# burchim/EfficientConformer

Hardware: AMD Instinct MI355X
Metric: audio-frames/sec through encoder, EffConformerCTC-Small, 1/2/4/8 GPU (higher is better)
Workload: dtype bf16; 1 GPU; EfficientConformerCTCSmall: bf16 operands / fp32 accumulate, B=256 utterances/GPU (the largest single-GPU batch measured; SURVEY.md 8d lists B in {4, 32, 128}: --batch 128 is 0.79 x this rate, profiles/r5_31_bench_b128.json), lognormal 1.5-16 s (LibriSpeech-shaped), sorted desc; ragged: every utterance at its own length in one concatenated row space per row range (no pad frames; outputs = the refe; global_batch=256, streams_per_gpu=3, parallelism=dp1 (utterance shards), row_ranges=3 ragged row range(s) per GPU, cut for equal valid frames

## Files before the change

efficientconformer_amd/csrc/attention2.hip:

```cpp
#include "kernels.h"

#include <cstdlib>
#include <type_traits>

namespace {

#ifdef EFFCONF_ABLATE
#define ABLATE(p) ((p).ablate)
#else
#define ABLATE(p) 0
#endif
constexpr int BJ = 64;
constexpr int SKEW_LD = 68;
constexpr float RESCALE_T = 4.0f;
constexpr float NEG_BIG = -1.0e30f;

__device__ __forceinline__ uint4 ld16(const bf16_t* p) {
    typedef uint32_t u32x4_a4 __attribute__((ext_vector_type(4), aligned(2)));
    const u32x4_a4 v = *reinterpret_cast<const u32x4_a4*>(p);
    return make_uint4(v[0], v[1], v[2], v[3]);
}

__device__ __forceinline__ uint4 ld16b(const char* p) { return ld16(reinterpret_cast<const bf16_t*>(p)); }

__device__ __forceinline__ void wave_sync() {
    __builtin_amdgcn_fence(__ATOMIC_RELEASE, "wavefront");
    __builtin_amdgcn_wave_barrier();
    __builtin_amdgcn_fence(__ATOMIC_ACQUIRE, "wavefront");
}

typedef short s16x4 __attribute__((ext_vector_type(4)));
__device__ __forceinline__ uint2 lds_tr16(const char* p) {
    const s16x4 v = __builtin_amdgcn_ds_read_tr16_b64_v4i16((__attribute__((address_space(3))) s16x4*)(p));
    union { s16x4 s; uint2 u; } c;
    c.s = v;
    return c.u;
}

template <int DP, int NWV, int QT>
struct Attn2Smem {
    static constexpr int BI = NWV * 16 * QT;
    static constexpr int ERING = 2 * BI;
    static constexpr bool SWZ = (DP == 64);
    static constexpr int KROW = SWZ ? DP * 2 : DP * 2 + 16;
    static __device__ __forceinline__ int koff(int row, int chunk) { return row * KROW + ((SWZ ? (chunk ^ (2 * ((row >> 1) & 3))) : chunk) << 4); }
    static constexpr int VP = DP * 2 + 32;
    static constexpr int K_BYTES = BJ * KROW, V_BYTES = BJ * VP, E_BYTES = ERING * KROW;
    static constexpr int S_BYTES = NWV * QT * 16 * SKEW_LD * 4;
    static constexpr int TOTAL = K_BYTES + V_BYTES + E_BYTES + S_BYTES;
};

template <int DP, int NWV, int QT, int SETS = 0>
__global__ __launch_bounds__(NWV * 64, (QT == 1 && NWV == 4 && DP <= 96) ? ((DP <= 64 && SETS == 1) ? 3 : 2) : 1) void relpos_attention2_kernel(const AttnParams p) {
    using SM = Attn2Smem<DP, NWV, QT>;
    constexpr int KS = DP / 32, DT = DP / 16, BI = SM::BI, NTHR = NWV * 64, CPR = DP / 8, ERING = SM::ERING;
    extern __shared__ __attribute__((aligned(16))) char smem[];
    char* sK = smem;
    char* sV = sK + SM::K_BYTES;
    char* sE = sV + SM::V_BYTES;
    float* sS = reinterpret_cast<float*>(sE + SM::E_BYTES);

    const int tid = threadIdx.x, lane = tid & 63, wave = tid >> 6;
    const int c = lane & 15, g = lane >> 4;
    int qtiles = (p.Tg + BI - 1) / BI;
    int id = xcd_remap(blockIdx.x, gridDim.x);
    int Tg = p.Tg, T = p.T, qt_wg, h, b;
    {
        const int per_b = p.H * qtiles, q8 = p.B >> 3, r8 = p.B & 7;
        const int u = p.rag_off ? ((ABLATE(p) & 8) ? (id * p.B) / (int)gridDim.x : ragged_find_wave(p.rag_wg, p.B, id)) : id / per_b;
        int x, j;
        if (u < r8 * (q8 + 1)) { x = u / (q8 + 1); j = u - x * (q8 + 1); }
        else { const int u2 = u - r8 * (q8 + 1); x = u2 / q8; j = u2 - x * q8; x += r8; }
        b = x + 8 * j;
        int local = id - (p.rag_off ? ((ABLATE(p) & 8) ? id : p.rag_wg[u]) : u * per_b);
        if (p.rag_off) { T = p.lens[b]; Tg = (T + p.G - 1) / p.G; qtiles = (Tg + BI - 1) / BI; }
        qt_wg = local % qtiles; h = local / qtiles;
    }
    if (ABLATE(p) & 128) return;
    const int i0 = qt_wg * BI, iw0 = i0 + wave * 16 * QT;
    const size_t orow0 = p.rag_off ? (size_t)p.rag_off[b] : (size_t)b * p.T;
    const size_t qoff = (p.rag_off ? orow0 * p.D : (size_t)b * p.q_bstride) + (size_t)h * p.q_hstride;
    const bf16_t* Qu = p.qu + qoff;
    const bf16_t* Kh = p.kh + qoff;
    const bf16_t* Vh = p.vt + qoff;
    const int RS = p.q_rowstride, ERS = p.e_rowstride;
    const bf16_t* Eh = p.eh + (size_t)h * p.e_hstride + (p.rag_off ? (size_t)(p.rag_tgmax - Tg) * ERS : 0);
    const int erows = p.causal ? Tg : 2 * Tg - 1;
    const int dceil = (p.d + 7) & ~7;
    const bool ragged_d = dceil != p.d;

    int nkv = (p.lens[b] + p.G - 1) / p.G;
    nkv = nkv < Tg ? nkv : Tg;
    const int band_l = p.band_l < Tg ? p.band_l : Tg, band_r = p.band_r < Tg ? p.band_r : Tg;
    const bool banded = band_l < Tg || band_r < Tg;
    const bool tile_dead = nkv < 1 || i0 + BI - 1 - band_l >= nkv;
    int kbeg = 0, nkeys = nkv;
    if (tile_dead) nkeys = Tg;
    else if (banded) {
        kbeg = i0 - band_l; kbeg = kbeg < 0 ? 0 : kbeg & ~(BJ - 1);
        const int ke = i0 + BI + band_r;
        nkeys = ke < nkv ? ke : nkv;
    }

    const int R0 = Tg - 1 - i0 - (BI - 1) + kbeg;
    constexpr int NB = ((BI + 63) * CPR + NTHR - 1) / NTHR;
    uint4 fb[NB];
    constexpr int NK = (BJ * CPR + NTHR - 1) / NTHR;
    struct Stage { uint4 lk[NK], lv[NK], le[NK]; };
    Stage sa, sb;
#pragma unroll
    for (int n = 0; n < NK; ++n) { sa.lk[n] = make_uint4(0, 0, 0, 0); sa.lv[n] = sa.lk[n]; sa.le[n] = sa.lk[n]; sb.lk[n] = sa.lk[n]; sb.lv[n] = sa.lk[n]; sb.le[n] = sa.lk[n]; }

    uint32_t koffs[NK];
    auto chunk_row = [&](int n) { int q = tid + NTHR * n; q = q < BJ * CPR ? q : BJ * CPR - 1; return q / CPR; };
    auto tail_mask = [&](uint4 a, int n) {
        int q = tid + NTHR * n; q = q < BJ * CPR ? q : BJ * CPR - 1;
        return mask_chunk(a, p.d - (q - (q / CPR) * CPR) * 8);
    };
#pragma unroll
    for (int n = 0; n < NK; ++n) {
        int q = tid + NTHR * n;
        q = q < BJ * CPR ? q : BJ * CPR - 1;
        const int r = q / CPR, x = (q - r * CPR) * 8, xc = x < dceil ? x : 0;
        koffs[n] = (uint32_t)(r * RS + xc) * 2u;
    }
    auto issue_loads = [&](Stage& st_, int jn) __attribute__((always_inline)) {
        if (((ABLATE(p) & 2) && jn > kbeg) || (ABLATE(p) & 64)) return;
        if (jn + BJ <= Tg - (ragged_d ? 1 : 0)) {
            const char* kb = reinterpret_cast<const char*>(Kh + (size_t)jn * RS);
            const char* vb = reinterpret_cast<const char*>(Vh + (size_t)jn * RS);
#pragma unroll
            for (int n = 0; n < NK; ++n) { st_.lk[n] = ld16b(kb + koffs[n]); st_.lv[n] = ld16b(vb + koffs[n]); }
        } else {
#pragma unroll
            for (int n = 0; n < NK; ++n) {
                const int kr = chunk_row(n), j = jn + kr;
                const size_t o = (size_t)(j < Tg ? j : Tg - 1) * RS * 2 + (koffs[n] - (uint32_t)(kr * RS) * 2u);
                st_.lk[n] = tail_mask(ld16b(reinterpret_cast<const char*>(Kh) + o), n); st_.lv[n] = tail_mask(ld16b(reinterpret_cast<const char*>(Vh) + o), n);
            }
        }
        if (jn > kbeg) {
            const int rnew = R0 + (jn - kbeg) + BI - 1;
            if (rnew >= 0 && rnew + 63 < erows - (ragged_d ? 1 : 0)) {
                const char* eb = reinterpret_cast<const char*>(Eh + (size_t)rnew * ERS);
#pragma unroll
                for (int n = 0; n < NK; ++n) st_.le[n] = ld16b(eb + koffs[n]);
            } else {
#pragma unroll
                for (int n = 0; n < NK; ++n) {
                    const int er = chunk_row(n);
                    int r = rnew + er;
                    r = r < 0 ? 0 : (r >= erows ? erows - 1 : r);
                    st_.le[n] = tail_mask(ld16b(reinterpret_cast<const char*>(Eh) + (size_t)r * ERS * 2 + (koffs[n] - (uint32_t)(er * RS) * 2u)), n);
                }
            }
        }
    };
    issue_loads(sa, kbeg);
#pragma unroll
    for (int n = 0; n < NB; ++n) {
        const int q = tid + NTHR * n;
        const int rr = q / CPR, x = (q - rr * CPR) * 8;
        const int r = R0 + (rr < BI + 63 ? rr : BI + 62);
        const int rc = r < 0 ? 0 : (r >= erows ? erows - 1 : r);
        fb[n] = (ABLATE(p) & 16) ? make_uint4(0, 0, 0, 0) : ld16(Eh + (size_t)rc * ERS + (x < dceil ? x : 0));
    }
    bf16x8 qu[QT][KS], qv[QT][KS];
    {
        const float* dv = p.dvu + (size_t)h * p.dvu_ld;
#pragma unroll
        for (int t = 0; t < QT; ++t) {
            const int i = iw0 + 16 * t + c, ic = i < Tg ? i : Tg - 1;
            uint4 ra[KS];
#pragma unroll
            for (int ks = 0; ks < KS; ++ks) {
                const int x = ks * 32 + g * 8;
                ra[ks] = (ABLATE(p) & 32) ? make_uint4(0, 0, 0, 0) : ld16(Qu + (size_t)ic * RS + (x < dceil ? x : 0));
            }
#pragma unroll
            for (int ks = 0; ks < KS; ++ks) {
                const int x = ks * 32 + g * 8;
                const float4 da = *reinterpret_cast<const float4*>(dv + x), db = *reinterpret_cast<const float4*>(dv + x + 4);
                const int valid = i < Tg ? p.d - x : 0;
                const uint4 m = mask_chunk(ra[ks], valid);
                qu[t][ks] = as_bf16x8(m);
                const uint4 w = make_uint4(pack_bf2(__uint_as_float(m.x << 16) + da.x, __uint_as_float(m.x & 0xFFFF0000u) + da.y),
                                           pack_bf2(__uint_as_float(m.y << 16) + da.z, __uint_as_float(m.y & 0xFFFF0000u) + da.w),
                                           pack_bf2(__uint_as_float(m.z << 16) + db.x, __uint_as_float(m.z & 0xFFFF0000u) + db.y),
                                           pack_bf2(__uint_as_float(m.w << 16) + db.z, __uint_as_float(m.w & 0xFFFF0000u) + db.w));
                qv[t][ks] = as_bf16x8(mask_chunk(w, valid));
            }
        }
    }
#pragma unroll
    for (int n = 0; n < NB; ++n) {
        const int q = tid + NTHR * n;
        const int rr = q / CPR, x = (q - rr * CPR) * 8;
        if (q < (BI + 63) * CPR)
            *reinterpret_cast<uint4*>(sE + SM::koff(rr, x >> 3)) = mask_chunk(fb[n], p.d - x);
    }

    f32x4 acc[QT][DT];
    float m_run[QT], l_run[QT];
#pragma unroll
    for (int t = 0; t < QT; ++t) {
        m_run[t] = NEG_BIG; l_run[t] = 0.f;
#pragma unroll
        for (int dt = 0; dt < DT; ++dt) acc[t][dt] = f32x4{0.f, 0.f, 0.f, 0.f};
    }
    const float scale2 = p.scale * 1.44269504088896340736f;
    float* skew0 = sS + (wave * QT) * 16 * SKEW_LD + c * SKEW_LD;
    const int wcol = c - 15 + 4 * g;
    const int woff1 = BI - 16 * QT - 16 * QT * wave;
    const char* vbase = sV + (4 * g + (c >> 2)) * SM::VP + (c & 3) * 8;

    static_assert(BI == 64, "ring phases: two (BI == BJ)");
    uint32_t ldk[NK], ldv[NK], lde[2][NK];
#pragma unroll
    for (int n = 0; n < NK; ++n) {
        int q = tid + NTHR * n;
        q = q < BJ * CPR ? q : BJ * CPR - 1;
        const int r = q / CPR, ch = q - r * CPR;
        ldk[n] = (uint32_t)SM::koff(r, ch);
        ldv[n] = (uint32_t)(r * SM::VP + ch * 16);
        lde[0][n] = (uint32_t)SM::koff((BI - 1 + r) & (ERING - 1), ch);
        lde[1][n] = (uint32_t)SM::koff((BI - 1 + r + 64) & (ERING - 1), ch);
    }
    constexpr bool FULL = (BJ * CPR) % NTHR == 0;
    auto publish = [&](const Stage& st_, int j0, int par) __attribute__((always_inline)) {
        __syncthreads();
#pragma unroll
        for (int n = 0; n < NK; ++n) {
            if (FULL || tid + NTHR * n < BJ * CPR) {
                *reinterpret_cast<uint4*>(sK + ldk[n]) = st_.lk[n];
                *reinterpret_cast<uint4*>(sV + ldv[n]) = st_.lv[n];
                if (j0 > kbeg) *reinterpret_cast<uint4*>(sE + lde[par][n]) = st_.le[n];
            }
        }
        __syncthreads();
    };

    auto compute_block = [&](int j0, int par, auto jtv) __attribute__((always_inline)) {
        constexpr int JTV = decltype(jtv)::value;
        f32x4 st[QT][JTV];
#pragma unroll
        for (int jt = 0; jt < JTV; ++jt) {
#pragma unroll
            for (int t = 0; t < QT; ++t) st[t][jt] = f32x4{0.f, 0.f, 0.f, 0.f};
#pragma unroll
            for (int ks = 0; ks < KS; ++ks) {
                const bf16x8 a = *reinterpret_cast<const bf16x8*>(sK + SM::koff(jt * 16 + c, ks * 4 + g));
#pragma unroll
                for (int t = 0; t < QT; ++t) st[t][jt] = __builtin_amdgcn_mfma_f32_16x16x32_bf16(a, qu[t][ks], st[t][jt], 0, 0, 0);
            }
        }
        const int rw1 = woff1 + 64 * par;
        constexpr int PU = JTV + 1;
        f32x4 pe[QT][PU];
#pragma unroll
        for (int t = 0; t < QT; ++t)
#pragma unroll
            for (int u = 0; u < PU; ++u) pe[t][u] = f32x4{0.f, 0.f, 0.f, 0.f};
#pragma unroll
        for (int u = 0; u < JTV + QT; ++u) {
            const int er = ((rw1 + u * 16) & (ERING - 1)) + c;
#pragma unroll
            for (int ks = 0; ks < KS; ++ks) {
                const bf16x8 a = *reinterpret_cast<const bf16x8*>(sE + SM::koff(er, ks * 4 + g));
#pragma unroll
                for (int t = 0; t < QT; ++t) {
                    const int ut = u - (QT - 1 - t);
                    if (ut >= 0 && ut < PU) pe[t][ut] = __builtin_amdgcn_mfma_f32_16x16x32_bf16(a, qv[t][ks], pe[t][ut], 0, 0, 0);
                }
            }
        }
#pragma unroll
        for (int t = 0; t < QT; ++t) {
            float* row = skew0 + t * 16 * SKEW_LD + wcol;
#pragma unroll
            for (int r = 0; r < 4; ++r) {
                const bool lo = wcol + r >= 0;
                row[r + (lo ? 0 : 16 * JTV)] = lo ? pe[t][0][r] : pe[t][JTV][r];
            }
#pragma unroll
            for (int u = 1; u < JTV; ++u)
#pragma unroll
                for (int r = 0; r < 4; ++r) row[u * 16 + r] = pe[t][u][r];
        }
        wave_sync();

#pragma unroll
        for (int t = 0; t < QT; ++t) {
            const float* skew = skew0 + t * 16 * SKEW_LD;
            float mloc = -INFINITY;
#pragma unroll
            for (int jt = 0; jt < JTV; ++jt) {
                const f32x4 s4 = *reinterpret_cast<const f32x4*>(skew + jt * 16 + g * 4);
#pragma unroll
                for (int r = 0; r < 4; ++r) st[t][jt][r] += s4[r];
            }
            const int iq0 = iw0 + 16 * t;
            if (j0 + BJ > nkv || (banded && (j0 - (iq0 + 15) < -band_l || j0 + BJ - 1 - iq0 > band_r))) {
                const int iq = iq0 + c;
#pragma unroll
                for (int jt = 0; jt < JTV; ++jt)
#pragma unroll
                    for (int r = 0; r < 4; ++r) {
                        const int j = j0 + jt * 16 + g * 4 + r, dj = j - iq;
                        st[t][jt][r] = (j < nkv && dj <= band_r && dj >= -band_l) ? st[t][jt][r] : NEG_BIG;
                    }
            }
            if (tile_dead) {
                const bool dead = nkv < 1 || iq0 + c - band_l >= nkv;
#pragma unroll
                for (int jt = 0; jt < JTV; ++jt)
#pragma unroll
                    for (int r = 0; r < 4; ++r) st[t][jt][r] = dead ? (j0 + jt * 16 + g * 4 + r < Tg ? 0.f : NEG_BIG) : st[t][jt][r];
            }
#pragma unroll
            for (int jt = 0; jt < JTV; ++jt)
#pragma unroll
                for (int r = 0; r < 4; ++r) mloc = fmaxf(mloc, st[t][jt][r]);
            mloc = fmaxf(mloc, __shfl_xor(mloc, 16));
            mloc = fmaxf(mloc, __shfl_xor(mloc, 32));
            if (!__all((mloc - m_run[t]) * scale2 <= RESCALE_T)) {
                const float m_new = fmaxf(m_run[t], mloc);
                const float alpha = __builtin_amdgcn_exp2f((m_run[t] - m_new) * scale2);
                l_run[t] *= alpha;
#pragma unroll
                for (int dt = 0; dt < DT; ++dt) { acc[t][dt][0] *= alpha; acc[t][dt][1] *= alpha; acc[t][dt][2] *= alpha; acc[t][dt][3] *= alpha; }
                m_run[t] = m_new;
            }
            const float nm = -m_run[t] * scale2;
            float lsum = 0.f;
#pragma unroll
            for (int jt = 0; jt < JTV; ++jt)
#pragma unroll
                for (int r = 0; r < 4; ++r) {
                    const float e = __builtin_amdgcn_exp2f(fmaf(st[t][jt][r], scale2, nm));
                    st[t][jt][r] = e;
                    lsum += e;
                }
            l_run[t] += lsum;
        }
#pragma unroll
        for (int c2 = 0; c2 < JTV / 2; ++c2) {
            bf16x8 pf[QT];
#pragma unroll
            for (int t = 0; t < QT; ++t) {
                uint4 pb;
                pb.x = pack_bf2(st[t][2 * c2][0], st[t][2 * c2][1]);
                pb.y = pack_bf2(st[t][2 * c2][2], st[t][2 * c2][3]);
                pb.z = pack_bf2(st[t][2 * c2 + 1][0], st[t][2 * c2 + 1][1]);
                pb.w = pack_bf2(st[t][2 * c2 + 1][2], st[t][2 * c2 + 1][3]);
                pf[t] = as_bf16x8(pb);
            }
#pragma unroll
            for (int dt = 0; dt < DT; ++dt) {
                const uint2 lo = lds_tr16(vbase + (2 * c2) * 16 * SM::VP + dt * 32);
                const uint2 hi = lds_tr16(vbase + (2 * c2 + 1) * 16 * SM::VP + dt * 32);
                const bf16x8 a = as_bf16x8(make_uint4(lo.x, lo.y, hi.x, hi.y));
#pragma unroll
                for (int t = 0; t < QT; ++t) acc[t][dt] = __builtin_amdgcn_mfma_f32_16x16x32_bf16(a, pf[t], acc[t][dt], 0, 0, 0);
            }
        }
    };

    const bool wave_idle = iw0 >= Tg;
    const bool short_ok = !tile_dead;
    auto run_block = [&](int j0, int par) __attribute__((always_inline)) {
        if (wave_idle || (ABLATE(p) & 1)) return;
        if (short_ok && nkeys - j0 <= 32) compute_block(j0, par, std::integral_constant<int, 2>{});
        else compute_block(j0, par, std::integral_constant<int, 4>{});
    };
    constexpr bool TWO_SETS = SETS == 2 || (SETS == 0 && !(NWV == 2 && DP >= 96));
    if constexpr (TWO_SETS) {
        if (kbeg + BJ < nkeys) issue_loads(sb, kbeg + BJ);
        for (int jb = kbeg; jb < nkeys; jb += 2 * BJ)
#pragma unroll
        for (int half2 = 0; half2 < 2; ++half2) {
            const int j0 = jb + half2 * BJ;
            if (j0 >= nkeys) break;
            if (half2 == 0) publish(sa, j0, 0); else publish(sb, j0, 1);
            if (j0 + 2 * BJ < nkeys) { if (half2 == 0) issue_loads(sa, j0 + 2 * BJ); else issue_loads(sb, j0 + 2 * BJ); }
            run_block(j0, half2);
        }
    } else {
        for (int jb = kbeg; jb < nkeys; jb += 2 * BJ)
#pragma unroll
        for (int half2 = 0; half2 < 2; ++half2) {
            const int j0 = jb + half2 * BJ;
            if (j0 >= nkeys) break;
            publish(sa, j0, half2);
            if (j0 + BJ < nkeys) issue_loads(sa, j0 + BJ);
            run_block(j0, half2);
        }
    }

#pragma unroll
    for (int t = 0; t < QT; ++t) {
        float l_tot = l_run[t] + __shfl_xor(l_run[t], 16);
        l_tot += __shfl_xor(l_tot, 32);
        const float inv = 1.0f / l_tot;
        const int i = iw0 + 16 * t + c;
        if (i >= Tg || (ABLATE(p) & 4)) continue;
#pragma unroll
        for (int dt = 0; dt < DT; ++dt) {
            const int x0 = dt * 16 + g * 4;
            if (x0 >= p.d) continue;
            int n0 = h * p.d + x0, toff = 0;
            while (n0 >= p.D) { n0 -= p.D; ++toff; }
            const int t0 = i * p.G + toff;
            if (x0 + 3 < p.d && n0 + 3 < p.D && (n0 & 1) == 0) {
                if (t0 < T || p.rag_off) {
                    typedef uint32_t u32x2_a4 __attribute__((ext_vector_type(2), aligned(4)));
                    u32x2_a4 w;
                    w[0] = t0 < T ? pack_bf2(acc[t][dt][0] * inv, acc[t][dt][1] * inv) : 0u;
                    w[1] = t0 < T ? pack_bf2(acc[t][dt][2] * inv, acc[t][dt][3] * inv) : 0u;
                    *reinterpret_cast<u32x2_a4*>(p.out + (orow0 + t0) * p.ldo + n0) = w;
                }
            } else {
#pragma unroll
                for (int r = 0; r < 4; ++r) {
                    const int x = x0 + r;
                    if (x >= p.d) continue;
                    int n = h * p.d + x, tf = 0;
                    while (n >= p.D) { n -= p.D; ++tf; }
                    const int tt = i * p.G + tf;
                    if (tt < T || p.rag_off) p.out[(orow0 + tt) * p.ldo + n] = tt < T ? f2bf(acc[t][dt][r] * inv) : (bf16_t)0;
                }
            }
        }
    }
}

template <int DP, int NWV, int QT, int SETS = 0>
int launch2(const AttnParams& p, hipStream_t s) {
    using SM = Attn2Smem<DP, NWV, QT>;
    static_assert(SM::TOTAL <= 160 * 1024, "LDS");
    static LdsAttr attr;
    ensure_dynamic_lds(reinterpret_cast<const void*>(&relpos_attention2_kernel<DP, NWV, QT, SETS>), SM::TOTAL, attr);
    const int qtiles = (p.Tg + SM::BI - 1) / SM::BI;
    const int nwg = p.rag_off ? p.rag_nwg : p.B * p.H * qtiles;
    if (nwg <= 0) return 0;
    hipLaunchKernelGGL((relpos_attention2_kernel<DP, NWV, QT, SETS>), dim3(nwg), dim3(NWV * 64), SM::TOTAL, s, p);
    return hipGetLastError() == hipSuccess ? 0 : -1;
}

}

bool relpos_attention2_supported(int dpad) { return dpad == 32 || dpad == 64 || dpad == 96 || dpad == 128 || dpad == 160; }

int launch_relpos_attention2(const AttnParams& p0, int waves, hipStream_t s) {
    if (p0.B <= 0 || p0.Tg <= 0) return 0;
    AttnParams p = p0;
#ifdef EFFCONF_ABLATE
    static const int abl = getenv("EFFCONF_ATTN_ABLATE") ? atoi(getenv("EFFCONF_ATTN_ABLATE")) : 0;
    p.ablate = abl;
#endif
    if (p.dpad < p.d || p.q_rowstride != p.e_rowstride) return -2;
    if (p.rag_off && (waves != 1 || !p.rag_wg || p.q_rowstride != p.G * p.D)) return -2;
#define ATT2_CASE(DPV, SETS1) case DPV: return waves == 1 ? launch2<DPV, 4, 1, SETS1>(p, s) : launch2<DPV, 2, 2>(p, s);
    switch (p.dpad) {
        ATT2_CASE(32, 0) ATT2_CASE(64, 1) ATT2_CASE(96, 1) ATT2_CASE(128, 0)
        case 160: return launch2<160, 4, 1>(p, s);
    }
#undef ATT2_CASE
    return -3;
}
```

efficientconformer_amd/csrc/encoder.hip:

```cpp
#include "kernels.h"
#include "../../include/effconf.h"
#ifdef EFFCONF_DEBUG_ABI
#include "../../include/effconf_debug.h"
#endif

#include <cmath>
#include <cstdio>
#include <cstdlib>
#include <cstring>
#include <map>
#include <string>
#include <vector>

namespace {

thread_local std::string g_err;
int fail(const std::string& m) { g_err = m; return -1; }
#define EC_TRY(expr) do { int _rc = (expr); if (_rc != 0) return fail(std::string(#expr) + " failed rc=" + std::to_string(_rc)); } while (0)

inline int ld8(int d) { return ec_round_up(d, 8); }

#ifdef EFFCONF_ABLATE
static int ablate_mask() { static const int m = getenv("EFFCONF_SKIP") ? atoi(getenv("EFFCONF_SKIP")) : 0; return m; }
#define EC_ABL(bit, stmt) do { if (!(ablate_mask() & (bit))) { stmt; } } while (0)
#else
#define EC_ABL(bit, stmt) do { stmt; } while (0)
#endif

uint16_t h_f2bf(float f) {
    uint32_t u; memcpy(&u, &f, 4);
    u += 0x7FFFu + ((u >> 16) & 1u);
    return (uint16_t)(u >> 16);
}

struct HostTensor { std::vector<float> data; std::vector<int64_t> shape; };

struct PackedLinear { const bf16_t* w = nullptr; const float* bias = nullptr; int N = 0, K = 0, ldw = 0; std::vector<float> hbias;  };
struct LNp { const float* g = nullptr; const float* b = nullptr; };

struct BlockW {
    LNp ln_ffn1, ln_att, ln_conv, ln_ffn2, ln_out;
    PackedLinear ffn1_a, ffn1_b, qkv, qkv_nat, pos, outp, pw1, pw2, res, ffn2_a, ffn2_b;
    const bf16_t *ffn1_bp = nullptr, *ffn2_bp = nullptr;
    const float *u = nullptr, *v = nullptr, *dw_w = nullptr, *dw_b = nullptr;
    const uint16_t* dw_a3 = nullptr;
    const uint16_t* dw_a = nullptr;
    const float* dvu = nullptr; int dvu_ld = 0;
    const bf16_t* pos_table = nullptr;
    bool chain_in = false, chain_out = false;
    PackedLinear c_outp, c_pw1, c_pw2, c_qkv, c_f1a, c_f2a;
    const bf16_t *c_f1b_cm = nullptr, *c_f2b_cm = nullptr;
    const bf16_t *c_f1b = nullptr, *c_f2b = nullptr; const float *c_f1b2 = nullptr, *c_f2b2 = nullptr;
    int c_qkv_chunks = 0, c_pw1_chunks = 0;
    std::vector<float> h_ln_out_g, h_ln_out_b, h_u, h_v, h_f1b2, h_f2b2;
    const uint16_t *xf_img[2] = {nullptr, nullptr}; const float* xf_b2[2] = {nullptr, nullptr}; int xf_nch[2] = {0, 0};
    const uint16_t *xc_wo = nullptr, *xc_p1 = nullptr, *xc_p2 = nullptr, *xc_qkv = nullptr, *xc_f[2] = {nullptr, nullptr};
    const float *xc_bo = nullptr, *xc_bp2 = nullptr; int xc_nch_p1 = 0;
    bool xc_in = false, xc_out = false;
    const float *cc_b = nullptr, *cc_head = nullptr, *cc_tail = nullptr, *cc_full = nullptr;
};

struct TraceEntry { char name[64]; int64_t offset, rows, cols, ld; int32_t dtype; };
struct ProfRec { int cls; double flops, bytes; };

}

int ec_fail(const char* msg) { return fail(msg ? msg : "error"); }


struct EcEncoder {
    EcConfig cfg;
    std::vector<EcBlock> blocks;
    std::map<std::string, HostTensor> host;
    bool finalized = false;
    std::vector<void*> allocs;
    int wide_gemm = 0;
    size_t guard_bytes = 0;
    const float *sub_w9 = nullptr, *sub_b = nullptr;
    PackedLinear lin;
    const bf16_t* lin_fused = nullptr; int lin_fused_ld = 0;
    const uint16_t *sub3_cimg = nullptr, *sub3_wimg = nullptr; const float* sub3_bias = nullptr; int sub3_ncb = 0, sub3_fo = 0;
    const bf16_t* lin_rs = nullptr; const float* conv_tab = nullptr;
    int fuse_subsample = 2;
    bool fuse_chain = true;
    int ctc_mfma = 2;
    int attention_v2 = 1;
    int chain_full_max = 192;
    int dwconv_mfma = 1;
    int chain_pair = 5;
    int chain_small_m = 4096;
    int chain_max_dim = 256;
    int tiled_auto = 1;
    bool tiled_auto_on = false;
    int tiled_min_k = 256;
    std::vector<float*> att_out;
    int split_chain = 1;
    int sub3_auto = 1;
    int split_sublin = 1;
    int split_ffn = 1;
    int exact_attention = 0;
    bool head_major_odd = false;
    const bf16_t* sub2_w = nullptr; const float* sub2_b = nullptr; int sub2_cp = 0;
    std::vector<BlockW> bw;
    const float *fc_wt = nullptr, *fc_b = nullptr;
    const bf16_t *fc_hi = nullptr, *fc_lo = nullptr;
    const int* block_stride = nullptr;
    const int *block_group = nullptr, *block_heads = nullptr;
    MelTables mel{};
    char* trace_arena = nullptr; size_t trace_bytes = 0, trace_used = 0;
    std::vector<TraceEntry> trace;
    bool e_cache_on = false;
    struct ECacheTag { const void* ws; int batch, tm; size_t layout; };
    std::vector<ECacheTag> e_cache;
    static constexpr size_t E_CACHE_MAX = 16;
    bool e_cache_hit(const void* ws, int batch, int tm, size_t layout) const {
        for (const ECacheTag& t : e_cache) if (t.ws == ws) return t.batch == batch && t.tm == tm && t.layout == layout;
        return false;
    }
    void e_cache_put(const void* ws, int batch, int tm, size_t layout) {
        e_cache_drop(ws);
        if (e_cache.size() >= E_CACHE_MAX) e_cache.erase(e_cache.begin());
        e_cache.push_back({ws, batch, tm, layout});
    }
    void e_cache_drop(const void* ws) {
        for (size_t i = 0; i < e_cache.size(); ++i) if (e_cache[i].ws == ws) { e_cache.erase(e_cache.begin() + i); break; }
    }
    bool exact_pack = false, exact_on = false;
    bool exact_split = false;
    struct SplitW { const uint16_t *hi, *lo; int ldh; };
    std::map<std::string, SplitW> xsplit;
    std::map<std::string, const float*> xw;
    std::map<std::pair<int, int>, const float*> xtab;
    const float *xsub_scale[2] = {nullptr, nullptr}, *xsub_shift[2] = {nullptr, nullptr};
    const uint16_t *xsub_cimg = nullptr, *xsub_wimg = nullptr; const float* xsub_bias = nullptr; int xsub_ncb = 0, xsub_fo = 0;
    bool prof_on = false;
    std::vector<hipEvent_t> prof_ev;
    std::vector<ProfRec> prof_rec;
    size_t prof_next = 0;
};

namespace {

template <class T>
const T* upload(EcEncoder* e, const std::vector<T>& v) {
    const size_t guard = e->guard_bytes, used = v.size() * sizeof(T);
    void* d = nullptr;
    size_t bytes = std::max<size_t>((used + 15) / 16 * 16, 16);
    if (hipMalloc(&d, bytes + 2 * guard) != hipSuccess) return nullptr;
    e->allocs.push_back(d);
    char* base = static_cast<char*>(d) + guard;
    if (guard && (hipMemset(d, 0xFF, guard) != hipSuccess || hipMemset(base + used, 0xFF, bytes - used + guard) != hipSuccess)) return nullptr;
    if (!v.empty() && hipMemcpy(base, v.data(), used, hipMemcpyHostToDevice) != hipSuccess) return nullptr;
    return reinterpret_cast<const T*>(base);
}

const HostTensor* find(EcEncoder* e, const std::string& k) {
    auto it = e->host.find(k);
    return it == e->host.end() ? nullptr : &it->second;
}

bool pack_linear(EcEncoder* e, const std::vector<const float*>& row_ptr, const std::vector<float>& bias, int K, PackedLinear* out,
                 bool kperm = false, const float* ln_g = nullptr, const float* ln_b = nullptr, int min_ldw = 0) {
    const int N = (int)row_ptr.size();
    const int Np = ec_round_up(N, 128), Kp = ec_round_up(K > min_ldw ? K : min_ldw, 64);
    std::vector<uint16_t> w((size_t)Np * Kp, 0);
    std::vector<float> b(Np, 0.f);
    for (int n = 0; n < N && n < (int)bias.size(); ++n) b[n] = bias[n];
    for (int n = 0; n < N; ++n) {
        if (!row_ptr[n]) continue;
        for (int k = 0; k < Kp; ++k) {
            int src = k;
            if (kperm) { const int g = k / 16, pp = k % 16, hh = pp >> 3, ee = pp & 7; src = g * 16 + 4 * hh + 8 * (ee >> 2) + (ee & 3); }
            if (src < K) w[(size_t)n * Kp + k] = h_f2bf(row_ptr[n][src] * (ln_g ? ln_g[src] : 1.0f));
        }
        if (ln_b) {
            double acc = 0.0;
            for (int k = 0; k < K; ++k) acc += (double)row_ptr[n][k] * ln_b[k];
            b[n] += (float)acc;
        }
    }
    out->w = upload(e, w);
    out->bias = upload(e, b);
    out->hbias = b;
    out->N = N; out->K = K; out->ldw = Kp;
    return out->w && out->bias;
}

bool pack_named_linear(EcEncoder* e, const std::string& prefix, int N, int K, PackedLinear* out, std::string* err, bool kperm = false,
                       const std::string& fold_ln = "", int min_ldw = 0) {
    const HostTensor* w = find(e, prefix + ".weight");
    const HostTensor* b = find(e, prefix + ".bias");
    if (!w || !b) { *err = "missing tensor " + prefix + ".weight/.bias"; return false; }
    if ((int64_t)w->data.size() != (int64_t)N * K || (int)b->data.size() != N) { *err = "shape mismatch for " + prefix; return false; }
    std::vector<const float*> rows(N);
    for (int n = 0; n < N; ++n) rows[n] = w->data.data() + (size_t)n * K;
    const HostTensor *lg = fold_ln.empty() ? nullptr : find(e, fold_ln + ".weight"), *lb = fold_ln.empty() ? nullptr : find(e, fold_ln + ".bias");
    if (!fold_ln.empty() && (!lg || !lb || (int)lg->data.size() != K || (int)lb->data.size() != K)) { *err = "missing LayerNorm " + fold_ln; return false; }
    return pack_linear(e, rows, b->data, K, out, kperm, lg ? lg->data.data() : nullptr, lb ? lb->data.data() : nullptr, min_ldw);
}

const bf16_t* pack_ffn2_permuted(EcEncoder* e, const std::string& prefix, int D, int F, float scale = 1.0f) {
    const HostTensor* w = find(e, prefix + ".weight");
    if (!w || (int64_t)w->data.size() != (int64_t)D * F) return nullptr;
    const int Np = ec_round_up(D, 128), Kp = ec_round_up(F, 64);
    std::vector<uint16_t> out((size_t)Np * Kp, 0);
    for (int n = 0; n < D; ++n)
        for (int k = 0; k < Kp; ++k) {
            const int g = k / 16, pp = k % 16, hh = pp >> 3, ee = pp & 7;
            const int src = g * 16 + 4 * hh + 8 * (ee >> 2) + (ee & 3);
            if (src < F) out[(size_t)n * Kp + k] = h_f2bf(scale * w->data[(size_t)n * F + src]);
        }
    return upload(e, out);
}

const bf16_t* pack_ffn2_chunkmajor(EcEncoder* e, const std::string& prefix, int D, int F, float scale, int DP) {
    const HostTensor* w = find(e, prefix + ".weight");
    if (!w || (int64_t)w->data.size() != (int64_t)D * F) return nullptr;
    const int nch = ec_round_up(F, 32) / 32;
    std::vector<uint16_t> out((size_t)nch * DP * 32, 0);
    for (int c = 0; c < nch; ++c)
        for (int n = 0; n < DP; ++n)
            for (int pc = 0; pc < 4; ++pc) {
                const int slot = 4 * n + ((pc + (n >> 2)) & 3);
                for (int i = 0; i < 8; ++i) {
                    const int k = 32 * c + 8 * pc + i;
                    const int g = k / 16, pp = k % 16, hh = pp >> 3, ee = pp & 7;
                    const int src = g * 16 + 4 * hh + 8 * (ee >> 2) + (ee & 3);
                    if (n < D && src < F) out[((size_t)c * DP * 4 + slot) * 8 + i] = h_f2bf(scale * w->data[(size_t)n * F + src]);
                }
            }
    return upload(e, out);
}

bool get_ln(EcEncoder* e, const std::string& prefix, int D, LNp* out, std::string* err) {
    const HostTensor* g = find(e, prefix + ".weight");
    const HostTensor* b = find(e, prefix + ".bias");
    if (!g || !b || (int)g->data.size() != D || (int)b->data.size() != D) { *err = "missing/mis-shaped LayerNorm " + prefix; return false; }
    out->g = upload(e, g->data);
    out->b = upload(e, b->data);
    return out->g && out->b;
}

constexpr float kSplitImgMax = 65000.f;
constexpr float kDwMfmaTwoPlaneNorm = 6.0f;

bool bn_fold(EcEncoder* e, const std::string& prefix, int C, std::vector<float>* scale, std::vector<float>* shift, std::string* err) {
    const HostTensor *g = find(e, prefix + ".weight"), *b = find(e, prefix + ".bias");
    const HostTensor *m = find(e, prefix + ".running_mean"), *v = find(e, prefix + ".running_var");
    if (!g || !b || !m || !v || (int)g->data.size() != C) { *err = "missing/mis-shaped BatchNorm " + prefix; return false; }
    scale->resize(C); shift->resize(C);
    for (int c = 0; c < C; ++c) {
        const float s = g->data[c] / std::sqrt(v->data[c] + 1e-5f);
        (*scale)[c] = s;
        (*shift)[c] = b->data[c] - m->data[c] * s;
    }
    return true;
}

const bf16_t* build_pos_table(EcEncoder* e, int max_pos, int D) {
    const int rows = 2 * max_pos - 1, ld = ld8(D);
    std::vector<uint16_t> t((size_t)rows * ld, 0);
    std::vector<float> denom(D / 2);
    for (int i = 0; i < D / 2; ++i) denom[i] = std::pow(10000.0f, (2.0f * (float)i) / (float)D);
    for (int r = 0; r < rows; ++r) {
        const float pos = (float)(max_pos - 1 - r);
        for (int i = 0; i < D / 2; ++i) {
            const float a = pos / denom[i];
            t[(size_t)r * ld + 2 * i] = h_f2bf(std::sin(a));
            t[(size_t)r * ld + 2 * i + 1] = h_f2bf(std::cos(a));
        }
    }
    return upload(e, t);
}

std::string mel_config_error(const EcConfig& c) {
    if (c.n_fft != 512) return "n_fft = " + std::to_string(c.n_fft) + ": only n_fft = 512 is native";
    if (c.win_length <= 0 || c.win_length > c.n_fft) return "win_length = " + std::to_string(c.win_length) + ": must be in 1..n_fft (" + std::to_string(c.n_fft) + ")";
    if (c.hop_length <= 0) return "hop_length = " + std::to_string(c.hop_length) + ": must be >= 1";
    if (c.n_mels < 1 || c.n_mels > 128) return "n_mels = " + std::to_string(c.n_mels) + ": must be in 1..128";
    if (c.sample_rate < 2) return "sample_rate = " + std::to_string(c.sample_rate) + ": must be >= 2";
    return "";
}

bool build_mel_tables(EcEncoder* e, std::string* err) {
    const EcConfig& c = e->cfg;
    *err = mel_config_error(c);
    if (!err->empty()) return false;
    std::vector<float> win(c.n_fft, 0.f);
    const int off = (c.n_fft - c.win_length) / 2;
    for (int n = 0; n < c.win_length; ++n) win[off + n] = (float)(0.5 - 0.5 * std::cos(2.0 * M_PI * n / c.win_length));
    std::vector<float2> tw(c.n_fft / 2);
    for (int k = 0; k < c.n_fft / 2; ++k) {
        const double a = -2.0 * M_PI * k / c.n_fft;
        tw[k] = make_float2((float)std::cos(a), (float)std::sin(a));
    }
    const int nf = c.n_fft / 2 + 1, nm = c.n_mels;
    const double fmin = 0.0, fmax = 8000.0;
    auto hz2mel = [](double f) { return 2595.0 * std::log10(1.0 + f / 700.0); };
    auto mel2hz = [](double m) { return 700.0 * (std::pow(10.0, m / 2595.0) - 1.0); };
    std::vector<double> fpts(nm + 2);
    for (int i = 0; i < nm + 2; ++i) fpts[i] = mel2hz(hz2mel(fmin) + (hz2mel(fmax) - hz2mel(fmin)) * i / (nm + 1));
    std::vector<int> start(nm), count(nm), offs(nm);
    std::vector<float> wts;
    for (int m = 0; m < nm; ++m) {
        int s0 = -1, cnt = 0;
        std::vector<float> row;
        for (int k = 0; k < nf; ++k) {
            const double f = (double)(c.sample_rate / 2) * k / (nf - 1);
            const double down = (f - fpts[m]) / (fpts[m + 1] - fpts[m]);
            const double up = (fpts[m + 2] - f) / (fpts[m + 2] - fpts[m + 1]);
            const double w = std::max(0.0, std::min(down, up));
            if (w > 0.0) {
                if (s0 < 0) s0 = k;
                row.resize(k - s0 + 1, 0.f);
                row[k - s0] = (float)w;
                cnt = k - s0 + 1;
            }
        }
        start[m] = s0 < 0 ? 0 : s0; count[m] = cnt; offs[m] = (int)wts.size();
        wts.insert(wts.end(), row.begin(), row.begin() + cnt);
    }
    e->mel.window = upload(e, win);
    e->mel.twiddle = upload(e, tw);
    e->mel.fb_start = upload(e, start);
    e->mel.fb_count = upload(e, count);
    e->mel.fb_offset = upload(e, offs);
    e->mel.fb_nnz = (int)wts.size();
    e->mel.fb_weight = upload(e, wts);
    return e->mel.window && e->mel.twiddle && e->mel.fb_weight;
}

struct Shapes {
    int B, Tm, T1;
    std::vector<int> Tin, Tout;
    std::vector<long long> Min, Mout, Mq;
    bool ragged = false;
    std::vector<int> wgs, tiles;
    std::vector<double> tg2;
    long long Mfinal = 0;
};

Shapes make_shapes(const EcEncoder* e, int B, int Tm) {
    Shapes s; s.B = B; s.Tm = Tm;
    int t = Tm;
    for (int i = 0; i < e->cfg.sub_layers; ++i) t = (t - 1) / 2 + 1;
    s.T1 = t;
    for (const EcBlock& b : e->blocks) {
        s.Tin.push_back(t);
        s.Min.push_back((long long)B * t);
        s.Mq.push_back((long long)B * ec_round_up(t, b.group_size));
        if (b.conv_stride > 1) t = (t - 1) / b.conv_stride + 1;
        s.Tout.push_back(t);
        s.Mout.push_back((long long)B * t);
    }
    return s;
}

Shapes make_shapes_ragged(const EcEncoder* e, const std::vector<int>& tm) {
    const int B = (int)tm.size(), nb = (int)e->blocks.size();
    int tmax = 0;
    for (int v : tm) tmax = std::max(tmax, v);
    Shapes s = make_shapes(e, B, tmax);
    s.ragged = true;
    s.Min.assign(nb, 0); s.Mout.assign(nb, 0); s.Mq.assign(nb, 0); s.wgs.assign(nb, 0); s.tiles.assign(nb, 0); s.tg2.assign(nb, 0.0);
    for (int b = 0; b < B; ++b) {
        int t = tm[b];
        for (int i = 0; i < e->cfg.sub_layers; ++i) t = (t - 1) / 2 + 1;
        for (int k = 0; k < nb; ++k) {
            const EcBlock& bk = e->blocks[k];
            const int G = bk.group_size, Gn = k + 1 < nb ? e->blocks[k + 1].group_size : 1;
            const int tp = ec_round_up(t, G);
            s.Min[k] += tp; s.Mq[k] += tp;
            s.wgs[k] += bk.num_heads * ec_cdiv(tp / G, 64);
            s.tg2[k] += (double)(tp / G) * (tp / G);
            if (bk.conv_stride > 1) t = (t - 1) / bk.conv_stride + 1;
            const int top = ec_round_up(t, Gn);
            s.Mout[k] += top;
            s.tiles[k] += ec_cdiv(top, 128);
        }
        s.Mfinal += t;
    }
    return s;
}

struct Workspace {
    size_t total = 0;
    size_t mel, sub, sub1, x0, x1, a, hbuf, qu, kh, vt, eh, o, gbuf, cbuf, xs, lens, preds;
    size_t mel_len = 0, row_off = 0, wg_off = 0, tile_off = 0;
    size_t xrect = 0;
// ... 61 lines not shown
    ProfScope(EcEncoder* e_, hipStream_t st_, int cls, double flops, double bytes) : e(e_), st(st_), on(e_->prof_on) {
        if (!on) return;
        if (e->prof_next + 2 > e->prof_ev.size()) {
            for (int i = 0; i < 2; ++i) { hipEvent_t ev; (void)hipEventCreate(&ev); e->prof_ev.push_back(ev); }
        }
        e->prof_rec.push_back(ProfRec{cls, flops, bytes});
        (void)hipEventRecord(e->prof_ev[e->prof_next], st);
    }
    ~ProfScope() {
        if (!on) return;
        (void)hipEventRecord(e->prof_ev[e->prof_next + 1], st);
        e->prof_next += 2;
    }
};
#define PROF(cls, flops, bytes) ProfScope _prof_scope(e, st, (cls), (double)(flops), (double)(bytes))

void trace_add(EcEncoder* e, hipStream_t st, const char* name, const void* ptr, int64_t rows, int64_t cols, int64_t ld, int dtype) {
    if (!e->trace_arena) return;
    const size_t esz = dtype == 1 ? 2 : 4;
    const size_t bytes = (size_t)rows * ld * esz;
    const size_t off = al(e->trace_used);
    if (off + bytes > e->trace_bytes) return;
    (void)hipMemcpyAsync(e->trace_arena + off, ptr, bytes, hipMemcpyDeviceToDevice, st);
    TraceEntry t{};
    snprintf(t.name, sizeof(t.name), "%s", name);
    t.offset = (int64_t)off; t.rows = rows; t.cols = cols; t.ld = ld; t.dtype = dtype;
    e->trace.push_back(t);
    e->trace_used = off + bytes;
}

enum ProfClass { PC_MEL = 0, PC_SUBCONV = 1, PC_GEMM_FFN = 2, PC_GEMM_OTHER = 3, PC_LAYERNORM = 4, PC_ATTENTION = 5,
                 PC_DWCONV = 6, PC_MISC = 7, PC_COUNT = 8 };

int run_gemm(EcEncoder* e, int cls, hipStream_t st, const bf16_t* A, int lda, int M, const PackedLinear& L, int epi, void* C, int ldc,
             const float* R = nullptr, int ldr = 0, float alpha = 1.f) {
    const double out_b = (epi == EPI_F32) ? 4.0 : (epi == EPI_RESID_F32 ? 8.0 : 2.0);
    PROF(cls, 2.0 * M * (double)L.N * L.K, (double)M * L.K * 2 + (double)L.N * L.K * 2 + (double)M * L.N * out_b);
    GemmParams p{};
    p.A = A; p.lda = lda; p.W = L.w; p.ldw = L.ldw; p.bias = L.bias;
    p.M = M; p.N = L.N; p.K = L.K; p.C = C; p.ldc = ldc; p.R = R; p.ldr = ldr; p.alpha = alpha;
    p.wide = e->wide_gemm;
    return launch_gemm(p, epi, st);
}

inline int F1c(const EcBlock& b) { return ec_round_up(b.dim_model * b.ff_ratio, 32); }

void fill_chain_head(ChainParams& cp, const BlockW& W, int D, int Fp, int T, int Tp, const GemmParams& q) {
    cp.D = D;
    cp.ln[2] = ChainLn{W.ln_ffn1.g, W.ln_ffn1.b};
    cp.ln[3] = ChainLn{W.ln_att.g, W.ln_att.b};
    cp.f[1] = ChainFfn{W.c_f1a.w, W.c_f1a.ldw, W.c_f1a.bias, W.c_f1b, W.ffn1_b.ldw, W.c_f1b2, Fp, W.c_f1b_cm};
    cp.g1 = ChainGemm{W.c_qkv.w, W.c_qkv.ldw, W.c_qkv.bias, W.c_qkv_chunks};
    cp.qu = q.qu; cp.kh = q.kh; cp.vt = q.vt; cp.u = W.u; cp.v = W.v; cp.T = T; cp.Tp = Tp;
}

bool prefer_tiled(const EcEncoder* e, int M, int N, int K);

int run_ffn(EcEncoder* e, hipStream_t st, const bf16_t* a, int M, int D, const PackedLinear& L1, const PackedLinear& L2,
            const bf16_t* w2p, float* x, bf16_t* hbuf, const LNp* ln = nullptr) {
    const int F = L1.N;
    if (ffn_fused_supported(D) && !(prefer_tiled(e, M, F, D) && !ln)) {
        PROF(PC_GEMM_FFN, 4.0 * M * (double)D * F, (double)M * D * 10 + 4.0 * D * F);
        FfnParams p{};
        p.A = a; p.lda = ld8(D); p.X = x; p.ldx = D; p.Y = x; p.ldy = D;
        p.W1 = L1.w; p.ldw1 = L1.ldw; p.b1 = L1.bias; p.W2 = w2p; p.ldw2 = L2.ldw; p.b2 = L2.bias;
        p.M = M; p.D = D; p.Fp = ec_round_up(F, 32); p.alpha = 0.5f;
        if (ln) { p.ln_g = ln->g; p.ln_b = ln->b; }
        return launch_ffn_fused(p, st);
    }
    int rc = run_gemm(e, PC_GEMM_FFN, st, a, ld8(D), M, L1, EPI_SWISH_BF16, hbuf, F);
    if (rc) return rc;
    return run_gemm(e, PC_GEMM_FFN, st, hbuf, F, M, L2, EPI_RESID_F32, x, D, x, D, 0.5f);
}

bool prefer_tiled(const EcEncoder* e, int M, int N, int K) {
    (void)M; (void)N;
    return (e->wide_gemm == 2 || e->wide_gemm == 3 || (e->wide_gemm == 0 && (e->tiled_auto == 2 || (e->tiled_auto && e->tiled_auto_on)))) && K > e->tiled_min_k && K % 8 == 0;
}

int run_rs_or_tiled(EcEncoder* e, int cls, hipStream_t st, const bf16_t* A, int lda, int M, const PackedLinear& L, int rs_epi,
                    int tiled_epi, void* C, int ldc, const float* R = nullptr, int ldr = 0, float alpha = 1.f,
                    const float* lnX = nullptr, const LNp* ln = nullptr) {
    const bool ok = (rs_epi == 0 || rs_epi == 1) ? rs_gemm_resident_supported(L.K, L.N) : rs_gemm_supported(L.K);
    if (!ok) return run_gemm(e, cls, st, A, lda, M, L, tiled_epi, C, ldc, R, ldr, alpha);
    if (prefer_tiled(e, M, L.N, L.K)) {
        if (lnX && ln) { PROF(PC_LAYERNORM, 0, (double)M * L.K * 6); EC_TRY(launch_layernorm(lnX, M, L.K, ln->g, ln->b, nullptr, const_cast<bf16_t*>(A), lda, nullptr, nullptr, st)); }
        return run_gemm(e, cls, st, A, lda, M, L, tiled_epi, C, ldc, R, ldr, alpha);
    }
    const double out_b = (tiled_epi == EPI_F32) ? 4.0 : (tiled_epi == EPI_RESID_F32 ? 8.0 : 2.0);
    PROF(cls, 2.0 * M * (double)L.N * L.K, (double)M * L.K * 2 + (double)L.N * L.K * 2 + (double)M * L.N * out_b);
    GemmParams p{};
    p.A = A; p.lda = lda; p.W = L.w; p.ldw = L.ldw; p.bias = L.bias;
    p.M = M; p.N = L.N; p.K = L.K; p.C = C; p.ldc = ldc; p.R = R; p.ldr = ldr; p.alpha = alpha;
    if (lnX && ln) { p.X = lnX; p.ldx = L.K; p.ln_g = ln->g; p.ln_b = ln->b; }
    return launch_rs_gemm(p, rs_epi, st);
}

bool use_sublinear3(const EcEncoder* e) {
    if (!e->sub3_wimg || e->cfg.sub_layers != 1) return false;
    if (e->fuse_subsample == 3) return true;
    return e->fuse_subsample == 2 && e->sub3_auto && (e->cfg.sub_filters[0] > 128 || e->blocks[0].dim_model > 128);
}

int run_subsample_linear(EcEncoder* e, hipStream_t st, const float* mel, int B, int Tm, int T1, bf16_t* sub, bf16_t* act1, float* x) {
    const EcConfig& c = e->cfg;
    const int C0 = c.sub_filters[0], F2 = c.n_mels / 2, Ksub = C0 * F2;
    if (c.sub_layers == 2) {
        const int Tl1 = (Tm - 1) / 2 + 1, F1 = c.n_mels / 2, F2q = c.n_mels / 4, C1 = c.sub_filters[1];
        { PROF(PC_SUBCONV, 2.0 * 9 * B * Tl1 * (double)C0 * F1, (double)B * c.n_mels * Tm * 4 + (double)B * Tl1 * F1 * e->sub2_cp * 2);
          EC_TRY(launch_subsample_conv_cl(mel, B, c.n_mels, Tm, Tl1, e->sub_w9, e->sub_b, C0, e->sub2_cp, act1, st)); }
        trace_add(e, st, "subsample1", act1, (int64_t)B * F1 * Tl1, C0, e->sub2_cp, 1);
        { PROF(PC_GEMM_OTHER, 2.0 * 9 * (double)B * F2q * T1 * C0 * C1, (double)B * Tl1 * F1 * e->sub2_cp * 2 + (double)B * T1 * F2q * C1 * 2);
          EC_TRY(launch_conv2_igemm(act1, B, F1, Tl1, e->sub2_cp, e->sub2_w, 9 * e->sub2_cp, e->sub2_b, C1, F2q, T1, sub, st)); }
        trace_add(e, st, "subsample", sub, (int64_t)B * T1, F2q * C1, F2q * C1, 1);
        EC_TRY(run_gemm(e, PC_GEMM_OTHER, st, sub, F2q * C1, B * T1, e->lin, EPI_F32, x, e->lin.N));
    } else if (use_sublinear3(e)) {
        PROF(PC_SUBCONV, 2.0 * 9 * B * T1 * (double)Ksub + 2.0 * B * T1 * (double)Ksub * e->lin.N,
             (double)B * c.n_mels * Tm * 4 + (double)B * T1 * e->lin.N * 4);
        SubLin3Params sp{};
        sp.mel = mel; sp.B = B; sp.F = c.n_mels; sp.Tm = Tm; sp.To = T1; sp.rows_max = T1;
        sp.cimg = e->sub3_cimg; sp.wimg = e->sub3_wimg; sp.bias = e->sub3_bias; sp.y = x; sp.ldy = e->lin.N; sp.N = e->lin.N; sp.ncb = e->sub3_ncb; sp.Fo = e->sub3_fo;
        EC_TRY(launch_sublinear3(sp, st));
    } else if (e->fuse_subsample >= 2 && e->lin_rs) {
        PROF(PC_SUBCONV, 2.0 * 9 * B * T1 * (double)Ksub + 2.0 * B * T1 * (double)Ksub * e->lin.N,
             (double)B * c.n_mels * Tm * 4 + (double)B * T1 * e->lin.N * 4);
        EC_TRY(launch_sublinear2(mel, B, c.n_mels, Tm, T1, e->conv_tab, e->lin_rs, e->lin.bias, C0, e->lin.N, x, e->lin.N, st));
    } else if (e->fuse_subsample && e->lin_fused) {
        PROF(PC_SUBCONV, 2.0 * 9 * B * T1 * (double)Ksub + 2.0 * B * T1 * (double)Ksub * e->lin.N,
             (double)B * c.n_mels * Tm * 4 + (double)B * T1 * e->lin.N * 4);
        EC_TRY(launch_sublinear_fused(mel, B, c.n_mels, Tm, T1, e->sub_w9, e->sub_b, C0, e->lin_fused, e->lin_fused_ld,
                                      e->lin.bias, e->lin.N, x, e->lin.N, st));
    } else {
        { PROF(PC_SUBCONV, 2.0 * 9 * B * T1 * (double)Ksub, (double)B * c.n_mels * Tm * 4 + (double)B * T1 * Ksub * 2); EC_TRY(launch_subsample_conv(mel, B, c.n_mels, Tm, T1, e->sub_w9, e->sub_b, C0, sub, Ksub, st)); }
        trace_add(e, st, "subsample", sub, (int64_t)B * T1, Ksub, Ksub, 1);
        EC_TRY(run_gemm(e, PC_GEMM_OTHER, st, sub, Ksub, B * T1, e->lin, EPI_F32, x, e->lin.N));
    }
    return 0;
}

static const void* dw_mfma_table(const EcEncoder* e, const uint16_t* t, int ks) { return (e->dwconv_mfma == 2 || (e->dwconv_mfma == 1 && ks == 15)) ? t : nullptr; }
static bool pair_on(const EcEncoder* e, int D) { return e->chain_pair && chain3_supported(D); }

int forward_core(EcEncoder* e, const float* mel, const int64_t* in_len, int from_audio, const Shapes& s, const Workspace& w,
                 char* ws, float* out, int64_t* out_len, hipStream_t st, int out_frames = 0) {
    const EcConfig& c = e->cfg;
    const int B = s.B, nb = (int)e->blocks.size();
    const bool rg = s.ragged;
    e->trace.clear(); e->trace_used = 0;
    int* lens = reinterpret_cast<int*>(ws + w.lens);
    const int *mel_len = nullptr, *row_off = nullptr, *wg_off = nullptr, *tile_off = nullptr;
    if (rg) {
        int* ml = reinterpret_cast<int*>(ws + w.mel_len); int* ro = reinterpret_cast<int*>(ws + w.row_off);
        int* wo = reinterpret_cast<int*>(ws + w.wg_off); int* to = reinterpret_cast<int*>(ws + w.tile_off);
        PROF(PC_MISC, 0, 0);
        EC_TRY(launch_lengths_ragged(in_len, B, from_audio, c.hop_length, c.sub_layers, e->block_stride, e->block_group, e->block_heads, nb, lens, ml,
                                     ro, wo, to, out_len, st));
        mel_len = ml; row_off = ro; wg_off = wo; tile_off = to;
    } else {
        PROF(PC_MISC, 0, 0); EC_TRY(launch_lengths(in_len, B, from_audio, c.hop_length, c.sub_layers, e->block_stride, nb, lens, out_len, st));
    }
    if (from_audio) trace_add(e, st, "mel", mel, (int64_t)B * c.n_mels, s.Tm, s.Tm, 0);
    auto rows_at = [&](int k) { RaggedRows r{}; r.off = row_off + (size_t)k * (B + 1); r.len = lens + (size_t)k * B; r.n = B;
                                r.rows = (int)(k < nb ? s.Min[k] : s.Mfinal); r.tmax = k < nb ? s.Tin[k] : s.Tout[nb - 1]; return r; };

    float* x = reinterpret_cast<float*>(ws + w.x0);
    float* xalt = reinterpret_cast<float*>(ws + w.x1);
    if (rg) {
        const int C0 = c.sub_filters[0], Ksub = C0 * (c.n_mels / 2);
        const RaggedRows r0 = rows_at(0);
        if (c.sub_layers == 2) {
            bf16_t* sub = reinterpret_cast<bf16_t*>(ws + w.sub);
            bf16_t* act1 = reinterpret_cast<bf16_t*>(ws + w.sub1);
            float* xrect = reinterpret_cast<float*>(ws + w.xrect);
            const int Tl1 = (s.Tm - 1) / 2 + 1, T1r = (Tl1 - 1) / 2 + 1, F1 = c.n_mels / 2, F2q = c.n_mels / 4, C1 = c.sub_filters[1];
            { PROF(PC_SUBCONV, 2.0 * 9 * B * Tl1 * (double)C0 * F1, (double)B * c.n_mels * s.Tm * 4 + (double)B * Tl1 * F1 * e->sub2_cp * 2);
              EC_TRY(launch_subsample_conv_cl(mel, B, c.n_mels, s.Tm, Tl1, e->sub_w9, e->sub_b, C0, e->sub2_cp, act1, st, mel_len)); }
            trace_add(e, st, "subsample1", act1, (int64_t)B * F1 * Tl1, C0, e->sub2_cp, 1);
            { PROF(PC_GEMM_OTHER, 2.0 * 9 * (double)B * F2q * T1r * C0 * C1, (double)B * Tl1 * F1 * e->sub2_cp * 2 + (double)B * T1r * F2q * C1 * 2);
              EC_TRY(launch_conv2_igemm(act1, B, F1, Tl1, e->sub2_cp, e->sub2_w, 9 * e->sub2_cp, e->sub2_b, C1, F2q, T1r, sub, st)); }
            trace_add(e, st, "subsample", sub, (int64_t)B * T1r, F2q * C1, F2q * C1, 1);
            EC_TRY(run_gemm(e, PC_GEMM_OTHER, st, sub, F2q * C1, B * T1r, e->lin, EPI_F32, xrect, e->lin.N));
            { PROF(PC_MISC, 0, (double)s.Min[0] * e->lin.N * 8); EC_TRY(launch_gather_rows(xrect, e->lin.N, T1r, r0, x, st)); }
        } else if (use_sublinear3(e)) {
            PROF(PC_SUBCONV, 2.0 * 9 * (double)s.Min[0] * Ksub + 2.0 * (double)s.Min[0] * Ksub * e->lin.N, (double)B * c.n_mels * s.Tm * 4 + (double)s.Min[0] * e->lin.N * 4);
            SubLin3Params sp{};
            sp.mel = mel; sp.B = B; sp.F = c.n_mels; sp.Tm = s.Tm; sp.mel_len = mel_len; sp.off = r0.off; sp.len = r0.len;
            sp.rows_max = ec_round_up(s.Tin[0], e->blocks[0].group_size);
            sp.cimg = e->sub3_cimg; sp.wimg = e->sub3_wimg; sp.bias = e->sub3_bias; sp.y = x; sp.ldy = e->lin.N; sp.N = e->lin.N; sp.ncb = e->sub3_ncb; sp.Fo = e->sub3_fo;
            EC_TRY(launch_sublinear3(sp, st));
        } else if (e->fuse_subsample >= 2 && e->lin_rs) {
            PROF(PC_SUBCONV, 2.0 * 9 * (double)s.Min[0] * Ksub + 2.0 * (double)s.Min[0] * Ksub * e->lin.N, (double)B * c.n_mels * s.Tm * 4 + (double)s.Min[0] * e->lin.N * 4);
            EC_ABL(32, EC_TRY(launch_sublinear2(mel, B, c.n_mels, s.Tm, s.T1, e->conv_tab, e->lin_rs, e->lin.bias, C0, e->lin.N, x, e->lin.N, st, &r0, mel_len)));
        } else {
            bf16_t* sub = reinterpret_cast<bf16_t*>(ws + w.sub);
            const int T1r = (s.Tm - 1) / 2 + 1;
            const int Tcover = T1r + e->blocks[0].group_size - 1;
            { PROF(PC_SUBCONV, 2.0 * 9 * (double)s.Min[0] * Ksub, (double)B * c.n_mels * s.Tm * 4 + (double)s.Min[0] * Ksub * 2);
              EC_TRY(launch_subsample_conv(mel, B, c.n_mels, s.Tm, Tcover, e->sub_w9, e->sub_b, C0, sub, Ksub, st, mel_len, &r0)); }
            trace_add(e, st, "subsample", sub, s.Min[0], Ksub, Ksub, 1);
            EC_TRY(run_gemm(e, PC_GEMM_OTHER, st, sub, Ksub, (int)s.Min[0], e->lin, EPI_F32, x, e->lin.N));
        }
    } else {
        EC_TRY(run_subsample_linear(e, st, mel, B, s.Tm, s.T1, reinterpret_cast<bf16_t*>(ws + w.sub), reinterpret_cast<bf16_t*>(ws + w.sub1), x));
    }
    trace_add(e, st, "linear", x, s.Min[0], e->lin.N, e->lin.N, 0);

    bf16_t* a = reinterpret_cast<bf16_t*>(ws + w.a);
    bf16_t* hbuf = reinterpret_cast<bf16_t*>(ws + w.hbuf);
    bf16_t* o = reinterpret_cast<bf16_t*>(ws + w.o);
    bf16_t* gbuf = reinterpret_cast<bf16_t*>(ws + w.gbuf);
    bf16_t* cbuf = reinterpret_cast<bf16_t*>(ws + w.cbuf);
    bf16_t* xs = reinterpret_cast<bf16_t*>(ws + w.xs);
    bool have_a = false, head_done = false;
    char nm[64];
    hipStreamCaptureStatus cap = hipStreamCaptureStatusNone;
    const bool capturing = hipStreamIsCapturing(st, &cap) == hipSuccess && cap != hipStreamCaptureStatusNone;
    const int e_tag = rg ? -(s.Tin[0] + 1) : s.Tm;
    const bool e_cached = !capturing && e->e_cache_on && e->e_cache_hit(ws, B, e_tag, w.eh_blk[0]);
    if (!e_cached) e->e_cache_drop(ws);

    int mask_stride = 1;
    for (int k = 0; k < nb; ++k) {
        const EcBlock& b = e->blocks[k];
        const BlockW& W = e->bw[k];
        const int T = s.Tin[k], To = s.Tout[k], D = b.dim_model, De = b.dim_expand;
        const int M = (int)s.Min[k], Mo = (int)s.Mout[k];
        const int G = b.group_size, H = b.num_heads;
        const int Tp = ec_round_up(T, G), Tg = Tp / G, Tgp = ec_round_up(Tg, 8);
        const int d = G * D / H, dpad = ec_round_up(d, 32);
        const bool head_major_odd = e->head_major_odd;
        const bool nat = (d % 2) == 0 || !head_major_odd;
        if (rg && !nat) return fail("ragged batches use the natural Q / K / V layout (option head_major_odd = 0)");
        const int qT = rg ? M : T, qTp = rg ? M : Tp;
        const bool chain_head = e->fuse_chain && W.chain_in && nat && chain_head_supported(D) && D <= e->chain_max_dim;
        const bool chain_b = e->fuse_chain && W.chain_in && D <= e->chain_max_dim;
        const bool chain_tail = e->fuse_chain && W.chain_out && chain_tail_supported(De) && De <= e->chain_max_dim;
        GemmParams p{};
        p.A = a; p.lda = ld8(D); p.W = W.qkv.w; p.ldw = W.qkv.ldw; p.bias = W.qkv.bias;
        p.M = M; p.N = 3 * D; p.K = D;
        p.T = qT; p.G = rg ? 1 : G; p.H = H; p.D = D; p.d = d; p.dpad = dpad; p.Tg = rg ? M : Tg; p.Tgp = Tgp;
        p.qu = reinterpret_cast<bf16_t*>(ws + w.qu);
        p.kh = reinterpret_cast<bf16_t*>(ws + w.kh); p.vt = reinterpret_cast<bf16_t*>(ws + w.vt);
        p.u = W.u; p.v = W.v;
        if (head_done) {
        } else if (chain_head) {
            ChainParams cp{};
            cp.small_m = e->chain_small_m; cp.pair = e->chain_pair;
            fill_chain_head(cp, W, D, F1c(b), qT, qTp, p);
            cp.M = M; cp.X = x; cp.ldx = D; cp.Y = x; cp.ldy = D; cp.consts = W.cc_head;
            PROF(PC_GEMM_FFN, 2.0 * M * (double)D * (2.0 * D * b.ff_ratio + 3.0 * D), (double)M * D * 16 + 22.0 * D * D);
            EC_ABL(2, EC_TRY(launch_chain(cp, CHAIN_A_HEAD, st)));
        } else {
            { PROF(PC_LAYERNORM, 0, (double)M * D * 6); if (!have_a) EC_TRY(launch_layernorm(x, M, D, W.ln_ffn1.g, W.ln_ffn1.b, nullptr, a, ld8(D), nullptr, nullptr, st)); }
            EC_TRY(run_ffn(e, st, a, M, D, W.ffn1_a, W.ffn1_b, W.ffn1_bp, x, hbuf));
            const bool qkv_tiled = nat && prefer_tiled(e, M, 3 * D, D);
            const bool ln_fused = rs_gemm_supported(D) && !qkv_tiled;
            if (!ln_fused) { PROF(PC_LAYERNORM, 0, (double)M * D * 6); EC_TRY(launch_layernorm(x, M, D, W.ln_att.g, W.ln_att.b, nullptr, a, ld8(D), nullptr, nullptr, st)); }
            { PROF(PC_GEMM_OTHER, 2.0 * M * 3.0 * D * D, (double)M * D * 2 + 3.0 * D * D * 2 + (double)M * D * 8);
              if (ln_fused) {
                  if (nat) { p.W = W.qkv_nat.w; p.ldw = W.qkv_nat.ldw; p.bias = W.qkv_nat.bias; }
                  p.X = x; p.ldx = D; p.ln_g = W.ln_att.g; p.ln_b = W.ln_att.b;
                  EC_TRY(launch_rs_gemm(p, nat ? 4 : 3, st));
              } else {
                  p.wide = e->wide_gemm;
                  EC_TRY(launch_gemm(p, nat ? EPI_QKV_NAT : EPI_QKV, st));
              } }
        }
        snprintf(nm, sizeof(nm), "blocks.%d.x_ffn1", k); trace_add(e, st, nm, x, M, D, D, 0);

        {
            { PROF(PC_MISC, 0, 0);
              if (rg) EC_ABL(64, EC_TRY(launch_attn_pad_rows_ragged(p.qu, p.kh, p.vt, W.u, D, G, rows_at(k), st)));
              else EC_TRY(nat ? launch_attn_pad_rows_nat(p, B, st) : launch_attn_pad_rows(p, B, st)); }
            GemmParams pe{};
            const int erows = c.causal ? Tp : 2 * Tp - G;
            pe.A = W.pos_table + (size_t)(b.max_pos - Tp + (c.causal ? 0 : G / 2)) * ld8(D); pe.lda = ld8(D);
            pe.W = W.pos.w; pe.ldw = W.pos.ldw; pe.bias = W.pos.bias;
            pe.M = erows; pe.N = D; pe.K = D;
            pe.T = erows; pe.G = G; pe.H = H; pe.D = D; pe.d = d; pe.dpad = dpad; pe.Tg = c.causal ? Tg : 2 * Tg - 1; pe.Tgp = 0;
            pe.kh = reinterpret_cast<bf16_t*>(ws + w.eh_blk[k]);
            pe.C = pe.kh; pe.ldc = D;
            if (Tp > b.max_pos) return fail("sequence longer than max_pos_encoding");
            if (!e_cached) { PROF(PC_GEMM_OTHER, 2.0 * erows * (double)D * D, (double)erows * D * 4 + (double)D * D * 2);
                             EC_TRY(launch_gemm(pe, nat ? EPI_BF16 : EPI_HEADS, st)); }
            if (e->trace_arena && nat) {
                const int64_t qrows = rg ? (int64_t)M : (int64_t)B * Tp;
                snprintf(nm, sizeof(nm), "blocks.%d.qu", k); trace_add(e, st, nm, p.qu, qrows, D, D, 1);
                snprintf(nm, sizeof(nm), "blocks.%d.k", k); trace_add(e, st, nm, p.kh, qrows, D, D, 1);
                snprintf(nm, sizeof(nm), "blocks.%d.v", k); trace_add(e, st, nm, p.vt, qrows, D, D, 1);
                snprintf(nm, sizeof(nm), "blocks.%d.e", k); trace_add(e, st, nm, pe.kh, erows, D, D, 1);
            }
            AttnParams ap{};
            ap.qu = p.qu; ap.kh = p.kh; ap.vt = p.vt; ap.eh = pe.kh;
            ap.dvu = W.dvu; ap.dvu_ld = W.dvu_ld;
            ap.lens = lens + (size_t)k * B;
            ap.B = B; ap.H = H; ap.T = T; ap.G = G; ap.D = D; ap.d = d; ap.dpad = dpad; ap.Tg = Tg; ap.Tgp = Tgp;
            if (nat) { ap.q_bstride = (long long)Tp * D; ap.q_hstride = d; ap.q_rowstride = G * D; ap.e_hstride = d; ap.e_rowstride = G * D; }
            else { ap.q_bstride = (long long)H * Tg * dpad; ap.q_hstride = (long long)Tg * dpad; ap.q_rowstride = dpad;
                   ap.e_hstride = (long long)(2 * Tg - 1) * dpad; ap.e_rowstride = dpad; }
            ap.out = o; ap.ldo = ld8(D); ap.scale = 1.0f / std::sqrt((float)d);
            const long long unit = (long long)mask_stride * G;
            ap.band_l = (int)std::min<long long>(c.left_context / unit, 1 << 30); ap.band_r = (int)std::min<long long>(c.right_context / unit, 1 << 30);
            ap.causal = c.causal;
            const bool streaming = c.causal || ap.band_l < Tg || ap.band_r < Tg;
            if (streaming && !(nat && relpos_attention2_supported(dpad) && e->attention_v2))
                return fail("streaming contexts / causal attention run on attention2.hip (natural layout, padded head width <= 160, option attention_v2 != 0)");
            if (rg) {
                if (!relpos_attention2_supported(dpad)) return fail("ragged batches need attention2.hip (padded head width <= 160)");
                ap.rag_off = row_off + (size_t)k * (B + 1); ap.rag_wg = wg_off + (size_t)k * (B + 1); ap.rag_nwg = s.wgs[k]; ap.rag_tgmax = Tg;
            }
            { PROF(PC_ATTENTION, 2.0 * H * (rg ? s.tg2[k] : (double)B * Tg * Tg) * d * 3.0, (double)M * D * 2 * 5);
              if (rg || streaming) EC_ABL(1, EC_TRY(launch_relpos_attention2(ap, 1, st))); else
              if (e->attention_v2 && nat && relpos_attention2_supported(dpad)) EC_TRY(launch_relpos_attention2(ap, e->attention_v2, st));
              else EC_TRY(launch_relpos_attention(ap, st)); }
            if ((int)e->att_out.size() == nb && e->att_out[k]) {
                EC_TRY(launch_attention_probs(ap, e->att_out[k], st));
            }
            snprintf(nm, sizeof(nm), "blocks.%d.att_o", k); trace_add(e, st, nm, o, M, D, ld8(D), 1);
            if (chain_b) {
                ChainParams cp{};
                cp.small_m = e->chain_small_m; cp.pair = e->chain_pair;
                cp.M = M; cp.D = D; cp.X = x; cp.ldx = D; cp.Y = x; cp.ldy = D; cp.A = o; cp.lda = ld8(D);
                cp.g0 = ChainGemm{W.c_outp.w, W.c_outp.ldw, W.c_outp.bias, 0};
                cp.ln[0] = ChainLn{W.ln_conv.g, W.ln_conv.b};
                cp.g1 = ChainGemm{W.c_pw1.w, W.c_pw1.ldw, W.c_pw1.bias, W.c_pw1_chunks};
                cp.glu = gbuf; cp.ldg = ld8(De); cp.Ng = De; cp.T = qT; cp.Tp = qTp; cp.consts = W.cc_b;
                PROF(PC_GEMM_OTHER, 2.0 * M * (double)D * (D + 2.0 * De), (double)M * D * 10 + (double)M * De * 2 + 2.0 * D * (D + 2.0 * De));
                EC_ABL(4, EC_TRY(launch_chain(cp, CHAIN_B, st)));
            } else {
                EC_TRY(run_rs_or_tiled(e, PC_GEMM_OTHER, st, o, ld8(D), M, W.outp, 0, EPI_RESID_F32, x, D, x, D, 1.0f));
            }
            snprintf(nm, sizeof(nm), "blocks.%d.x_mhsa", k); trace_add(e, st, nm, x, M, D, D, 0);
        }

        if (chain_b) {
        } else if (rs_gemm_supported(D)) {
            EC_TRY(run_rs_or_tiled(e, PC_GEMM_OTHER, st, a, ld8(D), M, W.pw1, 2, EPI_GLU_BF16, gbuf, ld8(De), nullptr, 0, 1.f, x, &W.ln_conv));
        } else {
            { PROF(PC_LAYERNORM, 0, (double)M * D * 6); EC_TRY(launch_layernorm(x, M, D, W.ln_conv.g, W.ln_conv.b, nullptr, a, ld8(D), nullptr, nullptr, st)); }
            EC_TRY(run_rs_or_tiled(e, PC_GEMM_OTHER, st, a, ld8(D), M, W.pw1, 2, EPI_GLU_BF16, gbuf, ld8(De)));
        }
        snprintf(nm, sizeof(nm), "blocks.%d.glu", k); trace_add(e, st, nm, gbuf, M, De, ld8(De), 1);
        RaggedConv rc{};
        if (rg) { rc.in_off = row_off + (size_t)k * (B + 1); rc.in_len = lens + (size_t)k * B; rc.out_off = row_off + (size_t)(k + 1) * (B + 1);
                  rc.out_len = lens + (size_t)(k + 1) * B; rc.tile_off = tile_off + (size_t)k * (B + 1); rc.tiles = s.tiles[k]; rc.n = B; rc.out_rows = Mo; }
        { PROF(PC_DWCONV, 2.0 * Mo * (double)De * b.kernel_size, (double)M * De * 2 + (double)Mo * De * 2); EC_ABL(8, EC_TRY(launch_dwconv(gbuf, B, T, To, De, ld8(De), W.dw_w, W.dw_b, b.kernel_size, b.conv_stride, cbuf, st, rg ? &rc : nullptr, c.causal, dw_mfma_table(e, W.dw_a, b.kernel_size), W.dw_a3))); }
        mask_stride *= b.conv_stride;
        snprintf(nm, sizeof(nm), "blocks.%d.dw", k); trace_add(e, st, nm, cbuf, Mo, De, ld8(De), 1);
        if (D != De) {
            { PROF(PC_MISC, 0, (double)Mo * D * 6); EC_ABL(64, EC_TRY(launch_cast_rows(x, D, T, b.conv_stride, To, B, xs, ld8(D), st, rg ? &rc : nullptr))); }
            EC_TRY(run_rs_or_tiled(e, PC_GEMM_OTHER, st, xs, ld8(D), Mo, W.res, 1, EPI_F32, xalt, De));
            std::swap(x, xalt);
        } else if (b.conv_stride > 1) {
            return fail("strided block without expansion is not native (no shipped config uses it)");
        }
        const bool last = (k == nb - 1);
        float* xo = (last && !rg) ? out : x;
        if (chain_tail) {
            bool next_head = false;
            if (!last) {
                const EcBlock& nbk = e->blocks[k + 1];
                next_head = W.cc_full && nbk.dim_model <= e->chain_max_dim && e->bw[k + 1].chain_in && chain_full_supported(De, pair_on(e, De) ? 256 : e->chain_full_max) && (((nbk.group_size * nbk.dim_model / nbk.num_heads) % 2) == 0 || !head_major_odd) && nbk.dim_model == De;
            }
            ChainParams cp{};
            cp.small_m = e->chain_small_m; cp.pair = e->chain_pair;
            cp.M = Mo; cp.D = De; cp.X = x; cp.ldx = De; cp.Y = xo; cp.ldy = De; cp.A = cbuf; cp.lda = ld8(De);
            cp.g0 = ChainGemm{W.c_pw2.w, W.c_pw2.ldw, W.c_pw2.bias, 0};
            cp.ln[0] = ChainLn{W.ln_ffn2.g, W.ln_ffn2.b};
            cp.ln[1] = ChainLn{W.ln_out.g, W.ln_out.b};
            cp.f[0] = ChainFfn{W.c_f2a.w, W.c_f2a.ldw, W.c_f2a.bias, W.c_f2b, W.ffn2_b.ldw, W.c_f2b2, ec_round_up(De * b.ff_ratio, 32), W.c_f2b_cm};
            double fl = 2.0 * Mo * (double)De * (De + 2.0 * De * b.ff_ratio), by = (double)Mo * De * 10 + 2.0 * De * De * (1 + 2.0 * b.ff_ratio);
            if (next_head) {
                const EcBlock& nbk = e->blocks[k + 1];
                const int Gn = nbk.group_size;
                const int Tn = rg ? Mo : s.Tin[k + 1], Tpn = rg ? Mo : ec_round_up(Tn, Gn);
                GemmParams pn{};
                pn.qu = reinterpret_cast<bf16_t*>(ws + w.qu);
                pn.kh = reinterpret_cast<bf16_t*>(ws + w.kh); pn.vt = reinterpret_cast<bf16_t*>(ws + w.vt);
                fill_chain_head(cp, e->bw[k + 1], De, F1c(nbk), Tn, Tpn, pn);
                fl += 2.0 * Mo * (double)De * (2.0 * De * nbk.ff_ratio + 3.0 * De); by += (double)Mo * De * 8 + 2.0 * De * De * (3 + 2.0 * nbk.ff_ratio);
            }
            cp.consts = next_head ? W.cc_full : W.cc_tail;
            { PROF(PC_GEMM_FFN, fl, by); EC_ABL(2, EC_TRY(launch_chain(cp, next_head ? CHAIN_A_FULL : CHAIN_A_TAIL, st))); }
            head_done = next_head;
            have_a = false;
            if (last) { snprintf(nm, sizeof(nm), "blocks.%d.out", k); trace_add(e, st, nm, xo, Mo, De, De, 0); }
            continue;
        }
        head_done = false;
        EC_TRY(run_rs_or_tiled(e, PC_GEMM_OTHER, st, cbuf, ld8(De), Mo, W.pw2, 0, EPI_RESID_F32, x, De, x, De, 1.0f));
        snprintf(nm, sizeof(nm), "blocks.%d.x_conv", k); trace_add(e, st, nm, x, Mo, De, De, 0);

        if (ffn_fused_supported(De) && !prefer_tiled(e, Mo, De * b.ff_ratio, De)) {
            EC_TRY(run_ffn(e, st, a, Mo, De, W.ffn2_a, W.ffn2_b, W.ffn2_bp, x, hbuf, &W.ln_ffn2));
        } else {
            { PROF(PC_LAYERNORM, 0, (double)Mo * De * 6); EC_TRY(launch_layernorm(x, Mo, De, W.ln_ffn2.g, W.ln_ffn2.b, nullptr, a, ld8(De), nullptr, nullptr, st)); }
            EC_TRY(run_ffn(e, st, a, Mo, De, W.ffn2_a, W.ffn2_b, W.ffn2_bp, x, hbuf));
        }
        { PROF(PC_LAYERNORM, 0, (double)Mo * De * 10); EC_TRY(launch_layernorm(x, Mo, De, W.ln_out.g, W.ln_out.b, xo, last ? nullptr : a, ld8(De),
                                last ? nullptr : e->bw[k + 1].ln_ffn1.g, last ? nullptr : e->bw[k + 1].ln_ffn1.b, st)); }
        have_a = !last;
        snprintf(nm, sizeof(nm), "blocks.%d.out", k); trace_add(e, st, nm, xo, Mo, De, De, 0);
    }
    if (!capturing) e->e_cache_put(ws, B, e_tag, w.eh_blk[0]);
    if (rg) {
        const RaggedRows rl = rows_at(nb);
        PROF(PC_MISC, 0, (double)s.Mfinal * e->blocks.back().dim_expand * 4 + (double)B * out_frames * e->blocks.back().dim_expand * 4);
        EC_TRY(launch_emit_rows(x, e->blocks.back().dim_expand, rl.off, rl.len, B, out_frames, out, st));
    }
    return 0;
}

struct XWorkspace { size_t total = 0, conv1, sub, x0, x1, a, h, q, k, v, e, o, p1, g, c, lens, scores = 0; size_t qkv_stride = 0;
                    std::vector<size_t> ep_blk;
                    size_t kp = 0, vp = 0, ep = 0, xs = 0, xrect = 0, mel_len = 0, row_off = 0, wg_off = 0, tile_off = 0; };

XWorkspace make_xworkspace(const EcEncoder* e, const Shapes& s) {
    XWorkspace w;
    size_t off = 0;
    auto take = [&](size_t floats) { size_t o = off; off += al(floats * 4); return o; };
    const size_t B = s.B;
    size_t mx = 0, mh = 0, mq = 0, me = 0, mp = 0, mg = 0, mc = 0, mkp = 0, mvp = 0, mep = 0, mxs = 0;
    for (size_t k = 0; k < e->blocks.size(); ++k) {
        const EcBlock& b = e->blocks[k];
        const size_t T = s.Tin[k], D = b.dim_model, De = b.dim_expand;
        const size_t Mi = (size_t)s.Min[k], Mo = (size_t)s.Mout[k], Mqk = (size_t)s.Mq[k];
        const size_t Tp = ec_round_up((int)T, b.group_size);
        mx = std::max(mx, std::max(Mi * D, Mo * De));
        mh = std::max(mh, std::max(Mi * D, Mo * De) * b.ff_ratio);
        mq = std::max(mq, Mqk * D);
        me = std::max(me, (2 * Tp - b.group_size) * D);
        {
            const size_t dh = b.group_size * D / b.num_heads, pk = sxf_attention_pk((int)dh), vx = sxf_attention_vx((int)dh), Tg = Tp / b.group_size;
            mkp = std::max(mkp, (Mqk / b.group_size + 64) * b.num_heads * 2 * pk / 2);
            mvp = std::max(mvp, B * b.num_heads * 2 * vx * (size_t)ec_round_up((int)Tg, 64) / 2);
            mep = std::max(mep, 2 * Tg * b.num_heads * 2 * pk / 2);
        }
        mp = std::max(mp, Mi * 2 * De);
        mg = std::max(mg, Mi * De);
        mc = std::max(mc, Mo * De);
        if (D != De) mxs = std::max(mxs, Mo * D);
    }
    const int L = e->cfg.sub_layers;
    size_t T1r = s.Tm; for (int i = 0; i < L; ++i) T1r = (T1r - 1) / 2 + 1;
    const size_t F1 = (e->cfg.n_mels - 1) / 2 + 1, Tl1 = (s.Tm - 1) / 2 + 1;
    w.conv1 = take(L == 2 ? B * e->cfg.sub_filters[0] * F1 * Tl1 : 0);
    int F = e->cfg.n_mels; for (int i = 0; i < L; ++i) F = (F - 1) / 2 + 1;
    w.sub = take(B * T1r * (size_t)e->cfg.sub_filters[L - 1] * F);
    w.x0 = take(mx); w.x1 = take(mx); w.a = take(mx); w.h = take(mh);
    w.q = take(mq); w.k = take(mq); w.v = take(mq); w.e = take(me); w.o = take(mq);
    w.p1 = take(mp); w.g = take(mg); w.c = take(mc);
    w.lens = take((e->blocks.size() + 1) * B);
    w.qkv_stride = (w.k - w.q) / 4;
    if (e->exact_split) {
        size_t ms = 0;
        if (!s.ragged)
            for (size_t k = 0; k < e->blocks.size(); ++k) {
                const EcBlock& b = e->blocks[k];
                const int Tg = ec_round_up(s.Tin[k], b.group_size) / b.group_size;
                ms = std::max(ms, sx_attention_scores_bytes(s.B, b.num_heads, Tg) / 4);
            }
        w.scores = take(ms);
        w.kp = take(mkp); w.vp = take(mvp); w.ep = take(mep); w.xs = take(mxs);
        for (size_t k = 0; k < e->blocks.size(); ++k) {
            const EcBlock& b = e->blocks[k];
            const size_t dh = b.group_size * b.dim_model / b.num_heads, pk = sxf_attention_pk((int)dh), Tg = ec_round_up(s.Tin[k], b.group_size) / b.group_size;
            w.ep_blk.push_back(take(2 * Tg * b.num_heads * 2 * pk / 2));
        }
        if (s.ragged) {
            const size_t nbk = e->blocks.size();
            w.xrect = take(B * T1r * e->blocks[0].dim_model);
            w.mel_len = take(B);
            w.row_off = take((nbk + 1) * (B + 1));
            w.wg_off = take(nbk * (B + 1));
            w.tile_off = take(nbk * (B + 1));
        }
    }
    w.total = off;
    return w;
}

const float* xget(EcEncoder* e, const std::string& k) {
    auto it = e->xw.find(k);
    return it == e->xw.end() ? nullptr : it->second;
}

int xgemm(EcEncoder* e, hipStream_t st, const float* A, int lda, int M, const std::string& prefix, int N, int K, float* C, int ldc, int epi = 0,
          const float* R = nullptr, float alpha = 1.f, int a_rows = 0, int a_pitch = 0, int a_stride = 0, int c_rows = 0, int c_pitch = 0,
          int split_cols = 0, size_t split_stride = 0, int cls = PC_GEMM_OTHER) {
    ExGemmParams p{};
    p.A = A; p.lda = lda; p.a_rows = a_rows; p.a_pitch = a_pitch; p.a_stride = a_stride;
    p.W = xget(e, prefix + ".weight"); p.ldw = K; p.bias = xget(e, prefix + ".bias");
    if (!p.bias) return fail("exact mode: missing " + prefix);
    p.M = M; p.N = N; p.K = K; p.C = C; p.ldc = ldc; p.c_rows = c_rows; p.c_pitch = c_pitch;
    p.split_cols = split_cols; p.split_stride = split_stride;
    p.R = R; p.ldr = ldc; p.alpha = alpha; p.epi = epi;
    PROF(cls, 2.0 * M * (double)N * K, 4.0 * ((double)M * K + (double)N * K + (double)M * N));
    if (e->exact_split) {
        auto it = e->xsplit.find(prefix);
        if (it != e->xsplit.end()) {
            SxGemmParams q{};
            q.g = p; q.Whi = it->second.hi; q.Wlo = it->second.lo; q.ldh = it->second.ldh;
            const int rc = launch_sx_gemm(q, st);
            if (rc != -2 || !p.W) return rc;
        }
    }
    if (!p.W) return fail("exact mode: missing " + prefix);
    return launch_ex_gemm(p, st);
}

int forward_core_exact(EcEncoder* e, const float* mel, const int64_t* in_len, int from_audio, const Shapes& s, const XWorkspace& w,
                       char* ws, float* out, int64_t* out_len, hipStream_t st) {
    const EcConfig& c = e->cfg;
    const int B = s.B, nb = (int)e->blocks.size();
    if (c.causal) return fail("the label-exact modes have no causal kernels (causal relative tables / depthwise pre-padding): bf16 path only");
    e->trace.clear(); e->trace_used = 0;
    e->e_cache_drop(ws);
    auto F32 = [&](size_t off) { return reinterpret_cast<float*>(ws + off); };
    int* lens = reinterpret_cast<int*>(ws + w.lens);
    EC_TRY(launch_lengths(in_len, B, from_audio, c.hop_length, c.sub_layers, e->block_stride, nb, lens, out_len, st));
    if (from_audio) trace_add(e, st, "mel", mel, (int64_t)B * c.n_mels, s.Tm, s.Tm, 0);
    float* sub = F32(w.sub);
    const int C0 = c.sub_filters[0];
    int Fl = c.n_mels, Cl = C0;
    if (c.sub_layers == 1) {
        EC_TRY(launch_ex_conv2d(mel, B, 1, c.n_mels, s.Tm, xget(e, "subsampling_module.layers.0.0.weight"), e->xsub_scale[0], e->xsub_shift[0], C0, sub, 1, st));
        Fl = (c.n_mels - 1) / 2 + 1;
    } else {
        float* img = F32(w.conv1);
        const int F1 = (c.n_mels - 1) / 2 + 1, T1 = (s.Tm - 1) / 2 + 1, C1 = c.sub_filters[1];
        EC_TRY(launch_ex_conv2d(mel, B, 1, c.n_mels, s.Tm, xget(e, "subsampling_module.layers.0.0.weight"), e->xsub_scale[0], e->xsub_shift[0], C0, img, 0, st));
        EC_TRY(launch_ex_conv2d(img, B, C0, F1, T1, xget(e, "subsampling_module.layers.1.0.weight"), e->xsub_scale[1], e->xsub_shift[1], C1, sub, 1, st));
        Fl = (F1 - 1) / 2 + 1; Cl = C1;
    }
    const int Ksub = Cl * Fl;
    trace_add(e, st, "subsample", sub, (int64_t)B * s.T1, Ksub, Ksub, 0);
    float* x = F32(w.x0);
    float* xalt = F32(w.x1);
    const int D0 = e->blocks[0].dim_model;
    EC_TRY(xgemm(e, st, sub, Ksub, B * s.T1, "linear", D0, Ksub, x, D0));
    trace_add(e, st, "linear", x, (int64_t)B * s.T1, D0, D0, 0);
    float *a = F32(w.a), *hb = F32(w.h), *q = F32(w.q), *kk = F32(w.k), *v = F32(w.v), *eb = F32(w.e), *o = F32(w.o), *p1 = F32(w.p1), *g = F32(w.g),
          *cb = F32(w.c);
    char nm[64];
    int xmask_stride = 1;
    for (int k = 0; k < nb; ++k) {
        const EcBlock& b = e->blocks[k];
        const BlockW& W = e->bw[k];
        const int T = s.Tin[k], To = s.Tout[k], D = b.dim_model, De = b.dim_expand, M = B * T, Mo = B * To;
        const int G = b.group_size, H = b.num_heads, Tp = ec_round_up(T, G), Tg = Tp / G, d = G * D / H;
        const std::string p = "blocks." + std::to_string(k);
        EC_TRY(launch_layernorm(x, M, D, W.ln_ffn1.g, W.ln_ffn1.b, a, nullptr, 0, nullptr, nullptr, st));
        EC_TRY(xgemm(e, st, a, D, M, p + ".feed_forward_module1.layers.1", D * b.ff_ratio, D, hb, D * b.ff_ratio, 1, nullptr, 1.f, 0, 0, 0, 0, 0, 0, 0, PC_GEMM_FFN));
        EC_TRY(xgemm(e, st, hb, D * b.ff_ratio, M, p + ".feed_forward_module1.layers.4", D, D * b.ff_ratio, x, D, 2, x, 0.5f, 0, 0, 0, 0, 0, 0, 0, PC_GEMM_FFN));
        snprintf(nm, sizeof(nm), "blocks.%d.x_ffn1", k); trace_add(e, st, nm, x, M, D, D, 0);
        const std::string m = p + ".multi_head_self_attention_module";
        EC_TRY(launch_layernorm(x, M, D, W.ln_att.g, W.ln_att.b, a, nullptr, 0, nullptr, nullptr, st));
        if (Tp != T) {
            if (hipMemsetAsync(q, 0, (size_t)B * Tp * D * 4, st) != hipSuccess || hipMemsetAsync(kk, 0, (size_t)B * Tp * D * 4, st) != hipSuccess ||
                hipMemsetAsync(v, 0, (size_t)B * Tp * D * 4, st) != hipSuccess) return fail("memset failed");
        }
        if (e->exact_split && e->xsplit.count(m + ".mhsa.qkv_layer")) {
            EC_TRY(xgemm(e, st, a, D, M, m + ".mhsa.qkv_layer", 3 * D, D, q, D, 0, nullptr, 1.f, 0, 0, 0, T, Tp, D, w.qkv_stride));
        } else {
            EC_TRY(xgemm(e, st, a, D, M, m + ".mhsa.query_layer", D, D, q, D, 0, nullptr, 1.f, 0, 0, 0, T, Tp));
            EC_TRY(xgemm(e, st, a, D, M, m + ".mhsa.key_layer", D, D, kk, D, 0, nullptr, 1.f, 0, 0, 0, T, Tp));
            EC_TRY(xgemm(e, st, a, D, M, m + ".mhsa.value_layer", D, D, v, D, 0, nullptr, 1.f, 0, 0, 0, T, Tp));
        }
        if (Tp > b.max_pos) return fail("sequence longer than max_pos_encoding");
        const float* tab = e->xtab[std::make_pair(b.max_pos, D)];
        EC_TRY(xgemm(e, st, tab + (size_t)(b.max_pos - Tp + G / 2) * D, D, 2 * Tp - G, m + ".mhsa.pos_layer", D, D, eb, D));
        ExAttnParams ap{};
        ap.q = q; ap.k = kk; ap.v = v; ap.e = eb; ap.u = W.u; ap.vb = W.v; ap.lens = lens + (size_t)k * B;
        ap.B = B; ap.H = H; ap.T = T; ap.Tp = Tp; ap.G = G; ap.D = D; ap.d = d; ap.Tg = Tg; ap.out = o; ap.variant = e->exact_attention;
        ap.att = (int)e->att_out.size() == nb ? e->att_out[k] : nullptr;
        {
            const long long unit = (long long)xmask_stride * G;
            ap.band_l = (int)std::min<long long>(c.left_context / unit, 1 << 30); ap.band_r = (int)std::min<long long>(c.right_context / unit, 1 << 30);
        }
        { PROF(PC_ATTENTION, 2.0 * B * H * (double)Tg * Tg * d * 3.0, (double)M * D * 4 * 5);
          if (e->exact_split && sx_attention_supported(d) && (long long)B * H <= 65535) EC_TRY(launch_sx_attention(ap, F32(w.scores), st));
          else EC_TRY(launch_ex_attention(ap, st)); }
        EC_TRY(xgemm(e, st, o, D, M, m + ".mhsa.output_layer", D, D, x, D, 2, x, 1.0f, T, Tp, 1));
        snprintf(nm, sizeof(nm), "blocks.%d.x_mhsa", k); trace_add(e, st, nm, x, M, D, D, 0);
        const std::string cm = p + ".convolution_module.layers";
        EC_TRY(launch_layernorm(x, M, D, W.ln_conv.g, W.ln_conv.b, a, nullptr, 0, nullptr, nullptr, st));
        EC_TRY(xgemm(e, st, a, D, M, cm + ".2", 2 * De, D, p1, 2 * De));
        EC_TRY(launch_ex_glu(p1, M, De, g, st));
        EC_TRY(launch_ex_dwconv(g, B, T, To, De, W.dw_w, W.dw_b, b.kernel_size, b.conv_stride, cb, st));
        xmask_stride *= b.conv_stride;
        if (D != De) {
            EC_TRY(xgemm(e, st, x, D, Mo, p + ".conv_res.1", De, D, xalt, De, 0, nullptr, 1.f, To, T, b.conv_stride));
            std::swap(x, xalt);
        } else if (b.conv_stride > 1) {
            return fail("strided block without expansion is not native (no shipped config uses it)");
        }
        EC_TRY(xgemm(e, st, cb, De, Mo, cm + ".7", De, De, x, De, 2, x, 1.0f));
        snprintf(nm, sizeof(nm), "blocks.%d.x_conv", k); trace_add(e, st, nm, x, Mo, De, De, 0);
        EC_TRY(launch_layernorm(x, Mo, De, W.ln_ffn2.g, W.ln_ffn2.b, a, nullptr, 0, nullptr, nullptr, st));
        EC_TRY(xgemm(e, st, a, De, Mo, p + ".feed_forward_module2.layers.1", De * b.ff_ratio, De, hb, De * b.ff_ratio, 1, nullptr, 1.f, 0, 0, 0, 0, 0, 0, 0, PC_GEMM_FFN));
        EC_TRY(xgemm(e, st, hb, De * b.ff_ratio, Mo, p + ".feed_forward_module2.layers.4", De, De * b.ff_ratio, x, De, 2, x, 0.5f, 0, 0, 0, 0, 0, 0, 0, PC_GEMM_FFN));
        float* xo = (k == nb - 1) ? out : xalt;
        EC_TRY(launch_layernorm(x, Mo, De, W.ln_out.g, W.ln_out.b, xo, nullptr, 0, nullptr, nullptr, st));
        if (k != nb - 1) std::swap(x, xalt);
        snprintf(nm, sizeof(nm), "blocks.%d.out", k); trace_add(e, st, nm, xo, Mo, De, De, 0);
    }
// ... 762 lines not shown
                    for (int n = 0; n < D; ++n) b2h[n] = 0.5f * b2->data[n];
                    e->bw[k].xf_img[which] = upload(e, img); e->bw[k].xf_b2[which] = upload(e, b2h); e->bw[k].xf_nch[which] = nch;
                }
            {
                auto perm16 = [](int pos) { const int khh = pos >> 3, ee = pos & 7; return 8 * (ee >> 2) + 4 * khh + (ee & 3); };
                bool over = false;
                auto put = [&](std::vector<uint16_t>& img, size_t hi_at, size_t lo_at, double wv) {
                    const float ws = (float)(wv * 1024.0);
                    if (!(std::fabs(ws) < kSplitImgMax)) { over = true; return; }
                    const _Float16 hh = (_Float16)ws;
                    img[hi_at] = half_bits((float)hh);
                    img[lo_at] = half_bits(ws - (float)hh);
                };
                auto f1_chunk = [&](std::vector<uint16_t>& img, size_t base, int DP1, int K, const float* const* wrow, const float* bias, const float* g, const float* beta) {
                    for (int r = 0; r < 32; ++r) {
                        if (!wrow[r]) continue;
                        double bsum = bias[r];
                        for (int col = 0; col < DP1; ++col) {
                            const int f = (col & ~15) + perm16(col & 15);
                            if (f < K) {
                                const double wv = wrow[r][f];
                                if (beta) bsum += wv * beta[f];
                                put(img, base + (size_t)r * DP1 + col, base + (size_t)32 * DP1 + (size_t)r * DP1 + col, g ? wv * g[f] : wv);
                            }
                        }
                        for (int col = 0; col < DP1; ++col)
                            if ((col & ~15) + perm16(col & 15) == K) put(img, base + (size_t)r * DP1 + col, base + (size_t)32 * DP1 + (size_t)r * DP1 + col, bsum);
                    }
                };
                auto f2_chunk = [&](std::vector<uint16_t>& img, size_t base, int DP2, int c, const float* Wm, int N, int K, int ldw, double scale) {
                    for (int n = 0; n < N; ++n)
                        for (int pos = 0; pos < 32; ++pos) {
                            const int kk = 32 * c + (pos & ~15) + perm16(pos & 15);
                            if (kk < K) put(img, base + (size_t)n * 32 + pos, base + (size_t)32 * DP2 + (size_t)n * 32 + pos, scale * Wm[(size_t)n * ldw + kk]);
                        }
                };
                auto padded = [&](const std::vector<float>& v, int n, float scale) { std::vector<float> o(n, 0.f); for (size_t i = 0; i < v.size() && (int)i < n; ++i) o[i] = scale * v[i]; return o; };
                for (size_t k = 0; k < e->blocks.size(); ++k) {
                    const EcBlock& b = e->blocks[k];
                    BlockW& W = e->bw[k];
                    const int D = b.dim_model, De = b.dim_expand;
                    const std::string pb = "blocks." + std::to_string(k);
                    const std::string mh = pb + ".multi_head_self_attention_module.", cm = pb + ".convolution_module.layers.";
                    auto ffn_image = [&](int which, int Dw) -> const uint16_t* {
                        const int F = Dw * b.ff_ratio;
                        const std::string pf = pb + (which ? ".feed_forward_module2.layers." : ".feed_forward_module1.layers.");
                        const HostTensor *g = find(e, pf + "0.weight"), *bt = find(e, pf + "0.bias"), *w1 = find(e, pf + "1.weight"), *b1 = find(e, pf + "1.bias"),
                                         *w2 = find(e, pf + "4.weight");
                        if (!g || !bt || !w1 || !b1 || !w2 || (int64_t)w1->data.size() != (int64_t)F * Dw || (int64_t)w2->data.size() != (int64_t)F * Dw ||
                            (int)g->data.size() != Dw || (int)bt->data.size() != Dw || (int)b1->data.size() != F || !W.xf_b2[which]) return nullptr;
                        int ks, nt; sxf_ffn_shape(Dw, &ks, &nt);
                        const int DP1 = 16 * ks, DP2 = 32 * nt, nch = (F + 31) / 32;
                        const size_t per = (size_t)64 * (DP1 + DP2);
                        std::vector<uint16_t> img((size_t)nch * per, 0);
                        for (int c = 0; c < nch; ++c) {
                            const float* rows[32]; float bias[32];
                            for (int r = 0; r < 32; ++r) { const int h = 32 * c + r; rows[r] = h < F ? w1->data.data() + (size_t)h * Dw : nullptr; bias[r] = h < F ? b1->data[h] : 0.f; }
                            f1_chunk(img, (size_t)c * per, DP1, Dw, rows, bias, g->data.data(), bt->data.data());
                            f2_chunk(img, (size_t)c * per + (size_t)64 * DP1, DP2, c, w2->data.data(), Dw, F, F, 0.5);
                        }
                        return over ? nullptr : upload(e, img);
                    };
                    if (sxc_supported(D) && sxf_ffn_supported(D)) {
                        int ks, nt; sxf_ffn_shape(D, &ks, &nt);
                        const int DP1 = 16 * ks, DP2 = 32 * nt, nte = (De + 31) / 32;
                        const HostTensor *wo = find(e, mh + "mhsa.output_layer.weight"), *bo = find(e, mh + "mhsa.output_layer.bias"), *lg = find(e, cm + "0.weight"), *lb = find(e, cm + "0.bias"),
                                         *w1 = find(e, cm + "2.weight"), *b1 = find(e, cm + "2.bias"), *ag = find(e, mh + "norm.weight"), *ab = find(e, mh + "norm.bias");
                        const HostTensor *wq[3] = {find(e, mh + "mhsa.query_layer.weight"), find(e, mh + "mhsa.key_layer.weight"), find(e, mh + "mhsa.value_layer.weight")};
                        const HostTensor *bq[3] = {find(e, mh + "mhsa.query_layer.bias"), find(e, mh + "mhsa.key_layer.bias"), find(e, mh + "mhsa.value_layer.bias")};
                        bool ok = wo && bo && lg && lb && w1 && b1 && ag && ab && (int)wo->data.size() == D * D && (int)bo->data.size() == D && (int)lg->data.size() == D && (int)lb->data.size() == D &&
                                  (int64_t)w1->data.size() == (int64_t)2 * De * D && (int)b1->data.size() == 2 * De && (int)ag->data.size() == D && (int)ab->data.size() == D;
                        for (int i = 0; i < 3; ++i) ok = ok && wq[i] && bq[i] && (int)wq[i]->data.size() == D * D && (int)bq[i]->data.size() == D;
                        if (ok) {
                            over = false;
                            std::vector<uint16_t> io((size_t)nt * 64 * DP2, 0);
                            for (int c = 0; c < nt; ++c) f2_chunk(io, (size_t)c * 64 * DP2, DP2, c, wo->data.data(), D, D, D, 1.0);
                            std::vector<uint16_t> ip((size_t)2 * nte * 64 * DP1, 0);
                            for (int c = 0; c < 2 * nte; ++c) {
                                const float* rows[32]; float bias[32];
                                for (int r = 0; r < 32; ++r) { const int f = 32 * (c >> 1) + r, n = (c & 1) * De + f; rows[r] = f < De ? w1->data.data() + (size_t)n * D : nullptr; bias[r] = f < De ? b1->data[n] : 0.f; }
                                f1_chunk(ip, (size_t)c * 64 * DP1, DP1, D, rows, bias, lg->data.data(), lb->data.data());
                            }
                            std::vector<uint16_t> iq((size_t)3 * nt * 64 * DP1, 0);
                            for (int c = 0; c < 3 * nt; ++c) {
                                const int which = c / nt, cc = c % nt;
                                const float* rows[32]; float bias[32];
                                for (int r = 0; r < 32; ++r) { const int n = 32 * cc + r; rows[r] = n < D ? wq[which]->data.data() + (size_t)n * D : nullptr; bias[r] = n < D ? bq[which]->data[n] : 0.f; }
                                f1_chunk(iq, (size_t)c * 64 * DP1, DP1, D, rows, bias, ag->data.data(), ab->data.data());
                            }
                            if (!over) {
                            W.xc_wo = upload(e, io); W.xc_bo = upload(e, padded(bo->data, DP2, 1.f)); W.xc_p1 = upload(e, ip); W.xc_nch_p1 = 2 * nte; W.xc_qkv = upload(e, iq);
                            W.xc_f[0] = ffn_image(0, D);
                            W.xc_in = W.xc_f[0] != nullptr;
                            }
                        }
                    }
                    if (sxc_supported(De) && sxf_ffn_supported(De)) {
                        int ks, nt; sxf_ffn_shape(De, &ks, &nt);
                        const int DP2 = 32 * nt;
                        const HostTensor *w2 = find(e, cm + "7.weight"), *b2 = find(e, cm + "7.bias");
                        if (w2 && b2 && (int64_t)w2->data.size() == (int64_t)De * De && (int)b2->data.size() == De) {
                            over = false;
                            std::vector<uint16_t> i2((size_t)nt * 64 * DP2, 0);
                            for (int c = 0; c < nt; ++c) f2_chunk(i2, (size_t)c * 64 * DP2, DP2, c, w2->data.data(), De, De, De, 1.0);
                            if (!over) {
                                W.xc_p2 = upload(e, i2); W.xc_bp2 = upload(e, padded(b2->data, DP2, 1.f));
                                W.xc_f[1] = ffn_image(1, De);
                                W.xc_out = W.xc_f[1] != nullptr;
                            }
                        }
                    }
                }
            }
        }
        for (const EcBlock& b : e->blocks) {
            auto key = std::make_pair(b.max_pos, b.dim_model);
            if (e->xtab.count(key)) continue;
            const int rows = 2 * b.max_pos - 1, D = b.dim_model;
            std::vector<float> t((size_t)rows * D, 0.f), denom(D / 2);
            for (int i = 0; i < D / 2; ++i) denom[i] = std::pow(10000.0f, (2.0f * (float)i) / (float)D);
            for (int r = 0; r < rows; ++r) {
                const float pos = (float)(b.max_pos - 1 - r);
                for (int i = 0; i < D / 2; ++i) { const float a = pos / denom[i]; t[(size_t)r * D + 2 * i] = std::sin(a); t[(size_t)r * D + 2 * i + 1] = std::cos(a); }
            }
            e->xtab[key] = upload(e, t);
        }
    }
    for (void* p : e->allocs) if (!p) return fail("device allocation failed");
    if (hipDeviceSynchronize() != hipSuccess) return fail("upload failed");
    e->host.clear();
    e->e_cache.clear();
    {
        int dmax = 0;
        for (const EcBlock& b : e->blocks) dmax = std::max(dmax, std::max(b.dim_model, b.dim_expand));
        e->tiled_auto_on = dmax > e->tiled_min_k && dmax <= 384;
    }
    e->finalized = true;
    return 0;
}

size_t effconf_encoder_workspace_bytes(const EcEncoder* e, int32_t batch, int32_t n, int32_t from_audio) {
    if (!e || batch <= 0 || n <= 0) return 0;
    const int Tm = from_audio ? n / e->cfg.hop_length + 1 : n;
    const Shapes s = make_shapes(e, batch, Tm);
    size_t bytes = make_workspace(e, s, from_audio != 0).total;
    if (e->exact_pack) bytes = std::max(bytes, make_xworkspace(e, s).total + (from_audio ? al((size_t)batch * e->cfg.n_mels * Tm * 4) : 0));
    return bytes;
}

int32_t effconf_encoder_out_frames(const EcEncoder* e, int32_t n, int32_t from_audio) {
    if (!e || n <= 0) return 0;
    const int Tm = from_audio ? n / e->cfg.hop_length + 1 : n;
    return make_shapes(e, 1, Tm).Tout.back();
}

int effconf_encoder_forward_mel(EcEncoder* e, const float* mel, const int64_t* mel_len, int32_t batch, int32_t n_frames,
                                float* out, int64_t* out_len, void* workspace, size_t workspace_bytes, void* stream) {
    if (!e || !e->finalized) return fail("encoder not finalized");
    if (!mel || !mel_len || !out || !workspace || batch <= 0 || n_frames <= 0) return fail("bad argument");
    const Shapes s = make_shapes(e, batch, n_frames);
    if (e->exact_on) {
        const XWorkspace xw = make_xworkspace(e, s);
        if (workspace_bytes < xw.total) return fail("workspace too small");
        if (split_fused_ok(e) && e->att_out.empty())
            return forward_core_split(e, mel, mel_len, 0, s, xw, reinterpret_cast<char*>(workspace), out, out_len, (hipStream_t)stream);
        return forward_core_exact(e, mel, mel_len, 0, s, xw, reinterpret_cast<char*>(workspace), out, out_len, (hipStream_t)stream);
    }
    const Workspace w = make_workspace(e, s, false);
    if (workspace_bytes < w.total) return fail("workspace too small");
    return forward_core(e, mel, mel_len, 0, s, w, reinterpret_cast<char*>(workspace), out, out_len, (hipStream_t)stream);
}

int effconf_encoder_forward(EcEncoder* e, const float* audio, const int64_t* x_len, int32_t batch, int32_t n_samples,
                            float* out, int64_t* out_len, void* workspace, size_t workspace_bytes, void* stream) {
    if (!e || !e->finalized) return fail("encoder not finalized");
    if (!audio || !x_len || !out || !workspace || batch <= 0 || n_samples <= e->cfg.n_fft / 2) return fail("bad argument");
    const int Tm = n_samples / e->cfg.hop_length + 1;
    const Shapes s = make_shapes(e, batch, Tm);
    if (e->exact_on) {
        const XWorkspace xw = make_xworkspace(e, s);
        if (workspace_bytes < xw.total + al((size_t)batch * e->cfg.n_mels * Tm * 4)) return fail("workspace too small");
        char* ws = reinterpret_cast<char*>(workspace);
        float* mel = reinterpret_cast<float*>(ws + xw.total);
        hipStream_t st = (hipStream_t)stream;
        { PROF(PC_MEL, 0, (double)batch * n_samples * 4 + (double)batch * e->cfg.n_mels * Tm * 4);
          EC_TRY(launch_mel(audio, batch, n_samples, e->mel, e->cfg.n_fft, e->cfg.hop_length, e->cfg.n_mels, Tm, e->cfg.normalize, e->cfg.mean, e->cfg.std, mel, st)); }
        if (split_fused_ok(e) && e->att_out.empty()) return forward_core_split(e, mel, x_len, 1, s, xw, ws, out, out_len, st);
        return forward_core_exact(e, mel, x_len, 1, s, xw, ws, out, out_len, st);
    }
    const Workspace w = make_workspace(e, s, true);
    if (workspace_bytes < w.total) return fail("workspace too small");
    char* ws = reinterpret_cast<char*>(workspace);
    float* mel = reinterpret_cast<float*>(ws + w.mel);
    hipStream_t st = (hipStream_t)stream;
    { PROF(PC_MEL, 0, (double)batch * n_samples * 4 + (double)batch * e->cfg.n_mels * Tm * 4); EC_TRY(launch_mel(audio, batch, n_samples, e->mel, e->cfg.n_fft, e->cfg.hop_length, e->cfg.n_mels, Tm,
                      e->cfg.normalize, e->cfg.mean, e->cfg.std, mel, st)); }
    return forward_core(e, mel, x_len, 1, s, w, ws, out, out_len, st);
}

static bool ragged_host_lengths(const EcEncoder* e, const int64_t* host_len, int32_t batch, int32_t n, int32_t from_audio, std::vector<int>* tm) {
    tm->resize(batch);
    for (int b = 0; b < batch; ++b) {
        const int64_t l = host_len[b];
        if (l > n || (from_audio ? l <= e->cfg.n_fft / 2 : l < 1)) return false;
        (*tm)[b] = from_audio ? (int)(l / e->cfg.hop_length + 1) : (int)l;
    }
    return true;
}

size_t effconf_encoder_workspace_bytes_ragged(const EcEncoder* e, const int64_t* x_len_host, int32_t batch, int32_t n, int32_t from_audio) {
    if (!e || !x_len_host || batch <= 0 || n <= 0) return 0;
    std::vector<int> tm;
    if (!ragged_host_lengths(e, x_len_host, batch, n, from_audio, &tm)) return 0;
    const Shapes s = make_shapes_ragged(e, tm);
    Shapes full = s; full.Tm = from_audio ? n / e->cfg.hop_length + 1 : n;
    size_t bytes = make_workspace(e, full, from_audio != 0).total;
    if (e->exact_pack) bytes = std::max(bytes, make_xworkspace(e, full).total + (from_audio ? al((size_t)batch * e->cfg.n_mels * full.Tm * 4) : 0));
    return bytes;
}

int effconf_encoder_forward_ragged(EcEncoder* e, const float* x, const int64_t* x_len, const int64_t* x_len_host, int32_t batch, int32_t n,
                                   int32_t from_audio, float* out, int32_t out_frames, int64_t* out_len, void* workspace, size_t workspace_bytes,
                                   void* stream) {
    if (!e || !e->finalized) return fail("encoder not finalized");
    if (e->exact_on && !split_fused_ok(e))
        return fail("ragged batches run on the bf16 path and in the split mode (exact_fp32 = 2, head widths <= 144); exact_fp32 = 1 keeps rectangular batches");
    if (e->exact_on && !e->att_out.empty()) return fail("attention maps of a ragged batch: bf16 path only");
    if (!x || !x_len || !x_len_host || !out || !workspace || batch <= 0 || n <= 0 || out_frames <= 0) return fail("bad argument");
    std::vector<int> tm;
    if (!ragged_host_lengths(e, x_len_host, batch, n, from_audio, &tm)) return fail("ragged lengths out of range (audio: n_fft / 2 < len <= n; mel: 1 <= len <= n)");
    Shapes s = make_shapes_ragged(e, tm);
    if (s.Tout.back() > out_frames) return fail("out_frames smaller than the longest utterance's output");
    s.Tm = from_audio ? n / e->cfg.hop_length + 1 : n;
    if (e->exact_on) {
        const XWorkspace xw = make_xworkspace(e, s);
        if (workspace_bytes < xw.total + (from_audio ? al((size_t)batch * e->cfg.n_mels * s.Tm * 4) : 0)) return fail("workspace too small");
        char* wsx = reinterpret_cast<char*>(workspace);
        hipStream_t stx = (hipStream_t)stream;
        const float* melx = x;
        if (from_audio) {
            float* m = reinterpret_cast<float*>(wsx + xw.total);
            hipStream_t st = stx;
            PROF(PC_MEL, 0, (double)batch * n * 4 + (double)batch * e->cfg.n_mels * s.Tm * 4);
            EC_TRY(launch_mel(x, batch, n, e->mel, e->cfg.n_fft, e->cfg.hop_length, e->cfg.n_mels, s.Tm, e->cfg.normalize, e->cfg.mean, e->cfg.std, m, st, x_len));
            melx = m;
        }
        return forward_core_split(e, melx, x_len, from_audio, s, xw, wsx, out, out_len, stx, out_frames);
    }
    const Workspace w = make_workspace(e, s, from_audio != 0);
    if (workspace_bytes < w.total) return fail("workspace too small");
    char* ws = reinterpret_cast<char*>(workspace);
    hipStream_t st = (hipStream_t)stream;
    const float* mel = x;
    if (from_audio) {
        float* m = reinterpret_cast<float*>(ws + w.mel);
        PROF(PC_MEL, 0, (double)batch * n * 4 + (double)batch * e->cfg.n_mels * s.Tm * 4);
        EC_ABL(16, EC_TRY(launch_mel(x, batch, n, e->mel, e->cfg.n_fft, e->cfg.hop_length, e->cfg.n_mels, s.Tm, e->cfg.normalize, e->cfg.mean, e->cfg.std, m, st, x_len)));
        mel = m;
    }
    return forward_core(e, mel, x_len, from_audio, s, w, ws, out, out_len, st, out_frames);
}

int effconf_mel_frontend(EcEncoder* e, const float* audio, int32_t batch, int32_t n_samples, float* mel, void* stream) {
    if (!e || !e->finalized) return fail("encoder not finalized");
    if (!audio || !mel) return fail("mel_frontend: null argument");
    if (batch > 0 && n_samples <= e->cfg.n_fft / 2) return fail("mel_frontend: n_samples must exceed n_fft / 2 (reflect padding)");
    const int Tm = n_samples / e->cfg.hop_length + 1;
    EC_TRY(launch_mel(audio, batch, n_samples, e->mel, e->cfg.n_fft, e->cfg.hop_length, e->cfg.n_mels, Tm,
                      e->cfg.normalize, e->cfg.mean, e->cfg.std, mel, (hipStream_t)stream));
    return 0;
}

#ifdef EFFCONF_DEBUG_ABI
int effconf_debug_mel(EcEncoder* e, int32_t variant, int32_t extra_lds, const float* audio, int32_t batch, int32_t n_samples, float* mel,
                      uint32_t* counters, void* stream) {
    if (!e || !e->finalized) return fail("encoder not finalized");
    const int Tm = n_samples / e->cfg.hop_length + 1;
    EC_TRY(launch_mel_debug(variant, extra_lds, audio, batch, n_samples, e->mel, e->cfg.n_fft, e->cfg.hop_length, e->cfg.n_mels, Tm,
                            e->cfg.normalize, e->cfg.mean, e->cfg.std, mel, counters, (hipStream_t)stream));
    return 0;
}

int effconf_debug_neighbour(int32_t kind, int32_t blocks, int32_t lds_bytes, int32_t iters, float* buf, size_t n_floats, void* stream) {
    EC_TRY(launch_debug_neighbour(kind, blocks, lds_bytes, iters, buf, n_floats, (hipStream_t)stream));
    return 0;
}

#endif

int effconf_relpos_attention(const uint16_t* qu, const uint16_t* k, const uint16_t* v, const uint16_t* e, const float* dvu, int32_t dvu_ld,
                             const int32_t* lens, int32_t batch, int32_t heads, int32_t frames, int32_t group, int32_t dim, uint16_t* out,
                             int32_t ld_out, int32_t variant, void* stream) {
    if (!qu || !k || !v || !e || !dvu || !lens || !out) return fail("null argument");
    if (batch <= 0 || heads <= 0 || frames <= 0 || group <= 0 || !(group & 1) || dim <= 0 || (group * dim) % heads) return fail("bad attention shape");
    AttnParams ap{};
    const int Tp = ec_round_up(frames, group), Tg = Tp / group, d = group * dim / heads, dpad = ec_round_up(d, 32);
    if (dpad > 192 || dvu_ld < dpad || ld_out < dim) return fail("unsupported head width / leading dimension");
    ap.qu = qu; ap.kh = k; ap.vt = v; ap.eh = e; ap.dvu = dvu; ap.dvu_ld = dvu_ld; ap.lens = lens;
    ap.B = batch; ap.H = heads; ap.T = frames; ap.G = group; ap.D = dim; ap.d = d; ap.dpad = dpad; ap.Tg = Tg; ap.Tgp = ec_round_up(Tg, 8);
    ap.q_bstride = (long long)Tp * dim; ap.q_hstride = d; ap.q_rowstride = group * dim; ap.e_hstride = d; ap.e_rowstride = group * dim;
    ap.out = out; ap.ldo = ld_out; ap.scale = 1.0f / std::sqrt((float)d);
    ap.band_l = ap.band_r = 1 << 30;
    if (variant == 0) { EC_TRY(launch_relpos_attention(ap, (hipStream_t)stream)); return 0; }
    if ((variant != 1 && variant != 2) || !relpos_attention2_supported(dpad)) return fail("attention variant not available for this head width");
    EC_TRY(launch_relpos_attention2(ap, variant, (hipStream_t)stream));
    return 0;
}

size_t effconf_module_workspace_bytes(const EcEncoder* e, int32_t batch, int32_t frames) {
    if (!e || batch <= 0 || frames <= 0) return 0;
    size_t mx = 0;
    for (const EcBlock& b : e->blocks) {
        const size_t D = (size_t)std::max(b.dim_model, b.dim_expand);
        mx = std::max(mx, D * ((size_t)b.ff_ratio + 4) * 2 + 64);
    }
    const size_t rows = (size_t)batch * frames;
    size_t sub = 0;
    {
        const int L = e->cfg.sub_layers, C = e->cfg.sub_filters[L - 1];
        int F = e->cfg.n_mels; for (int i = 0; i < L; ++i) F /= 2;
        const size_t t1 = (frames - 1) / 2 + 1;
        sub = al((size_t)batch * t1 * C * F * 2) + (L == 2 ? al((size_t)batch * (e->cfg.n_mels / 2) * t1 * ec_round_up(e->cfg.sub_filters[0], 64) * 2) : 0);
    }
    return std::max(al(rows * mx) + 4 * 256, sub + 256);
}

int effconf_ffn(EcEncoder* e, int32_t block, int32_t which, const float* x, int32_t rows, float* y, void* workspace, size_t workspace_bytes,
                void* stream) {
    if (!e || !e->finalized) return fail("encoder not finalized");
    if (block < 0 || block >= (int)e->blocks.size() || (which != 1 && which != 2) || !x || !y || rows <= 0 || !workspace) return fail("bad argument");
    const EcBlock& b = e->blocks[block];
    const BlockW& W = e->bw[block];
    const int D = which == 1 ? b.dim_model : b.dim_expand, F = D * b.ff_ratio;
    hipStream_t st = (hipStream_t)stream;
    char* ws = reinterpret_cast<char*>(workspace);
    const size_t a_bytes = al((size_t)rows * ld8(D) * 2), h_bytes = al((size_t)rows * F * 2);
    if (workspace_bytes < a_bytes + h_bytes) return fail("workspace too small");
    bf16_t* a = reinterpret_cast<bf16_t*>(ws);
    bf16_t* hbuf = reinterpret_cast<bf16_t*>(ws + a_bytes);
    if (y != x && hipMemcpyAsync(y, x, (size_t)rows * D * 4, hipMemcpyDeviceToDevice, st) != hipSuccess) return fail("copy failed");
    const LNp& ln = which == 1 ? W.ln_ffn1 : W.ln_ffn2;
    const PackedLinear &L1 = which == 1 ? W.ffn1_a : W.ffn2_a, &L2 = which == 1 ? W.ffn1_b : W.ffn2_b;
    const bf16_t* w2p = which == 1 ? W.ffn1_bp : W.ffn2_bp;
    if (ffn_fused_supported(D)) return run_ffn(e, st, a, rows, D, L1, L2, w2p, y, hbuf, &ln);
    EC_TRY(launch_layernorm(y, rows, D, ln.g, ln.b, nullptr, a, ld8(D), nullptr, nullptr, st));
    return run_ffn(e, st, a, rows, D, L1, L2, w2p, y, hbuf);
}

int effconf_conv_module(EcEncoder* e, int32_t block, const float* x, int32_t batch, int32_t frames, float* y, void* workspace,
                        size_t workspace_bytes, void* stream) {
    if (!e || !e->finalized) return fail("encoder not finalized");
    if (block < 0 || block >= (int)e->blocks.size() || !x || !y || batch <= 0 || frames <= 0 || !workspace) return fail("bad argument");
    const EcBlock& b = e->blocks[block];
    const BlockW& W = e->bw[block];
    const int D = b.dim_model, De = b.dim_expand, T = frames, To = (T - 1) / b.conv_stride + 1, M = batch * T, Mo = batch * To;
    hipStream_t st = (hipStream_t)stream;
    char* ws = reinterpret_cast<char*>(workspace);
    const size_t a_bytes = al((size_t)M * ld8(D) * 2), g_bytes = al((size_t)M * ld8(De) * 2), c_bytes = al((size_t)Mo * ld8(De) * 2);
    if (workspace_bytes < a_bytes + g_bytes + c_bytes) return fail("workspace too small");
    bf16_t* a = reinterpret_cast<bf16_t*>(ws);
    bf16_t* gbuf = reinterpret_cast<bf16_t*>(ws + a_bytes);
    bf16_t* cbuf = reinterpret_cast<bf16_t*>(ws + a_bytes + g_bytes);
    if (rs_gemm_supported(D)) {
        EC_TRY(run_rs_or_tiled(e, PC_GEMM_OTHER, st, a, ld8(D), M, W.pw1, 2, EPI_GLU_BF16, gbuf, ld8(De), nullptr, 0, 1.f, x, &W.ln_conv));
    } else {
        EC_TRY(launch_layernorm(x, M, D, W.ln_conv.g, W.ln_conv.b, nullptr, a, ld8(D), nullptr, nullptr, st));
        EC_TRY(run_rs_or_tiled(e, PC_GEMM_OTHER, st, a, ld8(D), M, W.pw1, 2, EPI_GLU_BF16, gbuf, ld8(De)));
    }
    EC_TRY(launch_dwconv(gbuf, batch, T, To, De, ld8(De), W.dw_w, W.dw_b, b.kernel_size, b.conv_stride, cbuf, st, nullptr, e->cfg.causal, dw_mfma_table(e, W.dw_a, b.kernel_size), W.dw_a3));
    return run_rs_or_tiled(e, PC_GEMM_OTHER, st, cbuf, ld8(De), Mo, W.pw2, 1, EPI_F32, y, De);
}

int effconf_subsample(EcEncoder* e, const float* mel, int32_t batch, int32_t n_frames, float* y, void* workspace, size_t workspace_bytes,
                      void* stream) {
    if (!e || !e->finalized) return fail("encoder not finalized");
    if (!mel || !y || batch <= 0 || n_frames <= 0 || !workspace) return fail("bad argument");
    const Shapes s = make_shapes(e, batch, n_frames);
    const int L = e->cfg.sub_layers, C = e->cfg.sub_filters[L - 1];
    int F = e->cfg.n_mels; for (int i = 0; i < L; ++i) F /= 2;
    const size_t sub_bytes = al((size_t)batch * s.T1 * C * F * 2);
    const size_t tl1 = (n_frames - 1) / 2 + 1;
    const size_t act_bytes = L == 2 ? al((size_t)batch * (e->cfg.n_mels / 2) * tl1 * ec_round_up(e->cfg.sub_filters[0], 64) * 2) : 0;
    if (workspace_bytes < sub_bytes + act_bytes) return fail("workspace too small");
    char* ws = reinterpret_cast<char*>(workspace);
    return run_subsample_linear(e, (hipStream_t)stream, mel, batch, n_frames, s.T1, reinterpret_cast<bf16_t*>(ws), reinterpret_cast<bf16_t*>(ws + sub_bytes), y);
}

int effconf_layernorm_residual(EcEncoder* e, int32_t block, int32_t which, const float* x, const float* r, float alpha, int32_t rows, float* y,
                               void* stream) {
    if (!e || !e->finalized) return fail("encoder not finalized");
    if (block < 0 || block >= (int)e->blocks.size() || which < 0 || which > 4 || !x || !y || rows <= 0) return fail("bad argument");
    const EcBlock& b = e->blocks[block];
    const BlockW& W = e->bw[block];
    const LNp* ln[5] = {&W.ln_ffn1, &W.ln_att, &W.ln_conv, &W.ln_ffn2, &W.ln_out};
    const int D = which >= 3 ? b.dim_expand : b.dim_model;
    EC_TRY(launch_layernorm_residual(x, r, alpha, rows, D, ln[which]->g, ln[which]->b, y, (hipStream_t)stream));
    return 0;
}

#ifdef EFFCONF_DEBUG_ABI
int effconf_debug_gemm(const uint16_t* a, int32_t lda, const uint16_t* w, int32_t ldw, const float* bias, int32_t m, int32_t n, int32_t k,
                       int32_t epi, int32_t wide, void* c, int32_t ldc, const float* r, int32_t ldr, float alpha, void* stream) {
    if (!a || !w || !bias || !c) return fail("null argument");
    if (epi < EPI_F32 || epi > EPI_GLU_BF16 || (epi == EPI_RESID_F32 && !r)) return fail("epilogue: 0 f32, 1 bf16, 2 swish bf16, 3 residual f32, 4 GLU bf16");
    if (wide < 0 || wide > 3) return fail("wide: 0 .. 3");
    GemmParams p{};
    p.A = a; p.lda = lda; p.W = w; p.ldw = ldw; p.bias = bias; p.M = m; p.N = n; p.K = k;
    p.C = c; p.ldc = ldc; p.R = r; p.ldr = ldr; p.alpha = alpha; p.wide = wide;
    if (wide >= 2 && !gemm256_supported(p, epi)) return fail("gemm256 does not take this shape / alignment");
    EC_TRY(launch_gemm(p, epi, (hipStream_t)stream));
    return 0;
}

int effconf_debug_sx_gemm(const float* a, int32_t lda, const uint16_t* w_hi, const uint16_t* w_lo, int32_t ldh, const float* bias, int32_t m, int32_t n,
                          int32_t k, int32_t epi, float* c, int32_t ldc, const float* r, int32_t ldr, float alpha, void* stream) {
    SxGemmParams q{};
    q.g.A = a; q.g.lda = lda; q.g.bias = bias; q.g.M = m; q.g.N = n; q.g.K = k; q.g.C = c; q.g.ldc = ldc; q.g.R = r; q.g.ldr = ldr; q.g.alpha = alpha; q.g.epi = epi;
    q.Whi = w_hi; q.Wlo = w_lo; q.ldh = ldh;
    const int rc = launch_sx_gemm(q, reinterpret_cast<hipStream_t>(stream));
    return rc ? fail("sx_gemm launch failed rc=" + std::to_string(rc)) : 0;
}

int effconf_debug_pack_dwconv_mfma(const float* w_kc, int32_t ksize, int32_t channels, uint16_t* dst, size_t dst_elems) {
    if (!w_kc || !dst || channels <= 0) return fail("null argument");
    if (!dwconv_mfma_supported(ksize, 1)) return fail("kernel size: 15, 31 or 7");
    if (dst_elems != (size_t)channels * 4 * dwconv_mfma_groups(ksize) * 8) return fail("dst: channels * 4 * groups * 8 bf16");
    pack_dwconv_mfma(w_kc, ksize, channels, dst);
    return 0;
}

int effconf_debug_dwconv(const uint16_t* g, int32_t batch, int32_t frames, int32_t channels, int32_t ld, const float* w_kc_host, const float* bias_host,
                         int32_t ksize, int32_t stride, int32_t use_mfma, int32_t causal, uint16_t* out, void* stream) {
    if (!g || !w_kc_host || !bias_host || !out || batch <= 0 || frames <= 0 || channels <= 0 || ld < channels || ld % 8) return fail("bad argument");
    if (use_mfma && !dwconv_mfma_supported(ksize, stride)) return fail("dwconv_mfma_kernel: stride 1, kernel size 15, 31 or 7");
    hipStream_t st = reinterpret_cast<hipStream_t>(stream);
    float *dw = nullptr, *db = nullptr; uint16_t* dt = nullptr;
    std::vector<uint16_t> tab;
    if (use_mfma) { tab.resize((size_t)channels * 4 * dwconv_mfma_groups(ksize) * 8); pack_dwconv_mfma(w_kc_host, ksize, channels, tab.data()); }
    if (hipMalloc(&dw, (size_t)ksize * channels * 4) != hipSuccess || hipMalloc(&db, (size_t)channels * 4) != hipSuccess ||
        (use_mfma && hipMalloc(&dt, tab.size() * 2) != hipSuccess)) return fail("hipMalloc failed");
    (void)hipMemcpy(dw, w_kc_host, (size_t)ksize * channels * 4, hipMemcpyHostToDevice);
    (void)hipMemcpy(db, bias_host, (size_t)channels * 4, hipMemcpyHostToDevice);
    if (use_mfma) (void)hipMemcpy(dt, tab.data(), tab.size() * 2, hipMemcpyHostToDevice);
    const int to = (frames - 1) / stride + 1;
    const int rc = launch_dwconv(g, batch, frames, to, channels, ld, dw, db, ksize, stride, out, st, nullptr, causal, use_mfma ? dt : nullptr);
    (void)hipStreamSynchronize(st);
    (void)hipFree(dw); (void)hipFree(db); if (dt) (void)hipFree(dt);
    return rc ? fail("launch_dwconv failed rc=" + std::to_string(rc)) : 0;
}

int effconf_debug_sxf_ffn(EcEncoder* e, int32_t block, int32_t which, const float* x, int32_t rows, float* y, int32_t with_norm, int32_t ablate, void* stream) {
    if (!e || !e->finalized || block < 0 || block >= (int)e->blocks.size() || which < 1 || which > 2 || !x || !y || rows <= 0) return fail("bad argument");
    const BlockW& W = e->bw[block];
    if (!W.xf_img[which - 1]) return fail("no fused split FFN image for this block (finalize with exact_fp32 = 2; width not built, or a folded weight beyond the image's range)");
    SxfFfnParams fp{};
    const int D = which == 2 ? e->blocks[block].dim_expand : e->blocks[block].dim_model;
    fp.X = x; fp.ldx = D; fp.Y = y; fp.ldy = D; fp.wimg = W.xf_img[which - 1]; fp.b2 = W.xf_b2[which - 1]; fp.M = rows; fp.D = D; fp.nchunk = W.xf_nch[which - 1];
    if (with_norm) { fp.ln_g = W.ln_out.g; fp.ln_b = W.ln_out.b; }
    fp.ablate = ablate;
    EC_TRY(launch_sxf_ffn(fp, reinterpret_cast<hipStream_t>(stream)));
    return 0;
}

int effconf_debug_spin(double microseconds, void* stream) {
    if (launch_debug_spin(microseconds, reinterpret_cast<hipStream_t>(stream)) != 0) return fail("spin launch failed");
    return 0;
}

int effconf_debug_lds_fill(int32_t mode, int32_t blocks, int32_t waves, const void* src, size_t window, int32_t kib_per_wave, int32_t passes, uint64_t* out, void* stream) {
    EC_TRY(launch_debug_lds_fill(mode, blocks, waves, reinterpret_cast<const char*>(src), window, kib_per_wave, passes, reinterpret_cast<unsigned long long*>(out), (hipStream_t)stream));
    return 0;
}

int effconf_debug_victim(int32_t kind, int32_t blocks, int32_t iters, float* out, void* stream) {
    EC_TRY(launch_debug_victim(kind, blocks, iters, out, (hipStream_t)stream));
    return 0;
}

#endif

int effconf_ctc_greedy(EcEncoder* e, const float* enc_out, const int64_t* out_len, int32_t batch, int32_t t_out,
                       int32_t* labels, int32_t* label_len, float* logits, void* workspace, size_t workspace_bytes, void* stream) {
    if (!e || !e->finalized) return fail("encoder not finalized");
    if (!e->fc_wt) return fail("no CTC head (fc.weight / fc.bias) loaded");
    if (workspace_bytes < (size_t)batch * t_out * 4) return fail("workspace too small");
    int* preds = reinterpret_cast<int*>(workspace);
    hipStream_t st = (hipStream_t)stream;
    const int mode = e->exact_on && e->ctc_mfma == 2 ? 1 : e->ctc_mfma;
    if (mode == 2 && e->fc_hi && launch_ctc_split(enc_out, batch * t_out, e->blocks.back().dim_expand, e->fc_hi, e->fc_lo, e->fc_b, e->cfg.vocab_size,
                                                  preds, logits, st) == 0) {
    } else
    EC_TRY(launch_ctc_argmax(enc_out, batch * t_out, e->blocks.back().dim_expand, e->fc_wt, e->fc_b, e->cfg.vocab_size,
                             preds, logits, st, mode != 0));
    EC_TRY(launch_ctc_collapse(preds, out_len, batch, t_out, labels, label_len, st));
    return 0;
}

int effconf_ctc_greedy_bf16(EcEncoder* e, const uint16_t* enc_out_bf16, const int64_t* out_len, int32_t batch, int32_t t_out,
                            int32_t* labels, int32_t* label_len, float* logits, void* workspace, size_t workspace_bytes, void* stream) {
    if (!e || !e->finalized) return fail("encoder not finalized");
    if (e->exact_on) return fail("effconf_ctc_greedy_bf16 belongs to the bf16 path (the label-exact modes keep fp32 rows and the fp32 head)");
    if (!e->fc_hi || !e->fc_lo) return fail("no CTC head (fc.weight / fc.bias) loaded");
    if (workspace_bytes < (size_t)batch * t_out * 4) return fail("workspace too small");
    int* preds = reinterpret_cast<int*>(workspace);
    hipStream_t st = (hipStream_t)stream;
    EC_TRY(launch_ctc_split(reinterpret_cast<const float*>(enc_out_bf16), batch * t_out, e->blocks.back().dim_expand, e->fc_hi, e->fc_lo, e->fc_b,
                            e->cfg.vocab_size, preds, logits, st, 1));
    EC_TRY(launch_ctc_collapse(preds, out_len, batch, t_out, labels, label_len, st));
    return 0;
}

int effconf_encoder_attention_dims(EcEncoder* e, int32_t n, int32_t from_audio, int32_t* heads, int32_t* tg) {
    if (!e || !e->finalized || !heads || !tg) return fail("effconf_encoder_attention_dims: null argument / encoder not finalized");
    if (n < 0) return fail("effconf_encoder_attention_dims: negative length");
    const Shapes s = make_shapes(e, 1, from_audio ? n / e->cfg.hop_length + 1 : n);
    for (size_t k = 0; k < e->blocks.size(); ++k) {
        const EcBlock& b = e->blocks[k];
        heads[k] = b.num_heads;
        tg[k] = ec_round_up(s.Tin[k], b.group_size) / b.group_size;
    }
    return 0;
}

int effconf_encoder_set_attention_outputs(EcEncoder* e, float* const* maps, int32_t n_blocks) {
    if (!e) return fail("null encoder");
    if (!maps || n_blocks == 0) { e->att_out.clear(); return 0; }
    if (n_blocks != (int)e->blocks.size()) return fail("effconf_encoder_set_attention_outputs: one pointer per block (null = skip that block)");
    e->att_out.assign(maps, maps + n_blocks);
    return 0;
}

int effconf_encoder_set_option(EcEncoder* e, const char* name, int32_t value) {
    if (!e || !name) return fail("null argument");
    if (!strcmp(name, "fuse_subsample")) { if (value < 0 || value > 3) return fail("fuse_subsample: 0, 1, 2 or 3"); e->fuse_subsample = value; return 0; }
    if (!strcmp(name, "fuse_chain")) { e->fuse_chain = value != 0; return 0; }
    if (!strcmp(name, "ctc_mfma")) { if (value < 0 || value > 2) return fail("ctc_mfma: 0 (VALU), 1 (fp32 MFMA) or 2 (split-bf16 MFMA)"); e->ctc_mfma = value; return 0; }
    if (!strcmp(name, "wide_gemm")) { if (value < 0 || (value > 3 && value < 16)) return fail("wide_gemm: 0 (by shape), 1 (never), 2 (256-column tile), 3 (128-column tile), >= 16 (by shape with this many 256 x 256 tiles as the threshold)"); e->wide_gemm = value; return 0; }
    if (!strcmp(name, "attention_v2")) { if (value != 0 && value != 1 && value != 2) return fail("attention_v2: 0, 1 or 2"); e->attention_v2 = value; return 0; }
    if (!strcmp(name, "chain_full_max")) { if (value < 0 || value > 256) return fail("chain_full_max: widest stage (0..256) that runs chain A as ONE kernel"); e->chain_full_max = value; return 0; }
    if (!strcmp(name, "chain_max_dim")) { e->chain_max_dim = value; return 0; }
    if (!strcmp(name, "chain_small_m")) { e->chain_small_m = value; return 0; }
    if (!strcmp(name, "chain_pair")) { if (value != 0 && value != 5) return fail("chain_pair: 0 (chain.hip everywhere) or 5 (chain3.hip for chain A, chain2.hip for chain B at padded width 256)"); e->chain_pair = value; return 0; }
    if (!strcmp(name, "dwconv_mfma")) { if (value < 0 || value > 2) return fail("dwconv_mfma: 0, 1 (kernel size 15) or 2 (15 / 31 / 7)"); e->dwconv_mfma = value; return 0; }
    if (!strcmp(name, "tiled_min_k")) { e->tiled_min_k = value; return 0; }
    if (!strcmp(name, "tiled_auto")) { e->tiled_auto = value; return 0; }
    if (!strcmp(name, "head_major_odd")) { e->head_major_odd = value != 0; return 0; }
    if (!strcmp(name, "split_ffn")) { e->split_ffn = value != 0; return 0; }
    if (!strcmp(name, "split_sublin")) { e->split_sublin = value != 0; return 0; }
    if (!strcmp(name, "sub3_auto")) { e->sub3_auto = value != 0; return 0; }
    if (!strcmp(name, "split_chain")) { e->split_chain = value != 0; return 0; }
    if (!strcmp(name, "exact_attention")) { if (value < 0 || value > 2) return fail("exact_attention: 0 (tiled), 2 (tiled, 16-row workgroups) or 1 (one wave per query row)"); e->exact_attention = value; return 0; }
    if (!strcmp(name, "cache_pos_embeddings")) { e->e_cache_on = value != 0; e->e_cache.clear(); return 0; }
    if (!strcmp(name, "exact_fp32")) {
        if (!e->finalized) { e->exact_pack = e->exact_on = value != 0; e->exact_split = value == 2; return 0; }
        if (value && !e->exact_pack) return fail("exact_fp32 must be requested before effconf_encoder_finalize (the fp32 weights are uploaded there)");
        if (value == 2 && e->xsplit.empty()) return fail("exact_fp32 = 2 must be requested before effconf_encoder_finalize (the split weight images are built there)");
        e->exact_on = value != 0; e->exact_split = value == 2;
        return 0;
    }
    return fail(std::string("unknown option ") + name);
}

int effconf_profile_enable(EcEncoder* e, int32_t enable) {
    if (!e) return fail("null encoder");
    e->prof_on = enable != 0; e->prof_next = 0; e->prof_rec.clear();
    return 0;
}

int effconf_profile_read(EcEncoder* e, int32_t cls, double* total_ms, int64_t* launches, double* flops, double* bytes) {
    if (!e || cls < 0 || cls >= PC_COUNT) return fail("bad profile class");
    if (hipDeviceSynchronize() != hipSuccess) return fail("sync failed");
    double ms = 0, fl = 0, by = 0; int64_t n = 0;
    for (size_t i = 0; i < e->prof_rec.size(); ++i) {
        if (e->prof_rec[i].cls != cls) continue;
        float t = 0.f;
        if (hipEventElapsedTime(&t, e->prof_ev[2 * i], e->prof_ev[2 * i + 1]) != hipSuccess) return fail("event read failed");
        ms += t; fl += e->prof_rec[i].flops; by += e->prof_rec[i].bytes; ++n;
    }
    *total_ms = ms; *launches = n; *flops = fl; *bytes = by;
    return 0;
}

int effconf_encoder_set_trace(EcEncoder* e, void* dev_arena, size_t bytes) {
    if (!e) return fail("null encoder");
    e->trace_arena = reinterpret_cast<char*>(dev_arena); e->trace_bytes = bytes; e->trace_used = 0; e->trace.clear();
    return 0;
}
int32_t effconf_encoder_trace_count(const EcEncoder* e) { return e ? (int32_t)e->trace.size() : 0; }
int effconf_encoder_trace_entry(const EcEncoder* e, int32_t i, char* name64, int64_t* offset, int64_t* rows, int64_t* cols,
                                int64_t* ld, int32_t* dtype) {
    if (!e || i < 0 || i >= (int)e->trace.size()) return fail("bad trace index");
    const TraceEntry& t = e->trace[i];
    memcpy(name64, t.name, 64);
    *offset = t.offset; *rows = t.rows; *cols = t.cols; *ld = t.ld; *dtype = t.dtype;
    return 0;
}

}
```

efficientconformer_amd/csrc/kernels.h:

```cpp
#pragma once
#include "common.h"

struct RaggedRows {
    const int* off;
    const int* len;
    int n;
    int rows;
    int tmax;
};

struct RaggedConv {
    const int *in_off, *in_len, *out_off, *out_len;
    const int* tile_off; int tiles;
    int n, out_rows;
};

enum GemmEpilogue {
    EPI_F32 = 0,
    EPI_BF16 = 1,
    EPI_SWISH_BF16 = 2,
    EPI_RESID_F32 = 3,
    EPI_GLU_BF16 = 4,
    EPI_QKV = 5,
    EPI_HEADS = 6,
    EPI_QKV_NAT = 7,
};

struct GemmParams {
    const bf16_t* A; int lda;
    int a_rows, a_pitch, a_stride;
    const bf16_t* W; int ldw;
    const float* bias;
    int M, N, K;
    void* C; int ldc;
    const float* R; int ldr; float alpha;
    int T, G, H, D, d, dpad, Tg, Tgp;
    bf16_t *qu, *kh, *vt;
    const float *u, *v;
    const float* X; int ldx; const float *ln_g, *ln_b;
    int wide;
};
int launch_gemm(const GemmParams& p, int epi, hipStream_t s);
bool gemm256_supported(const GemmParams& p, int epi);
int launch_gemm256(const GemmParams& p, int epi, int bn, hipStream_t s);

struct FfnParams {
    const bf16_t* A; int lda;
    const float* X; int ldx;
    float* Y; int ldy;
    const bf16_t* W1; int ldw1; const float* b1;
    const bf16_t* W2; int ldw2; const float* b2;
    int M, D, Fp;
    float alpha;
    const float *ln_g, *ln_b;
};
bool rs_gemm_supported(int K);
bool rs_gemm_resident_supported(int K, int N);
int launch_rs_gemm(const GemmParams& p, int epi, hipStream_t s);
bool ffn_fused_supported(int D);
int launch_ffn_fused(const FfnParams& p, hipStream_t s);


struct ChainGemm { const bf16_t* w; int ldw; const float* bias; int nchunks; };
struct ChainFfn { const bf16_t* w1; int ldw1; const float* b1; const bf16_t* w2; int ldw2; const float* b2; int Fp; const bf16_t* w2cm; };
struct ChainLn { const float* g; const float* b; };
struct ChainParams {
    int M, D;
    const float* X; int ldx;
    float* Y; int ldy;
    const bf16_t* A; int lda;
    ChainGemm g0;
    ChainLn ln[4];
    ChainFfn f[2];
    ChainGemm g1;
    bf16_t *qu, *kh, *vt; const float *u, *v; int T, Tp;
    bf16_t* glu; int ldg, Ng;
    const float* consts;
    int small_m;
    int pair;
};
enum { CHAIN_B = 0, CHAIN_A_FULL = 1, CHAIN_A_HEAD = 2, CHAIN_A_TAIL = 3 };
bool chain_supported(int D);
int chain_padded_width(int D);
int chain_const_layout(const ChainParams& p, int kind, int (&nf)[8]);
bool chain_head_supported(int D);
bool chain_tail_supported(int D);
bool chain_full_supported(int D, int dmax = 192);
int launch_chain(const ChainParams& p, int kind, hipStream_t s);
int launch_chain2(const ChainParams& p, hipStream_t s);
bool chain3_supported(int D);
int launch_chain3(const ChainParams& p, int kind, hipStream_t s);

int launch_layernorm(const float* x, int M, int D, const float* gamma, const float* beta,
                     float* out_f32, bf16_t* out_bf16, int ld_bf16,
                     const float* gamma2, const float* beta2, hipStream_t s);
int launch_layernorm_residual(const float* x, const float* r, float alpha, int M, int D, const float* gamma, const float* beta, float* y, hipStream_t s);
int launch_cast_rows(const float* x, int D, int rows_per_batch, int stride, int out_rows_per_batch, int batch,
                     bf16_t* out, int ld_out, hipStream_t s, const RaggedConv* rc = nullptr);
int launch_emit_rows(const float* x, int D, const int* off, const int* len, int batch, int t_out, float* out, hipStream_t s);

struct AttnParams {
    const bf16_t *qu, *kh, *vt, *eh;
    const float* dvu; int dvu_ld;
    long long q_bstride, q_hstride, e_hstride; int q_rowstride, e_rowstride;
    const int* lens;
    int B, H, T, G, D, d, dpad, Tg, Tgp;
    bf16_t* out; int ldo;
    float scale;
    const int *rag_off, *rag_wg; int rag_nwg, rag_tgmax;
    int band_l, band_r, causal;
    int ablate;
};
int launch_relpos_attention(const AttnParams& p, hipStream_t s);
int launch_attention_probs(const AttnParams& p, float* att, hipStream_t s);
bool relpos_attention2_supported(int dpad);
int launch_relpos_attention2(const AttnParams& p, int waves, hipStream_t s);
int launch_attn_pad_rows(const GemmParams& p, int B, hipStream_t s);
int launch_attn_pad_rows_nat(const GemmParams& p, int B, hipStream_t s);
int launch_attn_pad_rows_ragged(bf16_t* qu, bf16_t* kh, bf16_t* vt, const float* u, int D, int G, const RaggedRows& rg, hipStream_t s);

int launch_subsample_conv(const float* mel, int B, int F, int Tm, int T1, const float* w9, const float* bias, int C,
                          bf16_t* out, int ldo, hipStream_t s, const int* rag_tm = nullptr, const RaggedRows* rg = nullptr);
int launch_gather_rows(const float* x, int D, int t_pitch, const RaggedRows& rg, float* out, hipStream_t s);
bool sublinear_fused_supported(int F, int N);
int launch_sublinear_fused(const float* mel, int B, int F, int Tm, int T1, const float* w9, const float* cbias, int C,
                           const bf16_t* W, int ldw, const float* bias, int N, float* out, int ldc, hipStream_t s);
int sublinear2_groups(int F, int C, int N);
int launch_sublinear2(const float* mel, int B, int F, int Tm, int T1, const float* ctab, const bf16_t* Wp, const float* bias, int C, int N,
                      float* out, int ldc, hipStream_t s, const RaggedRows* rg = nullptr, const int* rag_tm = nullptr);
int launch_subsample_conv_cl(const float* mel, int B, int F, int Tm, int T1, const float* w9, const float* bias, int C, int Cp,
                             bf16_t* out, hipStream_t s, const int* rag_tm = nullptr);
int launch_conv2_igemm(const bf16_t* act1, int B, int F1, int T1, int Cp, const bf16_t* W, int ldw, const float* bias,
                       int N, int F2, int T2, bf16_t* out, hipStream_t s);
int launch_dwconv(const bf16_t* g, int B, int T, int To, int C, int ld, const float* w_kc, const float* bias,
                  int ksize, int stride, bf16_t* out, hipStream_t s, const RaggedConv* rc = nullptr, int causal = 0,
                  const void* w_mfma = nullptr,
                  const void* w_mfma3 = nullptr);
int dwconv_mfma_groups(int ksize);
bool dwconv_mfma_supported(int ksize, int stride);
void pack_dwconv_mfma3(const float* w_kc, int ksize, int C, uint16_t* dst);
void pack_dwconv_mfma(const float* w_kc, int ksize, int C, uint16_t* dst);

struct ExGemmParams {
    const float* A; int lda;
    int a_rows, a_pitch, a_stride;
    const float* W; int ldw;
    const float* bias;
    int M, N, K;
    float* C; int ldc;
    int c_rows, c_pitch;
    int split_cols; size_t split_stride;
    const float* R; int ldr; float alpha;
    int epi;
};
int launch_ex_gemm(const ExGemmParams& p, hipStream_t s);
int launch_ex_conv2d(const float* in, int B, int Cin, int F, int T, const float* w, const float* scale, const float* shift, int Co,
                     float* out, int flat, hipStream_t s, const int* tlen = nullptr);
int launch_ex_glu(const float* in, long long M, int N, float* out, hipStream_t s);
int launch_ex_dwconv(const float* g, int B, int T, int To, int C, const float* w_kc, const float* bias, int ks, int stride, float* out, hipStream_t s);
struct ExAttnParams {
    const float *q, *k, *v, *e, *u, *vb;
    const int* lens;
    int B, H, T, Tp, G, D, d, Tg;
    float* out;
    float* att;
    int variant;
    int band_l, band_r;
};
int launch_ex_attention(const ExAttnParams& p, hipStream_t s);

struct SxGemmParams {
    ExGemmParams g;
    const uint16_t *Whi, *Wlo; int ldh;
};
int launch_sx_gemm(const SxGemmParams& p, hipStream_t s);
struct SxAttnParams { ExAttnParams a; float* scores; int TgP; };
bool sx_attention_supported(int d);
size_t sx_attention_scores_bytes(int B, int H, int Tg);
int launch_sx_attention(const ExAttnParams& p, float* scores, hipStream_t s);

struct SxfAttnParams {
    const float *q, *k, *v;
    const uint16_t *kp, *vp, *ep;
    int vpitch;
    const float* u;
    const int* lens;
    const int* off;
    int B, H, G, D, d;
    int T, Tp, Tg;
    float* out;
    int band_l, band_r, causal;
};
bool sxf_attention_supported(int d);
int sxf_attention_pk(int d);
int sxf_attention_vx(int d);
int launch_sxf_pack_kv(const SxfAttnParams& p, hipStream_t s);
int launch_sxf_pack_e(const float* e, const float* u, const float* vb, int erows_grouped, int H, int G, int D, int d, uint16_t* ep, hipStream_t s);
int launch_sxf_attention(const SxfAttnParams& p, hipStream_t s);
struct SxfFfnParams {
    const float* X; int ldx;
    float* Y; int ldy;
    const uint16_t* wimg;
    const float* b2;
    const float *ln_g, *ln_b;
    int M, D, nchunk;
    int ablate;
};
struct SubLin3Params {
    const float* mel; int B, F, Tm;
    const int* mel_len;
    const int* off;
    const int* len;
    int To;
    int rows_max;
    const uint16_t* cimg;
    const uint16_t* wimg;
    const float* bias;
    float* y; int ldy, N;
    int ncb, Fo;
};
int sublinear3_tiles(int N);
int launch_sublinear3(const SubLin3Params& p, hipStream_t s);
struct SxfSubParams {
    const float* mel; int B, F, Tm;
    const int* mel_len;
    const int* off;
    const int* len;
    int To;
    int rows_max;
    const uint16_t* cimg;
    const uint16_t* wimg;
    const float* bias;
    float* y; int N;
    int ncb, Fo;
};
int sxf_sublin_tiles(int N);
int launch_sxf_sublin(const SxfSubParams& p, hipStream_t s);
void sxf_ffn_shape(int D, int* ks1, int* nt2);
bool sxf_ffn_supported(int D);
size_t sxf_ffn_image_halfs(int D, int F);
int launch_sxf_ffn(const SxfFfnParams& p, hipStream_t s);
struct SxcBParams {
    const float* o; int o_rows, o_pitch;
    float* x;
    float* g;
    int M, D, De;
    const uint16_t* w_o; const float* b_o;
    const uint16_t* w_p1; int nch_p1;
};
struct SxcAParams {
    int tail, head;
    const float* c;
    const float* xres;
    float* y;
    int M, D;
    const uint16_t* w_p2; const float* b_p2;
    const uint16_t* w_f2; int nch_f2; const float* b_f2;
    const float *ln_g, *ln_b;
    const uint16_t* w_f1; int nch_f1; const float* b_f1;
    const uint16_t* w_qkv;
    float* q; size_t qkv_stride;
    size_t qkv_bytes;
    int q_rows, q_pitch;
};
bool sxc_supported(int D);
int launch_sxc_b(const SxcBParams& p, hipStream_t s);
int launch_sxc_a(const SxcAParams& p, hipStream_t s);
int launch_sxf_dwconv(const float* g, int B, int T, int To, int C, const float* w_kc, const float* bias, int ks, int stride, float* out, hipStream_t s,
                      const RaggedConv* rc = nullptr, int causal = 0, int tcap_max = 0);
int launch_sxf_decimate(const float* x, int D, int stride, const RaggedConv& rc, float* out, hipStream_t s);
int launch_sxf_glu(const float* in, long long M, int N, float* out, hipStream_t s);

struct MelTables {
    const float* window;
    const float2* twiddle;
    const int* fb_start;
    const int* fb_count;
    const int* fb_offset;
    const float* fb_weight;
    int fb_nnz;
};
int launch_mel(const float* audio, int B, int L, const MelTables& t, int n_fft, int hop, int n_mels, int Tm,
               int normalize, float mean, float std, float* mel, hipStream_t s, const int64_t* ragged_len = nullptr);
int launch_mel_debug(int variant, int extra_lds, const float* audio, int B, int L, const MelTables& t, int n_fft, int hop, int n_mels,
                     int Tm, int normalize, float mean, float std, float* mel, unsigned int* dbg, hipStream_t s);
int launch_debug_neighbour(int kind, int blocks, int lds_bytes, int iters, float* buf, size_t n, hipStream_t s);
int launch_debug_spin(double microseconds, hipStream_t s);
int launch_debug_lds_fill(int mode, int blocks, int waves, const char* src, size_t window, int kib_per_wave, int passes, unsigned long long* out, hipStream_t s);
int launch_debug_victim(int kind, int blocks, int iters, float* out, hipStream_t s);
int launch_mel_debug_pk(int variant, int extra_lds, const float* audio, int B, int L, const MelTables& t, int n_fft, int hop, int n_mels,
                          int Tm, int normalize, float mean, float std, float* mel, unsigned int* dbg, hipStream_t s);

int launch_lengths(const int64_t* x_len, int B, int from_audio, int hop, int sub_layers, const int* block_stride,
                   int n_blocks, int* stage_lens , int64_t* out_len, hipStream_t s);
int launch_lengths_ragged(const int64_t* x_len, int B, int from_audio, int hop, int sub_layers, const int* block_stride, const int* group,
                          const int* heads, int n_blocks, int* stage_lens, int* mel_len, int* row_off, int* wg_off, int* tile_off,
                          int64_t* out_len, hipStream_t s);
int launch_ctc_argmax(const float* x, int M, int D, const float* Wt, const float* bias, int V,
                      int* preds, float* logits_or_null, hipStream_t s, int use_mfma = 1);
int launch_ctc_split(const float* x, int M, int D, const bf16_t* Whi, const bf16_t* Wlo, const float* bias, int V, int* preds, float* logits_or_null,
                     hipStream_t s, int x_is_bf16 = 0);
int launch_ctc_collapse(const int* preds, const int64_t* lens, int B, int T, int* labels, int* label_len, hipStream_t s);
```

Baseline: 59.51 million mel-frames/s (valid, 10 ms hop).

## Make relpos attention2 kernel persistent with next-tile prefetch overlapping epilogue

Adds a persistent variant of the relative-position attention kernel that launches one workgroup per occupancy slot and loops over work items in a serpentine order across XCD-partitioned ranges. While finishing one tile's epilogue it looks up the next item and issues its K/V/E and Q head loads, hiding load latency and removing per-workgroup launch and setup cost. It is enabled by default through a new attention_persist option. In exchange it adds register pressure from the prefetched state, a heavier per-item setup path, and possible load imbalance across the fixed slot count.

```diff
diff --git a/efficientconformer_amd/csrc/attention2.hip b/efficientconformer_amd/csrc/attention2.hip
--- a/efficientconformer_amd/csrc/attention2.hip
+++ b/efficientconformer_amd/csrc/attention2.hip
@@ -50,7 +50,15 @@
     static constexpr int TOTAL = K_BYTES + V_BYTES + E_BYTES + S_BYTES;
 };
 
-template <int DP, int NWV, int QT, int SETS = 0>
+struct Attn2Raw { int b, h, qt, len; size_t row0; };
+struct Attn2Item {
+    int Tg, T, h, i0, nkv, band_l, band_r, kbeg, nkeys, R0, erows;
+    bool banded, tile_dead;
+    size_t orow0;
+    const bf16_t *Qu, *Kh, *Vh, *Eh;
+};
+
+template <int DP, int NWV, int QT, int SETS = 0, bool PERS = false>
 __global__ __launch_bounds__(NWV * 64, (QT == 1 && NWV == 4 && DP <= 96) ? ((DP <= 64 && SETS == 1) ? 3 : 2) : 1) void relpos_attention2_kernel(const AttnParams p) {
     using SM = Attn2Smem<DP, NWV, QT>;
     constexpr int KS = DP / 32, DT = DP / 16, BI = SM::BI, NTHR = NWV * 64, CPR = DP / 8, ERING = SM::ERING;
@@ -60,51 +68,67 @@
     char* sE = sV + SM::V_BYTES;
     float* sS = reinterpret_cast<float*>(sE + SM::E_BYTES);
 
-    const int tid = threadIdx.x, lane = tid & 63, wave = tid >> 6;
+    const int tid = threadIdx.x, lane = tid & 63;
+    const int wave = __builtin_amdgcn_readfirstlane(tid >> 6);
     const int c = lane & 15, g = lane >> 4;
-    int qtiles = (p.Tg + BI - 1) / BI;
-    int id = xcd_remap(blockIdx.x, gridDim.x);
-    int Tg = p.Tg, T = p.T, qt_wg, h, b;
-    {
-        const int per_b = p.H * qtiles, q8 = p.B >> 3, r8 = p.B & 7;
-        const int u = p.rag_off ? ((ABLATE(p) & 8) ? (id * p.B) / (int)gridDim.x : ragged_find_wave(p.rag_wg, p.B, id)) : id / per_b;
+    auto item_tid = [&]() __attribute__((always_inline)) {
+        if constexpr (!PERS) return (int)threadIdx.x;
+        else {
+            int t = (int)__builtin_amdgcn_mbcnt_hi(~0u, __builtin_amdgcn_mbcnt_lo(~0u, 0u)) + 64 * wave;
+            asm volatile("" : "+v"(t));
+            return t;
+        }
+    };
+    typedef const __attribute__((address_space(4))) AttnParams* KernArgs;
+    KernArgs P = (KernArgs)__builtin_amdgcn_kernarg_segment_ptr();
+    const int qtiles0 = (p.Tg + BI - 1) / BI;
+    const int nwg = p.rag_off ? p.rag_nwg : p.B * p.H * qtiles0;
+    const int RS = p.q_rowstride, ERS = p.e_rowstride;
+    const int dceil = (p.d + 7) & ~7;
+    const bool ragged_d = dceil != p.d;
+
+    auto lookup = [&](int id) __attribute__((always_inline)) {
+        Attn2Raw r;
+        const int per_b = P->H * qtiles0, q8 = P->B >> 3, r8 = P->B & 7;
+        const int u = P->rag_off ? ((ABLATE(p) & 8) ? (id * P->B) / nwg : ragged_find_wave(P->rag_wg, P->B, id)) : id / per_b;
         int x, j;
         if (u < r8 * (q8 + 1)) { x = u / (q8 + 1); j = u - x * (q8 + 1); }
         else { const int u2 = u - r8 * (q8 + 1); x = u2 / q8; j = u2 - x * q8; x += r8; }
-        b = x + 8 * j;
-        int local = id - (p.rag_off ? ((ABLATE(p) & 8) ? id : p.rag_wg[u]) : u * per_b);
-        if (p.rag_off) { T = p.lens[b]; Tg = (T + p.G - 1) / p.G; qtiles = (Tg + BI - 1) / BI; }
-        qt_wg = local % qtiles; h = local / qtiles;
-    }
-    if (ABLATE(p) & 128) return;
-    const int i0 = qt_wg * BI, iw0 = i0 + wave * 16 * QT;
-    const size_t orow0 = p.rag_off ? (size_t)p.rag_off[b] : (size_t)b * p.T;
-    const size_t qoff = (p.rag_off ? orow0 * p.D : (size_t)b * p.q_bstride) + (size_t)h * p.q_hstride;
-    const bf16_t* Qu = p.qu + qoff;
-    const bf16_t* Kh = p.kh + qoff;
-    const bf16_t* Vh = p.vt + qoff;
-    const int RS = p.q_rowstride, ERS = p.e_rowstride;
-    const bf16_t* Eh = p.eh + (size_t)h * p.e_hstride + (p.rag_off ? (size_t)(p.rag_tgmax - Tg) * ERS : 0);
-    const int erows = p.causal ? Tg : 2 * Tg - 1;
-    const int dceil = (p.d + 7) & ~7;
-    const bool ragged_d = dceil != p.d;
-
-    int nkv = (p.lens[b] + p.G - 1) / p.G;
-    nkv = nkv < Tg ? nkv : Tg;
-    const int band_l = p.band_l < Tg ? p.band_l : Tg, band_r = p.band_r < Tg ? p.band_r : Tg;
-    const bool banded = band_l < Tg || band_r < Tg;
-    const bool tile_dead = nkv < 1 || i0 + BI - 1 - band_l >= nkv;
-    int kbeg = 0, nkeys = nkv;
-    if (tile_dead) nkeys = Tg;
-    else if (banded) {
-        kbeg = i0 - band_l; kbeg = kbeg < 0 ? 0 : kbeg & ~(BJ - 1);
-        const int ke = i0 + BI + band_r;
-        nkeys = ke < nkv ? ke : nkv;
-    }
-
-    const int R0 = Tg - 1 - i0 - (BI - 1) + kbeg;
-    constexpr int NB = ((BI + 63) * CPR + NTHR - 1) / NTHR;
-    uint4 fb[NB];
+        r.b = x + 8 * j;
+        const int local = id - (P->rag_off ? ((ABLATE(p) & 8) ? id : P->rag_wg[u]) : u * per_b);
+        r.len = P->lens[r.b];
+        int qt = qtiles0;
+        if (P->rag_off) { const int tg = (r.len + P->G - 1) / P->G; qt = (tg + BI - 1) / BI; }
+        r.qt = local % qt; r.h = local / qt;
+        r.row0 = P->rag_off ? (size_t)P->rag_off[r.b] : (size_t)r.b * P->T;
+        return r;
+    };
+    auto derive = [&](const Attn2Raw& r) __attribute__((always_inline)) {
+        Attn2Item it;
+        it.h = r.h; it.Tg = P->Tg; it.T = P->T;
+        if (P->rag_off) { it.T = r.len; it.Tg = (it.T + P->G - 1) / P->G; }
+        it.i0 = r.qt * BI;
+        it.orow0 = r.row0;
+        const size_t qoff = (P->rag_off ? r.row0 * P->D : (size_t)r.b * P->q_bstride) + (size_t)r.h * P->q_hstride;
+        it.Qu = P->qu + qoff; it.Kh = P->kh + qoff; it.Vh = P->vt + qoff;
+        it.Eh = P->eh + (size_t)r.h * P->e_hstride + (P->rag_off ? (size_t)(P->rag_tgmax - it.Tg) * ERS : 0);
+        it.erows = P->causal ? it.Tg : 2 * it.Tg - 1;
+        int nkv = (r.len + P->G - 1) / P->G;
+        it.nkv = nkv < it.Tg ? nkv : it.Tg;
+        it.band_l = P->band_l < it.Tg ? P->band_l : it.Tg; it.band_r = P->band_r < it.Tg ? P->band_r : it.Tg;
+        it.banded = it.band_l < it.Tg || it.band_r < it.Tg;
+        it.tile_dead = it.nkv < 1 || it.i0 + BI - 1 - it.band_l >= it.nkv;
+        it.kbeg = 0; it.nkeys = it.nkv;
+        if (it.tile_dead) it.nkeys = it.Tg;
+        else if (it.banded) {
+            int kb = it.i0 - it.band_l; it.kbeg = kb < 0 ? 0 : kb & ~(BJ - 1);
+            const int ke = it.i0 + BI + it.band_r;
+            it.nkeys = ke < it.nkv ? ke : it.nkv;
+        }
+        it.R0 = it.Tg - 1 - it.i0 - (BI - 1) + it.kbeg;
+        return it;
+    };
+
     constexpr int NK = (BJ * CPR + NTHR - 1) / NTHR;
     struct Stage { uint4 lk[NK], lv[NK], le[NK]; };
     Stage sa, sb;
@@ -124,90 +148,6 @@
         const int r = q / CPR, x = (q - r * CPR) * 8, xc = x < dceil ? x : 0;
         koffs[n] = (uint32_t)(r * RS + xc) * 2u;
     }
-    auto issue_loads = [&](Stage& st_, int jn) __attribute__((always_inline)) {
-        if (((ABLATE(p) & 2) && jn > kbeg) || (ABLATE(p) & 64)) return;
-        if (jn + BJ <= Tg - (ragged_d ? 1 : 0)) {
-            const char* kb = reinterpret_cast<const char*>(Kh + (size_t)jn * RS);
-            const char* vb = reinterpret_cast<const char*>(Vh + (size_t)jn * RS);
-#pragma unroll
-            for (int n = 0; n < NK; ++n) { st_.lk[n] = ld16b(kb + koffs[n]); st_.lv[n] = ld16b(vb + koffs[n]); }
-        } else {
-#pragma unroll
-            for (int n = 0; n < NK; ++n) {
-                const int kr = chunk_row(n), j = jn + kr;
-                const size_t o = (size_t)(j < Tg ? j : Tg - 1) * RS * 2 + (koffs[n] - (uint32_t)(kr * RS) * 2u);
-                st_.lk[n] = tail_mask(ld16b(reinterpret_cast<const char*>(Kh) + o), n); st_.lv[n] = tail_mask(ld16b(reinterpret_cast<const char*>(Vh) + o), n);
-            }
-        }
-        if (jn > kbeg) {
-            const int rnew = R0 + (jn - kbeg) + BI - 1;
-            if (rnew >= 0 && rnew + 63 < erows - (ragged_d ? 1 : 0)) {
-                const char* eb = reinterpret_cast<const char*>(Eh + (size_t)rnew * ERS);
-#pragma unroll
-                for (int n = 0; n < NK; ++n) st_.le[n] = ld16b(eb + koffs[n]);
-            } else {
-#pragma unroll
-                for (int n = 0; n < NK; ++n) {
-                    const int er = chunk_row(n);
-                    int r = rnew + er;
-                    r = r < 0 ? 0 : (r >= erows ? erows - 1 : r);
-                    st_.le[n] = tail_mask(ld16b(reinterpret_cast<const char*>(Eh) + (size_t)r * ERS * 2 + (koffs[n] - (uint32_t)(er * RS) * 2u)), n);
-                }
-            }
-        }
-    };
-    issue_loads(sa, kbeg);
-#pragma unroll
-    for (int n = 0; n < NB; ++n) {
-        const int q = tid + NTHR * n;
-        const int rr = q / CPR, x = (q - rr * CPR) * 8;
-        const int r = R0 + (rr < BI + 63 ? rr : BI + 62);
-        const int rc = r < 0 ? 0 : (r >= erows ? erows - 1 : r);
-        fb[n] = (ABLATE(p) & 16) ? make_uint4(0, 0, 0, 0) : ld16(Eh + (size_t)rc * ERS + (x < dceil ? x : 0));
-    }
-    bf16x8 qu[QT][KS], qv[QT][KS];
-    {
-        const float* dv = p.dvu + (size_t)h * p.dvu_ld;
-#pragma unroll
-        for (int t = 0; t < QT; ++t) {
-            const int i = iw0 + 16 * t + c, ic = i < Tg ? i : Tg - 1;
-            uint4 ra[KS];
-#pragma unroll
-            for (int ks = 0; ks < KS; ++ks) {
-                const int x = ks * 32 + g * 8;
-                ra[ks] = (ABLATE(p) & 32) ? make_uint4(0, 0, 0, 0) : ld16(Qu + (size_t)ic * RS + (x < dceil ? x : 0));
-            }
-#pragma unroll
-            for (int ks = 0; ks < KS; ++ks) {
-                const int x = ks * 32 + g * 8;
-                const float4 da = *reinterpret_cast<const float4*>(dv + x), db = *reinterpret_cast<const float4*>(dv + x + 4);
-                const int valid = i < Tg ? p.d - x : 0;
-                const uint4 m = mask_chunk(ra[ks], valid);
-                qu[t][ks] = as_bf16x8(m);
-                const uint4 w = make_uint4(pack_bf2(__uint_as_float(m.x << 16) + da.x, __uint_as_float(m.x & 0xFFFF0000u) + da.y),
-                                           pack_bf2(__uint_as_float(m.y << 16) + da.z, __uint_as_float(m.y & 0xFFFF0000u) + da.w),
-                                           pack_bf2(__uint_as_float(m.z << 16) + db.x, __uint_as_float(m.z & 0xFFFF0000u) + db.y),
-                                           pack_bf2(__uint_as_float(m.w << 16) + db.z, __uint_as_float(m.w & 0xFFFF0000u) + db.w));
-                qv[t][ks] = as_bf16x8(mask_chunk(w, valid));
-            }
-        }
-    }
-#pragma unroll
-    for (int n = 0; n < NB; ++n) {
-        const int q = tid + NTHR * n;
-        const int rr = q / CPR, x = (q - rr * CPR) * 8;
-        if (q < (BI + 63) * CPR)
-            *reinterpret_cast<uint4*>(sE + SM::koff(rr, x >> 3)) = mask_chunk(fb[n], p.d - x);
-    }
-
-    f32x4 acc[QT][DT];
-    float m_run[QT], l_run[QT];
-#pragma unroll
-    for (int t = 0; t < QT; ++t) {
-        m_run[t] = NEG_BIG; l_run[t] = 0.f;
-#pragma unroll
-        for (int dt = 0; dt < DT; ++dt) acc[t][dt] = f32x4{0.f, 0.f, 0.f, 0.f};
-    }
     const float scale2 = p.scale * 1.44269504088896340736f;
     float* skew0 = sS + (wave * QT) * 16 * SKEW_LD + c * SKEW_LD;
     const int wcol = c - 15 + 4 * g;
@@ -215,6 +155,7 @@
     const char* vbase = sV + (4 * g + (c >> 2)) * SM::VP + (c & 3) * 8;
 
     static_assert(BI == 64, "ring phases: two (BI == BJ)");
+    static_assert(!SM::SWZ || (SM::KROW == 128 && ERING == 128), "swizzled ring: phase = bit 13 of the byte address");
     uint32_t ldk[NK], ldv[NK], lde[2][NK];
 #pragma unroll
     for (int n = 0; n < NK; ++n) {
@@ -227,222 +168,415 @@
         lde[1][n] = (uint32_t)SM::koff((BI - 1 + r + 64) & (ERING - 1), ch);
     }
     constexpr bool FULL = (BJ * CPR) % NTHR == 0;
-    auto publish = [&](const Stage& st_, int j0, int par) __attribute__((always_inline)) {
-        __syncthreads();
-#pragma unroll
-        for (int n = 0; n < NK; ++n) {
-            if (FULL || tid + NTHR * n < BJ * CPR) {
-                *reinterpret_cast<uint4*>(sK + ldk[n]) = st_.lk[n];
-                *reinterpret_cast<uint4*>(sV + ldv[n]) = st_.lv[n];
-                if (j0 > kbeg) *reinterpret_cast<uint4*>(sE + lde[par][n]) = st_.le[n];
-            }
-        }
-        __syncthreads();
+
+    auto issue_loads = [&](Stage& st_, const Attn2Item& it, int jn) __attribute__((always_inline)) {
+        if (((ABLATE(p) & 2) && jn > it.kbeg) || (ABLATE(p) & 64)) return;
+        if (jn + BJ <= it.Tg - (ragged_d ? 1 : 0)) {
+            const char* kb = reinterpret_cast<const char*>(it.Kh + (size_t)jn * RS);
+            const char* vb = reinterpret_cast<const char*>(it.Vh + (size_t)jn * RS);
+#pragma unroll
+            for (int n = 0; n < NK; ++n) { st_.lk[n] = ld16b(kb + koffs[n]); st_.lv[n] = ld16b(vb + koffs[n]); }
+        } else {
+#pragma unroll
+            for (int n = 0; n < NK; ++n) {
+                const int kr = chunk_row(n), j = jn + kr;
+                const size_t o = (size_t)(j < it.Tg ? j : it.Tg - 1) * RS * 2 + (koffs[n] - (uint32_t)(kr * RS) * 2u);
+                st_.lk[n] = tail_mask(ld16b(reinterpret_cast<const char*>(it.Kh) + o), n); st_.lv[n] = tail_mask(ld16b(reinterpret_cast<const char*>(it.Vh) + o), n);
+            }
+        }
+        if (jn > it.kbeg) {
+            const int rnew = it.R0 + (jn - it.kbeg) + BI - 1;
+            if (rnew >= 0 && rnew + 63 < it.erows - (ragged_d ? 1 : 0)) {
+                const char* eb = reinterpret_cast<const char*>(it.Eh + (size_t)rnew * ERS);
+#pragma unroll
+                for (int n = 0; n < NK; ++n) st_.le[n] = ld16b(eb + koffs[n]);
+            } else {
+#pragma unroll
+                for (int n = 0; n < NK; ++n) {
+                    const int er = chunk_row(n);
+                    int r = rnew + er;
+                    r = r < 0 ? 0 : (r >= it.erows ? it.erows - 1 : r);
+                    st_.le[n] = tail_mask(ld16b(reinterpret_cast<const char*>(it.Eh) + (size_t)r * ERS * 2 + (koffs[n] - (uint32_t)(er * RS) * 2u)), n);
+                }
+            }
+        }
     };
-
-    auto compute_block = [&](int j0, int par, auto jtv) __attribute__((always_inline)) {
-        constexpr int JTV = decltype(jtv)::value;
-        f32x4 st[QT][JTV];
-#pragma unroll
-        for (int jt = 0; jt < JTV; ++jt) {
-#pragma unroll
-            for (int t = 0; t < QT; ++t) st[t][jt] = f32x4{0.f, 0.f, 0.f, 0.f};
+    constexpr int NB = ((BI + 63) * CPR + NTHR - 1) / NTHR;
+    uint4 fb[NB], qraw[QT][KS];
+    float4 dvr[KS][2];
+    auto issue_head = [&](const Attn2Item& it) __attribute__((always_inline)) {
+        issue_loads(sa, it, it.kbeg);
+        const int tq = item_tid();
+#pragma unroll
+        for (int n = 0; n < NB; ++n) {
+            const int q = tq + NTHR * n;
+            const int rr = q / CPR, x = (q - rr * CPR) * 8;
+            const int r = it.R0 + (rr < BI + 63 ? rr : BI + 62);
+            const int rc = r < 0 ? 0 : (r >= it.erows ? it.erows - 1 : r);
+            fb[n] = (ABLATE(p) & 16) ? make_uint4(0, 0, 0, 0) : ld16(it.Eh + (size_t)rc * ERS + (x < dceil ? x : 0));
+        }
+        const int cq = tq & 15, gq = (tq >> 4) & 3;
+        const int iw0 = it.i0 + wave * 16 * QT;
+        const float* dv = P->dvu + (size_t)it.h * P->dvu_ld;
+#pragma unroll
+        for (int t = 0; t < QT; ++t) {
+            const int i = iw0 + 16 * t + cq, ic = i < it.Tg ? i : it.Tg - 1;
 #pragma unroll
             for (int ks = 0; ks < KS; ++ks) {
-                const bf16x8 a = *reinterpret_cast<const bf16x8*>(sK + SM::koff(jt * 16 + c, ks * 4 + g));
-#pragma unroll
-                for (int t = 0; t < QT; ++t) st[t][jt] = __builtin_amdgcn_mfma_f32_16x16x32_bf16(a, qu[t][ks], st[t][jt], 0, 0, 0);
-            }
-        }
-        const int rw1 = woff1 + 64 * par;
-        constexpr int PU = JTV + 1;
-        f32x4 pe[QT][PU];
-#pragma unroll
-        for (int t = 0; t < QT; ++t)
-#pragma unroll
-            for (int u = 0; u < PU; ++u) pe[t][u] = f32x4{0.f, 0.f, 0.f, 0.f};
-#pragma unroll
-        for (int u = 0; u < JTV + QT; ++u) {
-            const int er = ((rw1 + u * 16) & (ERING - 1)) + c;
+                const int x = ks * 32 + gq * 8;
+                qraw[t][ks] = (ABLATE(p) & 32) ? make_uint4(0, 0, 0, 0) : ld16(it.Qu + (size_t)ic * RS + (x < dceil ? x : 0));
+            }
+        }
+#pragma unroll
+        for (int ks = 0; ks < KS; ++ks) {
+            const int x = ks * 32 + gq * 8;
+            dvr[ks][0] = *reinterpret_cast<const float4*>(dv + x); dvr[ks][1] = *reinterpret_cast<const float4*>(dv + x + 4);
+        }
+    };
+
+    int id = xcd_remap(blockIdx.x, gridDim.x);
+    [[maybe_unused]] int wj = 0, wround = 0, wodd = 0, wcnt = 0, wbase = 0, wstep = 0;
+    if constexpr (PERS) {
+        const int x = blockIdx.x & 7, q = nwg >> 3, r = nwg & 7;
+        wj = blockIdx.x >> 3;
+        wbase = x < r ? x * (q + 1) : r * (q + 1) + (x - r) * q;
+        wcnt = q + (x < r ? 1 : 0);
+        wstep = (int)gridDim.x == nwg ? wcnt : (int)(gridDim.x >> 3);
+        id = wbase + wj;
+    }
+    Attn2Item cur = derive(lookup(id));
+    if (ABLATE(p) & 128) return;
+    issue_head(cur);
+
+    for (;;) {
+        if constexpr (PERS) asm volatile("" : "+s"(P));
+        const int tq = item_tid();
+        const int cq = tq & 15, gq = (tq >> 4) & 3;
+        [[maybe_unused]] Attn2Raw nraw{};
+        [[maybe_unused]] bool has_next = false;
+        if constexpr (PERS) {
+            wround += wstep; wodd ^= 1;
+            const int wi = wround + (wodd ? wstep - 1 - wj : wj);
+            has_next = wi < wcnt;
+            if (has_next) nraw = lookup(wbase + wi);
+        }
+        const int Tg = cur.Tg, T = cur.T, h = cur.h, nkv = cur.nkv, band_l = cur.band_l, band_r = cur.band_r, kbeg = cur.kbeg, nkeys = cur.nkeys;
+        const bool banded = cur.banded, tile_dead = cur.tile_dead;
+        const size_t orow0 = cur.orow0;
+        const int iw0 = cur.i0 + wave * 16 * QT;
+        bf16x8 qu[QT][KS], qv[QT][KS];
+#pragma unroll
+        for (int t = 0; t < QT; ++t) {
+            const int i = iw0 + 16 * t + cq;
 #pragma unroll
             for (int ks = 0; ks < KS; ++ks) {
-                const bf16x8 a = *reinterpret_cast<const bf16x8*>(sE + SM::koff(er, ks * 4 + g));
+                const int x = ks * 32 + gq * 8;
+                const float4 da = dvr[ks][0], db = dvr[ks][1];
+                const int valid = i < Tg ? P->d - x : 0;
+                const uint4 m = mask_chunk(qraw[t][ks], valid);
+                qu[t][ks] = as_bf16x8(m);
+                const uint4 w = make_uint4(pack_bf2(__uint_as_float(m.x << 16) + da.x, __uint_as_float(m.x & 0xFFFF0000u) + da.y),
+                                           pack_bf2(__uint_as_float(m.y << 16) + da.z, __uint_as_float(m.y & 0xFFFF0000u) + da.w),
+                                           pack_bf2(__uint_as_float(m.z << 16) + db.x, __uint_as_float(m.z & 0xFFFF0000u) + db.y),
+                                           pack_bf2(__uint_as_float(m.w << 16) + db.z, __uint_as_float(m.w & 0xFFFF0000u) + db.w));
+                qv[t][ks] = as_bf16x8(mask_chunk(w, valid));
+            }
+        }
+        if constexpr (PERS) __syncthreads();
+#pragma unroll
+        for (int n = 0; n < NB; ++n) {
+            const int q = tq + NTHR * n;
+            const int rr = q / CPR, x = (q - rr * CPR) * 8;
+            if (q < (BI + 63) * CPR)
+                *reinterpret_cast<uint4*>(sE + SM::koff(rr, x >> 3)) = mask_chunk(fb[n], P->d - x);
+        }
+        if constexpr (PERS) {
+#pragma unroll
+            for (int n = 0; n < NB; ++n) fb[n] = make_uint4(0, 0, 0, 0);
+#pragma unroll
+            for (int ks = 0; ks < KS; ++ks) {
+                dvr[ks][0] = make_float4(0.f, 0.f, 0.f, 0.f); dvr[ks][1] = dvr[ks][0];
+#pragma unroll
+                for (int t = 0; t < QT; ++t) qraw[t][ks] = make_uint4(0, 0, 0, 0);
+            }
+        }
+
+        f32x4 acc[QT][DT];
+        float m_run[QT], l_run[QT];
+#pragma unroll
+        for (int t = 0; t < QT; ++t) {
+            m_run[t] = NEG_BIG; l_run[t] = 0.f;
+#pragma unroll
+            for (int dt = 0; dt < DT; ++dt) acc[t][dt] = f32x4{0.f, 0.f, 0.f, 0.f};
+        }
+        auto publish = [&](const Stage& st_, int j0, int par) __attribute__((always_inline)) {
+            __syncthreads();
+#pragma unroll
+            for (int n = 0; n < NK; ++n) {
+                if (FULL || tid + NTHR * n < BJ * CPR) {
+                    *reinterpret_cast<uint4*>(sK + ldk[n]) = st_.lk[n];
+                    *reinterpret_cast<uint4*>(sV + ldv[n]) = st_.lv[n];
+                    if (j0 > kbeg) *reinterpret_cast<uint4*>(sE + (SM::SWZ ? lde[0][n] ^ (par ? 64u * SM::KROW : 0u) : lde[par][n])) = st_.le[n];
+                }
+            }
+            __syncthreads();
+        };
+
+        auto compute_block = [&](int j0, int par, auto jtv) __attribute__((always_inline)) {
+            constexpr int JTV = decltype(jtv)::value;
+            f32x4 st[QT][JTV];
+#pragma unroll
+            for (int jt = 0; jt < JTV; ++jt) {
+#pragma unroll
+                for (int t = 0; t < QT; ++t) st[t][jt] = f32x4{0.f, 0.f, 0.f, 0.f};
+#pragma unroll
+                for (int ks = 0; ks < KS; ++ks) {
+                    const bf16x8 a = *reinterpret_cast<const bf16x8*>(sK + SM::koff(jt * 16 + c, ks * 4 + g));
+#pragma unroll
+                    for (int t = 0; t < QT; ++t) st[t][jt] = __builtin_amdgcn_mfma_f32_16x16x32_bf16(a, qu[t][ks], st[t][jt], 0, 0, 0);
+                }
+            }
+            int w1 = woff1;
+            asm volatile("" : "+s"(w1));
+            const int rw1 = w1 + 64 * par;
+            constexpr int PU = JTV + 1;
+            f32x4 pe[QT][PU];
+#pragma unroll
+            for (int t = 0; t < QT; ++t)
+#pragma unroll
+                for (int u = 0; u < PU; ++u) pe[t][u] = f32x4{0.f, 0.f, 0.f, 0.f};
+#pragma unroll
+            for (int u = 0; u < JTV + QT; ++u) {
+                const int er = ((rw1 + u * 16) & (ERING - 1)) + c;
+#pragma unroll
+                for (int ks = 0; ks < KS; ++ks) {
+                    const bf16x8 a = *reinterpret_cast<const bf16x8*>(sE + SM::koff(er, ks * 4 + g));
+#pragma unroll
+                    for (int t = 0; t < QT; ++t) {
+                        const int ut = u - (QT - 1 - t);
+                        if (ut >= 0 && ut < PU) pe[t][ut] = __builtin_amdgcn_mfma_f32_16x16x32_bf16(a, qv[t][ks], pe[t][ut], 0, 0, 0);
+                    }
+                }
+            }
+            int wl = (int)__builtin_amdgcn_mbcnt_hi(~0u, __builtin_amdgcn_mbcnt_lo(~0u, 0u));
+            asm volatile("" : "+v"(wl));
+            const int wc = (wl & 15) - 15 + 4 * (wl >> 4);
+#pragma unroll
+            for (int t = 0; t < QT; ++t) {
+                float* row = skew0 + t * 16 * SKEW_LD + wc;
+#pragma unroll
+                for (int r = 0; r < 4; ++r) {
+                    const bool lo = wc + r >= 0;
+                    row[r + (lo ? 0 : 16 * JTV)] = lo ? pe[t][0][r] : pe[t][JTV][r];
+                }
+#pragma unroll
+                for (int u = 1; u < JTV; ++u)
+#pragma unroll
+                    for (int r = 0; r < 4; ++r) row[u * 16 + r] = pe[t][u][r];
+            }
+            wave_sync();
+
+#pragma unroll
+            for (int t = 0; t < QT; ++t) {
+                const float* skew = skew0 + t * 16 * SKEW_LD;
+                float mloc = -INFINITY;
+#pragma unroll
+                for (int jt = 0; jt < JTV; ++jt) {
+                    const f32x4 s4 = *reinterpret_cast<const f32x4*>(skew + jt * 16 + g * 4);
+#pragma unroll
+                    for (int r = 0; r < 4; ++r) st[t][jt][r] += s4[r];
+                }
+                const int iq0 = iw0 + 16 * t;
+                if (j0 + BJ > nkv || (banded && (j0 - (iq0 + 15) < -band_l || j0 + BJ - 1 - iq0 > band_r))) {
+                    const int iq = iq0 + c;
+#pragma unroll
+                    for (int jt = 0; jt < JTV; ++jt)
+#pragma unroll
+                        for (int r = 0; r < 4; ++r) {
+                            const int j = j0 + jt * 16 + g * 4 + r, dj = j - iq;
+                            st[t][jt][r] = (j < nkv && dj <= band_r && dj >= -band_l) ? st[t][jt][r] : NEG_BIG;
+                        }
+                }
+                if (tile_dead) {
+                    const bool dead = nkv < 1 || iq0 + c - band_l >= nkv;
+#pragma unroll
+                    for (int jt = 0; jt < JTV; ++jt)
+#pragma unroll
+                        for (int r = 0; r < 4; ++r) st[t][jt][r] = dead ? (j0 + jt * 16 + g * 4 + r < Tg ? 0.f : NEG_BIG) : st[t][jt][r];
+                }
+#pragma unroll
+                for (int jt = 0; jt < JTV; ++jt)
+#pragma unroll
+                    for (int r = 0; r < 4; ++r) mloc = fmaxf(mloc, st[t][jt][r]);
+                mloc = fmaxf(mloc, __shfl_xor(mloc, 16));
+                mloc = fmaxf(mloc, __shfl_xor(mloc, 32));
+                if (!__all((mloc - m_run[t]) * scale2 <= RESCALE_T)) {
+                    const float m_new = fmaxf(m_run[t], mloc);
+                    const float alpha = __builtin_amdgcn_exp2f((m_run[t] - m_new) * scale2);
+                    l_run[t] *= alpha;
+#pragma unroll
+                    for (int dt = 0; dt < DT; ++dt) { acc[t][dt][0] *= alpha; acc[t][dt][1] *= alpha; acc[t][dt][2] *= alpha; acc[t][dt][3] *= alpha; }
+                    m_run[t] = m_new;
+                }
+                const float nm = -m_run[t] * scale2;
+                float lsum = 0.f;
+#pragma unroll
+                for (int jt = 0; jt < JTV; ++jt)
+#pragma unroll
+                    for (int r = 0; r < 4; ++r) {
+                        const float e = __builtin_amdgcn_exp2f(fmaf(st[t][jt][r], scale2, nm));
+                        st[t][jt][r] = e;
+                        lsum += e;
+                    }
+                l_run[t] += lsum;
+            }
+#pragma unroll
+            for (int c2 = 0; c2 < JTV / 2; ++c2) {
+                bf16x8 pf[QT];
 #pragma unroll
                 for (int t = 0; t < QT; ++t) {
-                    const int ut = u - (QT - 1 - t);
-                    if (ut >= 0 && ut < PU) pe[t][ut] = __builtin_amdgcn_mfma_f32_16x16x32_bf16(a, qv[t][ks], pe[t][ut], 0, 0, 0);
-                }
-            }
-        }
-#pragma unroll
-        for (int t = 0; t < QT; ++t) {
-            float* row = skew0 + t * 16 * SKEW_LD + wcol;
-#pragma unroll
-            for (int r = 0; r < 4; ++r) {
-                const bool lo = wcol + r >= 0;
-                row[r + (lo ? 0 : 16 * JTV)] = lo ? pe[t][0][r] : pe[t][JTV][r];
-            }
-#pragma unroll
-            for (int u = 1; u < JTV; ++u)
-#pragma unroll
-                for (int r = 0; r < 4; ++r) row[u * 16 + r] = pe[t][u][r];
-        }
-        wave_sync();
-
-#pragma unroll
-        for (int t = 0; t < QT; ++t) {
-            const float* skew = skew0 + t * 16 * SKEW_LD;
-            float mloc = -INFINITY;
-#pragma unroll
-            for (int jt = 0; jt < JTV; ++jt) {
-                const f32x4 s4 = *reinterpret_cast<const f32x4*>(skew + jt * 16 + g * 4);
-#pragma unroll
-                for (int r = 0; r < 4; ++r) st[t][jt][r] += s4[r];
-            }
-            const int iq0 = iw0 + 16 * t;
-            if (j0 + BJ > nkv || (banded && (j0 - (iq0 + 15) < -band_l || j0 + BJ - 1 - iq0 > band_r))) {
-                const int iq = iq0 + c;
-#pragma unroll
-                for (int jt = 0; jt < JTV; ++jt)
-#pragma unroll
-                    for (int r = 0; r < 4; ++r) {
-                        const int j = j0 + jt * 16 + g * 4 + r, dj = j - iq;
-                        st[t][jt][r] = (j < nkv && dj <= band_r && dj >= -band_l) ? st[t][jt][r] : NEG_BIG;
+                    uint4 pb;
+                    pb.x = pack_bf2(st[t][2 * c2][0], st[t][2 * c2][1]);
+                    pb.y = pack_bf2(st[t][2 * c2][2], st[t][2 * c2][3]);
+                    pb.z = pack_bf2(st[t][2 * c2 + 1][0], st[t][2 * c2 + 1][1]);
+                    pb.w = pack_bf2(st[t][2 * c2 + 1][2], st[t][2 * c2 + 1][3]);
+                    pf[t] = as_bf16x8(pb);
+                }
+#pragma unroll
+                for (int dt = 0; dt < DT; ++dt) {
+                    const uint2 lo = lds_tr16(vbase + (2 * c2) * 16 * SM::VP + dt * 32);
+                    const uint2 hi = lds_tr16(vbase + (2 * c2 + 1) * 16 * SM::VP + dt * 32);
+                    const bf16x8 a = as_bf16x8(make_uint4(lo.x, lo.y, hi.x, hi.y));
+#pragma unroll
+                    for (int t = 0; t < QT; ++t) acc[t][dt] = __builtin_amdgcn_mfma_f32_16x16x32_bf16(a, pf[t], acc[t][dt], 0, 0, 0);
+                }
+            }
+        };
+
+        const bool wave_idle = iw0 >= Tg;
+        const bool short_ok = !tile_dead;
+        auto run_block = [&](int j0, int par) __attribute__((always_inline)) {
+            if (wave_idle || (ABLATE(p) & 1)) return;
+            if (short_ok && nkeys - j0 <= 32) compute_block(j0, par, std::integral_constant<int, 2>{});
+            else compute_block(j0, par, std::integral_constant<int, 4>{});
+        };
+        constexpr bool TWO_SETS = SETS == 2 || (SETS == 0 && !(NWV == 2 && DP >= 96));
+        if constexpr (TWO_SETS) {
+            if (kbeg + BJ < nkeys) issue_loads(sb, cur, kbeg + BJ);
+            for (int jb = kbeg; jb < nkeys; jb += 2 * BJ)
+#pragma unroll
+            for (int half2 = 0; half2 < 2; ++half2) {
+                const int j0 = jb + half2 * BJ;
+                if (j0 >= nkeys) break;
+                if (half2 == 0) publish(sa, j0, 0); else publish(sb, j0, 1);
+                if (j0 + 2 * BJ < nkeys) { if (half2 == 0) issue_loads(sa, cur, j0 + 2 * BJ); else issue_loads(sb, cur, j0 + 2 * BJ); }
+                run_block(j0, half2);
+            }
+        } else {
+            for (int jb = kbeg; jb < nkeys; jb += 2 * BJ)
+#pragma unroll
+            for (int half2 = 0; half2 < 2; ++half2) {
+                const int j0 = jb + half2 * BJ;
+                if (j0 >= nkeys) break;
+                publish(sa, j0, half2);
+                if (j0 + BJ < nkeys) issue_loads(sa, cur, j0 + BJ);
+                run_block(j0, half2);
+            }
+        }
+
+        auto epilogue = [&]() __attribute__((always_inline)) {
+            const int te = item_tid();
+            const int cq = te & 15, gq = (te >> 4) & 3;
+#pragma unroll
+            for (int t = 0; t < QT; ++t) {
+                float l_tot = l_run[t] + __shfl_xor(l_run[t], 16);
+                l_tot += __shfl_xor(l_tot, 32);
+                const float inv = 1.0f / l_tot;
+                const int i = iw0 + 16 * t + cq;
+                if (i >= Tg || (ABLATE(p) & 4)) continue;
+#pragma unroll
+                for (int dt = 0; dt < DT; ++dt) {
+                    const int x0 = dt * 16 + gq * 4;
+                    if (x0 >= P->d) continue;
+                    int n0 = h * P->d + x0, toff = 0;
+                    while (n0 >= P->D) { n0 -= P->D; ++toff; }
+                    const int t0 = i * P->G + toff;
+                    if (x0 + 3 < P->d && n0 + 3 < P->D && (n0 & 1) == 0) {
+                        if (t0 < T || P->rag_off) {
+                            typedef uint32_t u32x2_a4 __attribute__((ext_vector_type(2), aligned(4)));
+                            u32x2_a4 w;
+                            w[0] = t0 < T ? pack_bf2(acc[t][dt][0] * inv, acc[t][dt][1] * inv) : 0u;
+                            w[1] = t0 < T ? pack_bf2(acc[t][dt][2] * inv, acc[t][dt][3] * inv) : 0u;
+                            *reinterpret_cast<u32x2_a4*>(P->out + (orow0 + t0) * P->ldo + n0) = w;
+                        }
+                    } else {
+#pragma unroll
+                        for (int r = 0; r < 4; ++r) {
+                            const int x = x0 + r;
+                            if (x >= P->d) continue;
+                            int n = h * P->d + x, tf = 0;
+                            while (n >= P->D) { n -= P->D; ++tf; }
+                            const int tt = i * P->G + tf;
+                            if (tt < T || P->rag_off) P->out[(orow0 + tt) * P->ldo + n] = tt < T ? f2bf(acc[t][dt][r] * inv) : (bf16_t)0;
+                        }
                     }
-            }
-            if (tile_dead) {
-                const bool dead = nkv < 1 || iq0 + c - band_l >= nkv;
-#pragma unroll
-                for (int jt = 0; jt < JTV; ++jt)
-#pragma unroll
-                    for (int r = 0; r < 4; ++r) st[t][jt][r] = dead ? (j0 + jt * 16 + g * 4 + r < Tg ? 0.f : NEG_BIG) : st[t][jt][r];
-            }
-#pragma unroll
-            for (int jt = 0; jt < JTV; ++jt)
-#pragma unroll
-                for (int r = 0; r < 4; ++r) mloc = fmaxf(mloc, st[t][jt][r]);
-            mloc = fmaxf(mloc, __shfl_xor(mloc, 16));
-            mloc = fmaxf(mloc, __shfl_xor(mloc, 32));
-            if (!__all((mloc - m_run[t]) * scale2 <= RESCALE_T)) {
-                const float m_new = fmaxf(m_run[t], mloc);
-                const float alpha = __builtin_amdgcn_exp2f((m_run[t] - m_new) * scale2);
-                l_run[t] *= alpha;
-#pragma unroll
-                for (int dt = 0; dt < DT; ++dt) { acc[t][dt][0] *= alpha; acc[t][dt][1] *= alpha; acc[t][dt][2] *= alpha; acc[t][dt][3] *= alpha; }
-                m_run[t] = m_new;
-            }
-            const float nm = -m_run[t] * scale2;
-            float lsum = 0.f;
-#pragma unroll
-            for (int jt = 0; jt < JTV; ++jt)
-#pragma unroll
-                for (int r = 0; r < 4; ++r) {
-                    const float e = __builtin_amdgcn_exp2f(fmaf(st[t][jt][r], scale2, nm));
-                    st[t][jt][r] = e;
-                    lsum += e;
-                }
-            l_run[t] += lsum;
-        }
-#pragma unroll
-        for (int c2 = 0; c2 < JTV / 2; ++c2) {
-            bf16x8 pf[QT];
-#pragma unroll
-            for (int t = 0; t < QT; ++t) {
-                uint4 pb;
-                pb.x = pack_bf2(st[t][2 * c2][0], st[t][2 * c2][1]);
-                pb.y = pack_bf2(st[t][2 * c2][2], st[t][2 * c2][3]);
-                pb.z = pack_bf2(st[t][2 * c2 + 1][0], st[t][2 * c2 + 1][1]);
-                pb.w = pack_bf2(st[t][2 * c2 + 1][2], st[t][2 * c2 + 1][3]);
-                pf[t] = as_bf16x8(pb);
-            }
-#pragma unroll
-            for (int dt = 0; dt < DT; ++dt) {
-                const uint2 lo = lds_tr16(vbase + (2 * c2) * 16 * SM::VP + dt * 32);
-                const uint2 hi = lds_tr16(vbase + (2 * c2 + 1) * 16 * SM::VP + dt * 32);
-                const bf16x8 a = as_bf16x8(make_uint4(lo.x, lo.y, hi.x, hi.y));
-#pragma unroll
-                for (int t = 0; t < QT; ++t) acc[t][dt] = __builtin_amdgcn_mfma_f32_16x16x32_bf16(a, pf[t], acc[t][dt], 0, 0, 0);
-            }
-        }
-    };
-
-    const bool wave_idle = iw0 >= Tg;
-    const bool short_ok = !tile_dead;
-    auto run_block = [&](int j0, int par) __attribute__((always_inline)) {
-        if (wave_idle || (ABLATE(p) & 1)) return;
-        if (short_ok && nkeys - j0 <= 32) compute_block(j0, par, std::integral_constant<int, 2>{});
-        else compute_block(j0, par, std::integral_constant<int, 4>{});
-    };
-    constexpr bool TWO_SETS = SETS == 2 || (SETS == 0 && !(NWV == 2 && DP >= 96));
-    if constexpr (TWO_SETS) {
-        if (kbeg + BJ < nkeys) issue_loads(sb, kbeg + BJ);
-        for (int jb = kbeg; jb < nkeys; jb += 2 * BJ)
-#pragma unroll
-        for (int half2 = 0; half2 < 2; ++half2) {
-            const int j0 = jb + half2 * BJ;
-            if (j0 >= nkeys) break;
-            if (half2 == 0) publish(sa, j0, 0); else publish(sb, j0, 1);
-            if (j0 + 2 * BJ < nkeys) { if (half2 == 0) issue_loads(sa, j0 + 2 * BJ); else issue_loads(sb, j0 + 2 * BJ); }
-            run_block(j0, half2);
-        }
-    } else {
-        for (int jb = kbeg; jb < nkeys; jb += 2 * BJ)
-#pragma unroll
-        for (int half2 = 0; half2 < 2; ++half2) {
-            const int j0 = jb + half2 * BJ;
-            if (j0 >= nkeys) break;
-            publish(sa, j0, half2);
-            if (j0 + BJ < nkeys) issue_loads(sa, j0 + BJ);
-            run_block(j0, half2);
+                }
+            }
+        };
+        if constexpr (PERS) {
+            if (!has_next) { epilogue(); return; }
+            asm volatile("" : "+s"(P));
+            const Attn2Item nxt = derive(nraw);
+            issue_head(nxt);
+            asm volatile("" ::: "memory");
+            epilogue();
+            cur = nxt;
+        } else {
+            epilogue();
+            return;
         }
     }
-
-#pragma unroll
-    for (int t = 0; t < QT; ++t) {
-        float l_tot = l_run[t] + __shfl_xor(l_run[t], 16);
-        l_tot += __shfl_xor(l_tot, 32);
-        const float inv = 1.0f / l_tot;
-        const int i = iw0 + 16 * t + c;
-        if (i >= Tg || (ABLATE(p) & 4)) continue;
-#pragma unroll
-        for (int dt = 0; dt < DT; ++dt) {
-            const int x0 = dt * 16 + g * 4;
-            if (x0 >= p.d) continue;
-            int n0 = h * p.d + x0, toff = 0;
-            while (n0 >= p.D) { n0 -= p.D; ++toff; }
-            const int t0 = i * p.G + toff;
-            if (x0 + 3 < p.d && n0 + 3 < p.D && (n0 & 1) == 0) {
-                if (t0 < T || p.rag_off) {
-                    typedef uint32_t u32x2_a4 __attribute__((ext_vector_type(2), aligned(4)));
-                    u32x2_a4 w;
-                    w[0] = t0 < T ? pack_bf2(acc[t][dt][0] * inv, acc[t][dt][1] * inv) : 0u;
-                    w[1] = t0 < T ? pack_bf2(acc[t][dt][2] * inv, acc[t][dt][3] * inv) : 0u;
-                    *reinterpret_cast<u32x2_a4*>(p.out + (orow0 + t0) * p.ldo + n0) = w;
-                }
-            } else {
-#pragma unroll
-                for (int r = 0; r < 4; ++r) {
-                    const int x = x0 + r;
-                    if (x >= p.d) continue;
-                    int n = h * p.d + x, tf = 0;
-                    while (n >= p.D) { n -= p.D; ++tf; }
-                    const int tt = i * p.G + tf;
-                    if (tt < T || p.rag_off) p.out[(orow0 + tt) * p.ldo + n] = tt < T ? f2bf(acc[t][dt][r] * inv) : (bf16_t)0;
-                }
-            }
-        }
+}
+
+template <int DP, int NWV, int QT, int SETS>
+int persistent_slots() {
+    using SM = Attn2Smem<DP, NWV, QT>;
+    static int slots[16] = {};
+    int dev = 0;
+    (void)hipGetDevice(&dev);
+    dev &= 15;
+    if (slots[dev] == 0) {
+        constexpr int shaped = DP <= 64 && SETS == 1 ? 3 : (DP <= 96 ? 2 : 1);
+        int cus = 0, per_cu = 0;
+        if (hipDeviceGetAttribute(&cus, hipDeviceAttributeMultiprocessorCount, dev) != hipSuccess || cus <= 0) { (void)hipGetLastError(); return -1; }
+        if (hipOccupancyMaxActiveBlocksPerMultiprocessor(&per_cu, reinterpret_cast<const void*>(&relpos_attention2_kernel<DP, NWV, QT, SETS, true>), NWV * 64,
+                                                         SM::TOTAL) != hipSuccess || per_cu <= 0) { (void)hipGetLastError(); return -1; }
+        per_cu = per_cu < shaped ? per_cu : shaped;
+        const int n = cus * per_cu / 8 * 8;
+        slots[dev] = n >= 8 ? n : 8;
     }
+    return slots[dev];
 }
 
 template <int DP, int NWV, int QT, int SETS = 0>
 int launch2(const AttnParams& p, hipStream_t s) {
     using SM = Attn2Smem<DP, NWV, QT>;
     static_assert(SM::TOTAL <= 160 * 1024, "LDS");
-    static LdsAttr attr;
-    ensure_dynamic_lds(reinterpret_cast<const void*>(&relpos_attention2_kernel<DP, NWV, QT, SETS>), SM::TOTAL, attr);
     const int qtiles = (p.Tg + SM::BI - 1) / SM::BI;
     const int nwg = p.rag_off ? p.rag_nwg : p.B * p.H * qtiles;
     if (nwg <= 0) return 0;
+    if constexpr (NWV == 4 && QT == 1) {
+        if (p.persist) {
+            static LdsAttr pattr;
+            ensure_dynamic_lds(reinterpret_cast<const void*>(&relpos_attention2_kernel<DP, NWV, QT, SETS, true>), SM::TOTAL, pattr);
+            const int slots = persistent_slots<DP, NWV, QT, SETS>();
+            if (slots <= 0) return -1;
+            hipLaunchKernelGGL((relpos_attention2_kernel<DP, NWV, QT, SETS, true>), dim3(nwg < slots ? nwg : slots), dim3(NWV * 64), SM::TOTAL, s, p);
+            return hipGetLastError() == hipSuccess ? 0 : -1;
+        }
+    }
+    static LdsAttr attr;
+    ensure_dynamic_lds(reinterpret_cast<const void*>(&relpos_attention2_kernel<DP, NWV, QT, SETS>), SM::TOTAL, attr);
     hipLaunchKernelGGL((relpos_attention2_kernel<DP, NWV, QT, SETS>), dim3(nwg), dim3(NWV * 64), SM::TOTAL, s, p);
     return hipGetLastError() == hipSuccess ? 0 : -1;
 }
diff --git a/efficientconformer_amd/csrc/encoder.hip b/efficientconformer_amd/csrc/encoder.hip
--- a/efficientconformer_amd/csrc/encoder.hip
+++ b/efficientconformer_amd/csrc/encoder.hip
@@ -85,6 +85,7 @@
     bool fuse_chain = true;
     int ctc_mfma = 2;
     int attention_v2 = 1;
+    int attention_persist = 1;
     int chain_full_max = 192;
     int dwconv_mfma = 1;
     int chain_pair = 5;
@@ -752,6 +753,7 @@
             const long long unit = (long long)mask_stride * G;
             ap.band_l = (int)std::min<long long>(c.left_context / unit, 1 << 30); ap.band_r = (int)std::min<long long>(c.right_context / unit, 1 << 30);
             ap.causal = c.causal;
+            ap.persist = e->attention_persist;
             const bool streaming = c.causal || ap.band_l < Tg || ap.band_r < Tg;
             if (streaming && !(nat && relpos_attention2_supported(dpad) && e->attention_v2))
                 return fail("streaming contexts / causal attention run on attention2.hip (natural layout, padded head width <= 160, option attention_v2 != 0)");
@@ -2120,8 +2122,9 @@
     ap.out = out; ap.ldo = ld_out; ap.scale = 1.0f / std::sqrt((float)d);
     ap.band_l = ap.band_r = 1 << 30;
     if (variant == 0) { EC_TRY(launch_relpos_attention(ap, (hipStream_t)stream)); return 0; }
-    if ((variant != 1 && variant != 2) || !relpos_attention2_supported(dpad)) return fail("attention variant not available for this head width");
-    EC_TRY(launch_relpos_attention2(ap, variant, (hipStream_t)stream));
+    if ((variant != 1 && variant != 2 && variant != 3) || !relpos_attention2_supported(dpad)) return fail("attention variant not available for this head width");
+    ap.persist = variant == 1;
+    EC_TRY(launch_relpos_attention2(ap, variant == 3 ? 1 : variant, (hipStream_t)stream));
     return 0;
 }
 
@@ -2354,6 +2357,7 @@
     if (!strcmp(name, "fuse_chain")) { e->fuse_chain = value != 0; return 0; }
     if (!strcmp(name, "ctc_mfma")) { if (value < 0 || value > 2) return fail("ctc_mfma: 0 (VALU), 1 (fp32 MFMA) or 2 (split-bf16 MFMA)"); e->ctc_mfma = value; return 0; }
     if (!strcmp(name, "wide_gemm")) { if (value < 0 || (value > 3 && value < 16)) return fail("wide_gemm: 0 (by shape), 1 (never), 2 (256-column tile), 3 (128-column tile), >= 16 (by shape with this many 256 x 256 tiles as the threshold)"); e->wide_gemm = value; return 0; }
+    if (!strcmp(name, "attention_persist")) { if (value != 0 && value != 1) return fail("attention_persist: 0 or 1"); e->attention_persist = value; return 0; }
     if (!strcmp(name, "attention_v2")) { if (value != 0 && value != 1 && value != 2) return fail("attention_v2: 0, 1 or 2"); e->attention_v2 = value; return 0; }
     if (!strcmp(name, "chain_full_max")) { if (value < 0 || value > 256) return fail("chain_full_max: widest stage (0..256) that runs chain A as ONE kernel"); e->chain_full_max = value; return 0; }
     if (!strcmp(name, "chain_max_dim")) { e->chain_max_dim = value; return 0; }
diff --git a/efficientconformer_amd/csrc/kernels.h b/efficientconformer_amd/csrc/kernels.h
--- a/efficientconformer_amd/csrc/kernels.h
+++ b/efficientconformer_amd/csrc/kernels.h
@@ -109,6 +109,7 @@
     float scale;
     const int *rag_off, *rag_wg; int rag_nwg, rag_tgmax;
     int band_l, band_r, causal;
+    int persist;
     int ablate;
 };
 int launch_relpos_attention(const AttnParams& p, hipStream_t s);
```

Result: slower. 58.42 million mel-frames/s (valid, 10 ms hop) (-1.8%).
